# i8run/BigDL

Measured on AMD Instinct MI355X. Metric: images/sec (whole node) ResNet-50 224x224 bf16 at 1/2/4/8 MI355X, higher is better.
Workload: dtype bf16; 1 GPU; model=ResNet-50 v1.5 (BigDL ImageNet builder), global_batch=256, per_gpu_batch=256, image=224, parallelism=dp1, optimizer=SGD momentum 0.9 + L2 1e-4 (one rank: no gradient exchange), hip_graph=False, wgrad_side_stream=True, bucketed_overlap=False, grad_compress=none (no exchange)

## Files before the change

bigdl_amd/nn/conv.py:

```python
import math

import torch
import torch.nn.functional as F

from .. import ops
from ..ops import bn as bnops
from ..ops import conv as cv
from ..ops import conv_fn
from ..ops import side_stream
from .abstractnn import AutogradModule, TensorModule, _t_begin, _t_end
from .init_methods import RandomUniform, Zeros

CL = torch.channels_last
BF16 = torch.bfloat16


def _same_pad(inp, k, s, d=1):
    out = -(-inp // s)
    total = max((out - 1) * s + (k - 1) * d + 1 - inp, 0)
    return total // 2, total - total // 2


class SpatialConvolution(TensorModule):
    def __init__(self, nInputPlane, nOutputPlane, kernelW, kernelH, strideW=1, strideH=1, padW=0, padH=0,
# ... 66 lines not shown
            return 0, 0
        bh, ah = _same_pad(H, self.kernelH, self.strideH, self.dilationH)
        bw, aw = _same_pad(W, self.kernelW, self.strideW, self.dilationW)
        return ah - bh, aw - bw

    def _prep(self, x):
        H, W = x.shape[2], x.shape[3]
        ph, pw = self._pads(H, W)
        eh, ew = self._same_extra(H, W)
        if eh or ew:
            x = F.pad(x, (0, ew, 0, eh))
            if x.is_cuda:
                x = x.contiguous(memory_format=CL)
        return x, ph, pw, eh, ew

    def _nchw(self, x):
        if self.format == "NHWC":
            return x.permute(0, 3, 1, 2)
        return x

    def _fmt_out(self, y):
        if self.format == "NHWC":
            return y.permute(0, 2, 3, 1)
        return y

    def _pre_ok(self, x):
        if not (x.is_cuda and x.dim() == 4 and self.format == "NCHW" and self.nGroup == 1
                and x.shape[1] == self.nInputPlane and x.shape[1] % 8 == 0 and x.dtype == BF16
                and x.is_contiguous(memory_format=CL)):
            return False
        if self._same_extra(x.shape[2], x.shape[3]) != (0, 0) or self._pair_path(x):
            return False
        return getattr(self, "_fuse_out", None) is None and getattr(self, "_fuse_addend", None) is None

    def updateOutput(self, input):
        if getattr(input, "_bn_pre", None) is not None and not self._pre_ok(input):
            input = bnops.materialize(input)
        x = self._nchw(input)
        squeeze = x.dim() == 3
        if squeeze:
            x = x.unsqueeze(0)
        x, ph, pw, _, _ = self._prep(x)
        if x.is_cuda and self.nGroup == 1:
            y = self._fwd_gpu(x, ph, pw)
        elif x.is_cuda:
            y = self._fwd_gpu_grouped(x, ph, pw)
        else:
            y = F.conv2d(x.float(), self.weight, self.bias, (self.strideH, self.strideW), (ph, pw),
                         (self.dilationH, self.dilationW), self.nGroup)
            if self.fuse_relu:
                y = torch.relu(y)
        if squeeze:
            y = y.squeeze(0)
        return self._fmt_out(y)

    def _w16_padded(self):
        w16 = self.w16("weight")
        if w16.shape[1] % 8 != 0:
            w16 = cv.weight_krsc_bf16(w16.float())
        return w16

    def _pair_path(self, x):
        return (cv.pair_ok(x.shape[1], (self.strideH, self.strideW), (self.dilationH, self.dilationW), self.nGroup)
                and self.nInputPlane == x.shape[1] and getattr(self, "_fuse_out", None) is None
                and getattr(self, "_fuse_addend", None) is None)

    def _fwd_gpu_pairs(self, x, ph, pw):
        R, S, sh = self.kernelH, self.kernelW, self.strideH
        OH, OW, S2, _, _ = cv.pair_geometry(x.shape[2], x.shape[3], R, S, sh, ph, pw)
        xp = cv.to_pairs_bf16(x, R, S, sh, ph, pw)
        self._xpair = (xp, tuple(x.shape), ph, pw)
        self._x16 = None
        wp = cv.pair_weight(self.w16("weight"))
        stats = None
        if self.emit_stats and self.train and self.nOutputPlane % 8 == 0:
            stats = bnops.new_stats(self.nOutputPlane, x.device)
        y = cv.conv2d_pairs_fwd(xp, wp, self.bias, self.nOutputPlane, OH, OW, R, S2, sh, relu=self.fuse_relu,
                                stats=stats)
        if stats is not None:
            y._bn_stats = stats
        self._geom = (x.shape, ph, pw)
        return y

    def _wgrad_gpu_pairs(self, x, gy16):
        xp, shape, ph, pw = self._xpair
        R, S, K = self.kernelH, self.kernelW, self.nOutputPlane
        S2 = (S + 1) // 2
        dwp = ops.zeros(K, R * S2 * 8, device=x.device)
        db = None
        if self.bias is not None:
            db = self.gradBias if self.scaleB == 1.0 else ops.zeros(K, device=x.device)
        cv.conv2d_pairs_wgrad(gy16, xp, R, S2, self.strideH, dwp, db)
        ops.native.get().pair_wgrad_add(dwp, self.gradWeight, float(self.scaleW))
        if db is not None and db is not self.gradBias:
            self.gradBias.add_(db, alpha=self.scaleB)

    def _fwd_gpu(self, x, ph, pw):
        self._xpair = None
        self._x16_pre = None
        pre = getattr(x, "_bn_pre", None)
        if self._pair_path(x) and self.nOutputPlane % 8 == 0 and pre is None:
            return self._fwd_gpu_pairs(x, ph, pw)
        x16 = cv.to_nhwc_bf16(x)
        self._x16 = x16
        w16 = self._w16_padded()
        stats = None
        if self.emit_stats and self.train and self.nOutputPlane % 8 == 0:
            stats = bnops.new_stats(self.nOutputPlane, x.device)
        out, addend = getattr(self, "_fuse_out", None), getattr(self, "_fuse_addend", None)
        self._fuse_out = self._fuse_addend = None
        y = cv.conv2d_fwd(x16, w16, self.bias, (self.strideH, self.strideW), (ph, pw),
                          (self.dilationH, self.dilationW), relu=self.fuse_relu, stats=stats, out=out,
                          addend=addend, pre=pre)
        if pre is not None:
            y, mat = y
            if mat is None:
                self._x16_pre = pre
            else:
                self._x16 = mat
        if stats is not None:
            y._bn_stats = stats
        self._geom = (x.shape, ph, pw)
        return y

    def _direct_groups(self):
        return self.nGroup > 1 and self.nInputPlane // self.nGroup <= 16

    def _geo_g(self, ph, pw):
        return [self.strideH, self.strideW, ph, pw, self.dilationH, self.dilationW, self.nGroup]

    def _fwd_gpu_grouped(self, x, ph, pw):
        G = self.nGroup
        cin, cout = self.nInputPlane // G, self.nOutputPlane // G
        if self._direct_groups():
            xf = x.float().contiguous()
            OH = cv.out_size(x.shape[2], self.kernelH, self.strideH, ph, self.dilationH)
            OW = cv.out_size(x.shape[3], self.kernelW, self.strideW, pw, self.dilationW)
            y = xf.new_empty(x.shape[0], self.nOutputPlane, OH, OW)
            ops.native.get().gconv(0, xf, self.weight.float().contiguous(),
                                   self.bias.float().contiguous() if self.bias is not None else None, y,
                                   self._geo_g(ph, pw))
            if self.fuse_relu:
                y.relu_()
            self._xf = xf
            self._geom = (x.shape, ph, pw)
            return y.to(BF16).contiguous(memory_format=CL)
        outs = []
        w = self.weight
        self._x16 = cv.to_nhwc_bf16(x) if x.shape[1] % 8 == 0 else None
        for g in range(G):
            xg = cv.to_nhwc_bf16(x[:, g * cin:(g + 1) * cin].contiguous(memory_format=CL))
            wg = cv.weight_krsc_bf16(w[g * cout:(g + 1) * cout])
            bg = self.bias[g * cout:(g + 1) * cout] if self.bias is not None else None
            outs.append(cv.conv2d_fwd(xg, wg, bg, (self.strideH, self.strideW), (ph, pw),
                                      (self.dilationH, self.dilationW), relu=self.fuse_relu))
        self._geom = (x.shape, ph, pw)
        return torch.cat(outs, dim=1).contiguous(memory_format=CL)

    def updateGradInput(self, input, gradOutput):
        if not self.propagateBack:
            return None
        x = self._nchw(input)
        gy = self._nchw(gradOutput)
        squeeze = x.dim() == 3
        if squeeze:
            x, gy = x.unsqueeze(0), gy.unsqueeze(0)
        H, W = x.shape[2], x.shape[3]
        x, ph, pw, eh, ew = self._prep(x)
        compact = getattr(self, "_dgrad_compact_once", False) and not (squeeze or eh or ew or self.format != "NCHW")
        self._dgrad_compact_once = False
        if gy.is_cuda:
            gy = self._relu_mask(gy)
            once = getattr(self, "_dgrad_bn_once", False)
            self._dgrad_bn_once = False
            bn_src = getattr(input, "_bn_bwd", None) if (getattr(self, "_dgrad_bn_ok", False) or once) else None
# ... 27 lines not shown
            if gy16.shape[1] % 8:
                gy16 = cv.pad_dim(gy16, 1)
                w16 = cv.pad_dim(w16, 0)
            wt = getattr(self, "_wt_cache", None)
            if getattr(self, "_wt_stamp", None) != cv.WT_STAMP[0] or wt is None or \
                    tuple(wt.shape) != (w16.shape[1], w16.shape[2], w16.shape[3], w16.shape[0]):
                wt = cv.transpose_w(w16)
            Cp = w16.shape[1]
            xs = (x.shape[0], Cp, x.shape[2], x.shape[3])
            addend = getattr(self, "_dgrad_addend", None)
            self._dgrad_addend = None
            addend_zm = None
            if isinstance(addend, tuple):
                addend, addend_zm = addend
            if addend is not None and Cp != x.shape[1]:
                raise RuntimeError("dgrad addend requires unpadded channels")
            bn = None
            if bn_src is not None and Cp == x.shape[1]:
                bnmod, bx, bmean, baff, bz = bn_src
                bzm = None
                if bz is not None and bz.dtype == torch.uint8:
                    bz, bzm = None, bz
                bn = {"x": bx, "z": bz, "zm": bzm, "mean": bmean, "aff": baff,
                      "red": bnops.new_stats(Cp, gy16.device)}
            gi = cv.conv2d_dgrad(gy16, wt, xs, (self.strideH, self.strideW), (ph, pw),
                                 (self.dilationH, self.dilationW), addend=addend, bn=bn, addend_zm=addend_zm,
                                 compact=compact and Cp == x.shape[1])
            if Cp != x.shape[1]:
                gi = gi[:, : x.shape[1]].contiguous(memory_format=CL)
            elif bn is not None and bn.get("done"):
                gi._bn_red = (bnmod, bn["red"])
            return gi
        G = self.nGroup
        cin, cout = self.nInputPlane // G, self.nOutputPlane // G
        if self._direct_groups():
            gyf = gy.float().contiguous()
            dx = torch.empty(x.shape[0], self.nInputPlane, x.shape[2], x.shape[3], device=gy.device)
            ops.native.get().gconv(1, dx, self.weight.float().contiguous(), None, gyf, self._geo_g(ph, pw))
            return dx.to(BF16).contiguous(memory_format=CL)
        parts = []
        for g in range(G):
            wg = cv.pad_dim(cv.weight_krsc_bf16(self.weight[g * cout:(g + 1) * cout]), 0)
            gyg = cv.pad_dim(gy16[:, g * cout:(g + 1) * cout].contiguous(memory_format=CL), 1)
            xs = (x.shape[0], wg.shape[1], x.shape[2], x.shape[3])
            gi = cv.conv2d_dgrad(gyg, cv.transpose_w(wg), xs, (self.strideH, self.strideW), (ph, pw),
                                 (self.dilationH, self.dilationW))
            parts.append(gi[:, :cin])
        return torch.cat(parts, dim=1).contiguous(memory_format=CL)

    def backward(self, input, gradOutput):
        side = None if self._frozen else side_stream.stream_for(gradOutput)
        if side is None:
            return super().backward(input, gradOutput)
        t0 = _t_begin(gradOutput)
        self.gradInput = self.updateGradInput(input, gradOutput)
        side_stream.begin(side)
        with torch.cuda.stream(side):
            self.accGradParameters(input, gradOutput)
            self._apply_regularizers()
        side_stream.keep(side, input, gradOutput, self.output, getattr(self, "_x16", None),
                         *(getattr(self, "_xpair", None) or (None,))[:1])
        _t_end(self, t0, "backward_time")
        return self.gradInput

    def accGradParameters(self, input, gradOutput):
        x = self._nchw(input)
        gy = self._nchw(gradOutput)
        if x.dim() == 3:
            x, gy = x.unsqueeze(0), gy.unsqueeze(0)
        x, ph, pw, _, _ = self._prep(x)
        if gy.is_cuda:
            gy = self._relu_mask(gy) if self.fuse_relu and not getattr(self, "_masked_cached", False) else gy
            self._wgrad_gpu(x, gy, ph, pw)
            return
        gy = self._relu_mask(gy).float()
        gw = torch.nn.grad.conv2d_weight(x.float(), self.weight.shape, gy, (self.strideH, self.strideW), (ph, pw),
                                         (self.dilationH, self.dilationW), self.nGroup)
        self.gradWeight.add_(gw, alpha=self.scaleW)
        if self.bias is not None:
            self.gradBias.add_(gy.sum(dim=(0, 2, 3)), alpha=self.scaleB)

    def _wgrad_gpu(self, x, gy, ph, pw):
        gy16 = gy if (gy.dtype == BF16 and gy.is_contiguous(memory_format=CL)) else gy.to(BF16, memory_format=CL)
        xpair = getattr(self, "_xpair", None)
        if (xpair is not None and xpair[1] == tuple(x.shape) and xpair[2:] == (ph, pw) and self.nGroup == 1
                and self.gradWeight.dtype == torch.float32):
            self._wgrad_gpu_pairs(x, gy16)
            return
        x16 = getattr(self, "_x16", None)
        pre = None
        if x16 is None or x16.shape[0] != x.shape[0] or x16.shape[2:] != x.shape[2:]:
            x16 = cv.to_nhwc_bf16(bnops.materialize(x))
        elif getattr(self, "_x16_pre", None) is not None:
            pre = self._x16_pre
        st, pd, dl = (self.strideH, self.strideW), (ph, pw), (self.dilationH, self.dilationW)
        if self.nGroup != 1 and self._direct_groups():
            xf = getattr(self, "_xf", None)
            if xf is None or xf.shape != x.shape:
                xf = x.float().contiguous()
            dw = ops.zeros(self.weight.shape, device=x.device)
            db = ops.zeros(self.nOutputPlane, device=x.device) if self.bias is not None else None
            ops.native.get().gconv(2, xf, dw, db, gy.float().contiguous(), self._geo_g(pd[0], pd[1]))
            self.gradWeight.add_(dw, alpha=self.scaleW)
            if db is not None:
                self.gradBias.add_(db, alpha=self.scaleB)
            return
        if self.nGroup != 1:
            G = self.nGroup
            cin, cout = self.nInputPlane // G, self.nOutputPlane // G
            for g in range(G):
                xg = cv.to_nhwc_bf16(x[:, g * cin:(g + 1) * cin].contiguous(memory_format=CL))
                gyg = cv.pad_dim(gy16[:, g * cout:(g + 1) * cout].contiguous(memory_format=CL), 1)
                dw = ops.zeros(gyg.shape[1], xg.shape[1], self.kernelH, self.kernelW, device=x.device,
                               memory_format=CL)
                db = ops.zeros(gyg.shape[1], device=x.device) if self.bias is not None else None
                cv.conv2d_wgrad(gyg, xg, dw, db, st, pd, dl)
                self.gradWeight[g * cout:(g + 1) * cout].add_(dw[:cout, :cin], alpha=self.scaleW)
                if db is not None:
                    self.gradBias[g * cout:(g + 1) * cout].add_(db[:cout], alpha=self.scaleB)
            return
        K = self.nOutputPlane
        direct = (x16.shape[1] == self.nInputPlane and K % 8 == 0 and self.scaleW == 1.0 and self.scaleB == 1.0
                  and self.gradWeight.is_contiguous(memory_format=CL))
        if pre is not None and not direct:
            x16 = bnops.materialize(bnops.deferred(x16, pre))
        if direct:
            cv.conv2d_wgrad(gy16, x16, self.gradWeight, self.gradBias, st, pd, dl, pre=pre)
        else:
            gyp = cv.pad_dim(gy16, 1)
            dw = ops.zeros(gyp.shape[1], x16.shape[1], self.kernelH, self.kernelW, device=x.device,
                           memory_format=CL)
            db = ops.zeros(gyp.shape[1], device=x.device) if self.bias is not None else None
            cv.conv2d_wgrad(gyp, x16, dw, db, st, pd, dl)
            self.gradWeight.add_(dw[:K, : self.nInputPlane], alpha=self.scaleW)
            if db is not None:
                self.gradBias.add_(db[:K], alpha=self.scaleB)

    def clearState(self):
        super().clearState()
        self._x16 = None
        self._x16_pre = None
        self._xpair = None
        return self

    def __repr__(self):
        return (f"SpatialConvolution({self.nInputPlane} -> {self.nOutputPlane}, {self.kernelW} x {self.kernelH}, "
                f"{self.strideW}, {self.strideH}, {self.padW}, {self.padH})")


class SpatialShareConvolution(SpatialConvolution):
    """Reference shares im2col buffers across layers to save host memory (ResNet ``optnet``). On the GPU
    engine there is no im2col buffer at all (implicit GEMM), so this is SpatialConvolution."""


class SpatialDilatedConvolution(SpatialConvolution):
    def __init__(self, nInputPlane, nOutputPlane, kW, kH, dW=1, dH=1, padW=0, padH=0, dilationW=1, dilationH=1,
                 wRegularizer=None, bRegularizer=None):
        super().__init__(nInputPlane, nOutputPlane, kW, kH, dW, dH, padW, padH, wRegularizer=wRegularizer,
                         bRegularizer=bRegularizer, dilationW=dilationW, dilationH=dilationH)


class SpatialFullConvolution(AutogradModule):

    def __init__(self, nInputPlane, nOutputPlane, kW, kH, dW=1, dH=1, padW=0, padH=0, adjW=0, adjH=0, nGroup=1,
                 noBias=False, wRegularizer=None, bRegularizer=None):
        super().__init__()
        self.nInputPlane, self.nOutputPlane = nInputPlane, nOutputPlane
        self.kW, self.kH, self.dW, self.dH = kW, kH, dW, dH
        self.padW, self.padH, self.adjW, self.adjH, self.nGroup = padW, padH, adjW, adjH, nGroup
        self.wRegularizer, self.bRegularizer = wRegularizer, bRegularizer
        self.register_parameter("weight", "gradWeight", torch.empty(nInputPlane, nOutputPlane // nGroup, kH, kW))
# ... 249 lines not shown
```

bigdl_amd/nn/fusion.py:

```python
import os

import torch

from ..utils.table import Table
from .activation import ReLU
from .containers import ConcatTable, Sequential, add_activity
from .conv import SpatialConvolution
from .linear import Linear
from .normalization import BatchNormalization
from .table_ops import CAddTable


_TRAIN_NODE_ATTRS = ("res_src", "pass_index", "fold_fanout", "fold_bn")


def _reset(m):
    from .graph import Graph

    for x in [m] + list(m.flattened_layers()):
        if isinstance(x, Graph) and getattr(x, "_order0", None) is not None:
            x.order = x._order0
            x._order0 = None
        if isinstance(x, Graph):
            for n in x.order:
                for a in _TRAIN_NODE_ATTRS:
                    n.__dict__.pop(a, None)
        if isinstance(x, BatchNormalization):
            x._graph_dres = False
    for x in m.flattened_layers():
        for attr, val in (("emit_stats", False), ("fuse_relu", False), ("passthrough", False),
                          ("_dgrad_bn_ok", False), ("_defer_ok", False)):
            if hasattr(x, attr):
                setattr(x, attr, val)
        if isinstance(x, Sequential):
            x._residual_plan = None


def _dgrad_bn_enabled():
    return os.environ.get("BIGDL_DGRAD_BN", "1") == "1"


def fuse_for_training(model):
    from .graph import DynamicGraph, Graph

    _reset(model)
    for m in model.flattened_layers():
        if isinstance(m, Sequential):
            _fuse_sequential(m)
        elif isinstance(m, Graph) and not isinstance(m, DynamicGraph) and not getattr(m, "_inference_fused", False):
            _fuse_graph_training(m)
    return model


def _fuse_graph_training(g):
    users = _graph_users(g)
    outs = {n.id for n in g.output_nodes}
    _plan_graph_residuals(g, users, outs)

    def only_user(n):
        us = users.get(n.id, [])
        ok = (len(us) == 1 and n.id not in outs and len(us[0].prevs) == 1 and us[0].prev_index[0] is None
              and not (n.element.hasName() and n.element.getName() in g._stop_grad))
        return us[0] if ok else None

    for n in g.order:
        m, u = n.element, only_user(n)
        if u is None:
            continue
        c = u.element
        if isinstance(m, SpatialConvolution) and isinstance(c, BatchNormalization) and m.nGroup == 1:
            m.emit_stats = True
        elif isinstance(m, BatchNormalization) and isinstance(c, ReLU):
            m.fuse_relu = True
            c.passthrough = True
        elif isinstance(m, (SpatialConvolution, Linear)) and isinstance(c, ReLU):
            m.fuse_relu = True
            c.passthrough = True
    _plan_fanout_folds(g, users)
    for n in g.order:
        m, u = n.element, only_user(n)
        if isinstance(m, BatchNormalization) and u is not None and isinstance(u.element, ReLU):
            v = only_user(u)
            if v is not None:
                _plan_deferred_bn(m, u.element, v.element)
    if not _dgrad_bn_enabled():
        return
    for n in g.order:
        m, u = n.element, only_user(n)
        if not (isinstance(m, BatchNormalization) and m.fuse_relu and u is not None and isinstance(u.element, ReLU)
                and u.element.passthrough):
            continue
        v = only_user(u)
        if v is not None and isinstance(v.element, SpatialConvolution) and v.element.nGroup == 1:
            v.element._dgrad_bn_ok = True


def _stopped(g, n):
    return n.element.hasName() and n.element.getName() in g._stop_grad


def _plan_graph_residuals(g, users, outs):
    for a in list(g.order):
        if not isinstance(a.element, CAddTable) or len(a.prevs) != 2 or any(k is not None for k in a.prev_index):
            continue
        ua = users.get(a.id, [])
        if (len(ua) != 1 or a.id in outs or _stopped(g, a) or not isinstance(ua[0].element, ReLU)
                or len(ua[0].prevs) != 1 or ua[0].prev_index[0] is not None):
            continue
        for ib in (0, 1):
            b, sc = a.prevs[ib], a.prevs[1 - ib]
            bn = b.element
            if (b is sc or not isinstance(bn, BatchNormalization) or users.get(b.id) != [a] or b.id in outs
                    or _stopped(g, b) or bn.fuse_relu or bn.nOutput % 8 != 0 or getattr(b, "res_src", None)):
                continue
            order = g.order
            if order.index(sc) > order.index(b):
                if getattr(g, "_order0", None) is None:
                    g._order0 = list(order)
                order.remove(b)
                order.insert(order.index(sc) + 1, b)
            bn.fuse_relu = True
            bn._graph_dres = True
            b.res_src = sc
            a.pass_index = ib + 1
            ua[0].element.passthrough = True
            break


def _plan_fanout_folds(g, users):
    pos = {n.id: i for i, n in enumerate(g.order)}
    contrib = {}
    for n in g.order:
        rs = getattr(n, "res_src", None)
        if rs is not None:
            contrib.setdefault(rs.id, []).append(n)
    for p in g.order:
        us = [u for u in users.get(p.id, []) if getattr(u, "pass_index", None) is None]
        srcs = us + contrib.get(p.id, [])
        if len(srcs) < 2:
            continue
        c = min(srcs, key=lambda u: pos[u.id])
        cv = c.element
        if (c not in us or len(c.prevs) != 1 or c.prev_index[0] is not None or _stopped(g, c)
                or not isinstance(cv, SpatialConvolution) or cv.nGroup != 1 or not cv.propagateBack
                or cv.format != "NCHW" or cv.nInputPlane % 8 != 0):
            continue
        c.fold_fanout = True
        c.fold_bn = _dgrad_bn_enabled()


def unfuse(model):
    _reset(model)
    return model


def _last_leaf(m):
    while isinstance(m, Sequential) and m.modules and m._residual_plan is None:
        m = m.modules[-1]
    return m


def _fuse_sequential(seq):
    mods = seq.modules
    if (len(mods) == 3 and isinstance(mods[0], ConcatTable) and len(mods[0].modules) == 2
            and isinstance(mods[1], CAddTable) and isinstance(mods[2], ReLU)):
        branch, short = mods[0].modules
        if isinstance(branch, Sequential) and branch.modules and isinstance(branch.modules[-1], BatchNormalization):
            bn = branch.modules[-1]
            if bn.nOutput % 8 == 0:
                bn.fuse_relu = True
                seq._residual_plan = (branch, short, bn)
    for a, b in zip(mods[:-1], mods[1:]):
        if isinstance(a, SpatialConvolution) and isinstance(b, BatchNormalization) and a.nGroup == 1:
            a.emit_stats = True
        elif isinstance(a, BatchNormalization) and isinstance(b, ReLU):
            a.fuse_relu = True
            b.passthrough = True
    for a, b, c in zip(mods[:-2], mods[1:-1], mods[2:]):
        if (_dgrad_bn_enabled() and isinstance(a, BatchNormalization) and a.fuse_relu and isinstance(b, ReLU) and b.passthrough
                and isinstance(c, SpatialConvolution) and c.nGroup == 1):
            c._dgrad_bn_ok = True
        elif isinstance(a, (SpatialConvolution, Linear)) and isinstance(b, ReLU):
            a.fuse_relu = True
            b.passthrough = True
    for a, b, c in zip(mods[:-2], mods[1:-1], mods[2:]):
        _plan_deferred_bn(a, b, c)


DEFER_LEVEL = [int(os.environ.get("BIGDL_BN_DEFER", "1") or 0)]


def _defer_consumer(c):
    from .pooling import SpatialMaxPooling

    if isinstance(c, SpatialConvolution):
        if DEFER_LEVEL[0] < 2:
            return False
        return (c.nGroup == 1 and c.format == "NCHW" and type(c).updateOutput is SpatialConvolution.updateOutput
                and type(c)._wgrad_gpu is SpatialConvolution._wgrad_gpu and c.kernelW == 3 and c.kernelH == 3
                and c.strideW == 1 and c.strideH == 1 and c.dilationW == 1 and c.dilationH == 1)
    return DEFER_LEVEL[0] >= 1 and type(c) is SpatialMaxPooling and c.format == "NCHW"


def _plan_deferred_bn(a, b, c):
    if (isinstance(a, BatchNormalization) and a.fuse_relu and not getattr(a, "_graph_dres", False)
            and isinstance(b, ReLU) and b.passthrough and _defer_consumer(c)):
        a._defer_ok = True


def residual_forward(seq, x):
    branch, short, bn = seq._residual_plan
    concat, add, relu = seq.modules
    res = short.forward(x)
    h = x
    for m in branch.modules[:-1]:
        h = m.forward(h)
    if tuple(res.shape) != tuple(h.shape[:1]) + (bn.nOutput,) + tuple(h.shape[2:]):
        raise ValueError(f"residual block: shortcut output {tuple(res.shape)} does not match the branch output")
    out = bn.updateOutput(h, residual=res)
    bn.output = out
    branch.output = out
    concat.output = Table(out, res)
    add.output = out
    relu.output = out
    seq._res_h = h
    return out


MASKED_ADDEND = [os.environ.get("BIGDL_MASKED_ADDEND", "1") != "0"]


SHORTCUT_BN_RED = [os.environ.get("BIGDL_SHORTCUT_BN_RED", "1") != "0"]


def _native_det():
    from ..ops import native

    return native.deterministic()


def _compact_shortcut_conv(short, first, x):
    from ..ops import conv as cv

    if not (cv.COMPACT_SHORTCUT[0] and isinstance(short, Sequential) and len(short.modules) == 2):
        return None
    sconv, sbn = short.modules
    if not (isinstance(sconv, SpatialConvolution) and isinstance(sbn, BatchNormalization)
            and type(sconv).updateGradInput is SpatialConvolution.updateGradInput
            and type(sconv)._dgrad_gpu is SpatialConvolution._dgrad_gpu
            and torch.is_tensor(x) and x.is_cuda and x.dim() == 4 and x.dtype == torch.bfloat16
            and x.is_contiguous(memory_format=torch.channels_last)):
        return None

    def plain_1x1(c, strided):
        return (c.kernelH == 1 and c.kernelW == 1 and c.padH == 0 and c.padW == 0 and c.nGroup == 1
                and c.format == "NCHW" and c.propagateBack and not c._frozen
                and c.nInputPlane == x.shape[1] and c.nInputPlane % 8 == 0 and c.nOutputPlane % 8 == 0
                and ((c.strideH > 1 and c.strideW > 1) if strided else (c.strideH == 1 and c.strideW == 1)))

    if not (plain_1x1(sconv, True) and plain_1x1(first, False)
            and type(first)._dgrad_gpu is SpatialConvolution._dgrad_gpu):
        return None
    N, C, H, W = x.shape
    stride = (sconv.strideH, sconv.strideW)
    if not all(cv.addend_stride_applies(N, first.nOutputPlane, H, W, C, stride, bnm) for bnm in (0, 1, 2)):
        return None
    return sconv


def residual_backward(seq, x, gradOutput):
    branch, short, bn = seq._residual_plan
    mods = branch.modules
    first = mods[0]
    sconv = None
    can_fold = (isinstance(first, SpatialConvolution) and first.propagateBack and first.nGroup == 1
                and first.format == "NCHW" and first.nInputPlane % 8 == 0)
    masked = None
    zm = getattr(bn, "_zm", None)
    if (MASKED_ADDEND[0] and can_fold and zm is not None and type(short).__name__ == "Identity" and first.strideH == 1
            and first.strideW == 1 and torch.is_tensor(gradOutput) and gradOutput.is_cuda
            and tuple(gradOutput.shape) == tuple(x.shape) and x.dtype == torch.bfloat16):
        dh, _ = bn.backward_fused(seq._res_h, gradOutput, need_dres=False)
        gz = gradOutput
        if gz.dtype != torch.bfloat16 or not gz.is_contiguous(memory_format=torch.channels_last):
            gz = gz.to(torch.bfloat16).contiguous(memory_format=torch.channels_last)
        masked = (gz, zm)
        gs = None
    else:
        sec, sbn = None, None
        if SHORTCUT_BN_RED[0] and isinstance(short, Sequential) and short.modules:
            sbn = short.modules[-1]
            xs = getattr(sbn, "_xin", None)
            xb = getattr(bn, "_xin", None)
            if (isinstance(sbn, BatchNormalization) and sbn.train and not sbn.fuse_relu and xs is not None
                    and xb is not None and xs.is_cuda and xs.shape == xb.shape and xs.stride() == xb.stride()
                    and xs.dtype == torch.bfloat16 and xs.shape[1] % 8 == 0 and not _native_det()):
                from ..ops import bn as bnops

                sec = (xs, sbn.saveMean, bnops.new_stats(xs.shape[1], xs.device))
        dh, dres = bn.backward_fused(seq._res_h, gradOutput, need_dres=True, sec=sec)
        if sec is not None:
            dres._bn_red = (sbn, sec[2])
        sconv = _compact_shortcut_conv(short, first, x) if can_fold else None
        if sconv is not None:
            sconv._dgrad_compact_once = True
        gs = short.backward(x, dres)
        if sconv is not None:
            sconv._dgrad_compact_once = False
    bn.gradInput = dh
    from ..ops import conv as cv

    compact = gs is not None and cv.compact_stride(gs) is not None
    if compact and not (can_fold and sconv is not None and gs.dtype == x.dtype):
        gs, compact = cv.expand_compact(gs, x.shape[2], x.shape[3]), False
    fold = masked is not None or (can_fold and gs is not None and gs.dtype == x.dtype
                                  and (compact or gs.shape == x.shape))
    g = dh
    for i in range(len(mods) - 2, -1, -1):
        inp = mods[i - 1].output if i > 0 else x
        if i == 0 and fold:
            first._dgrad_addend = masked if masked is not None else gs
            first._dgrad_bn_once = _dgrad_bn_enabled()
        g = mods[i].backward(inp, g)
    return g if fold else add_activity(g, gs)


def _graph_users(g):
    users = {}
    for n in g.order:
        for p in n.prevs:
            users.setdefault(p.id, []).append(n)
    return users


def _conv_fusable(n):
    m = n.element
    return (type(m).__name__ in ("SpatialConvolution", "SpatialShareConvolution", "SpatialDilatedConvolution")
            and isinstance(m, SpatialConvolution) and m.nGroup == 1 and m.format == "NCHW")


def _conv_out_shape(conv, x):
    from ..ops.conv import out_size

    N, _, H, W = x.shape
    ph, pw = conv._pads(H, W)
    return (N, conv.nOutputPlane, out_size(H, conv.kernelH, conv.strideH, ph, conv.dilationH),
            out_size(W, conv.kernelW, conv.strideW, pw, conv.dilationW))


def _topo_with_deps(g, extra):
    order, state = [], {}
    for root in list(g.output_nodes) + list(g.inputs_nodes):
        stack = [(root, False)]
        while stack:
            n, done = stack.pop()
            if done:
                if state.get(n.id) != 2:
                    state[n.id] = 2
                    order.append(n)
                continue
            st = state.get(n.id)
            if st == 2:
                continue
            if st == 1:
                raise ValueError("inference fusion created a cycle")
            state[n.id] = 1
            stack.append((n, True))
            for p in reversed(list(n.prevs) + extra.get(n.id, [])):
                if state.get(p.id) != 2:
                    if state.get(p.id) == 1:
                        raise ValueError("inference fusion created a cycle")
                    stack.append((p, False))
    return order


class _ResidualLink:

    def __init__(self, conv, other_id, add, idx, relu):
        self.conv, self.other_id, self.add, self.idx, self.relu = conv, other_id, add, idx, relu
        self.used = False

    def pre_conv(self, outs, x):
        import torch
# ... 140 lines not shown
```

bigdl_amd/nn/normalization.py:

```python
import math
import os

import torch
import torch.nn.functional as F

from .. import ops
from ..ops import bn as bnops
from .abstractnn import AutogradModule, TensorModule, _t_begin, _t_end
from .init_methods import Ones, RandomUniform, Zeros

_ZMASK = os.environ.get("BIGDL_BN_ZMASK", "1") != "0"
_DEFER = [os.environ.get("BIGDL_BN_DEFER", "1") != "0"]
CL = torch.channels_last
BF16 = torch.bfloat16


class BatchNormalization(TensorModule):

    def __init__(self, nOutput, eps=1e-5, momentum=0.1, affine=True, initWeight=None, initBias=None,
                 initGradWeight=None, initGradBias=None, dataFormat="NCHW"):
        super().__init__()
        self.nOutput = nOutput
        self.eps = eps
        self.momentum = momentum
        self.affine = affine
        self.dataFormat = dataFormat
        self.fuse_relu = False
        self.sync_fn = None
        if affine:
            self.register_parameter("weight", "gradWeight", torch.empty(nOutput))
            self.register_parameter("bias", "gradBias", torch.empty(nOutput))
        else:
            self.weight = self.bias = self.gradWeight = self.gradBias = None
        self.runningMean = torch.zeros(nOutput)
        self.runningVar = torch.ones(nOutput)
        self._buffers = ["runningMean", "runningVar"]
        self.saveMean = None
        self.saveStd = None
        self.weightInitMethod = RandomUniform(0.0, 1.0) if affine else None
        self.biasInitMethod = Zeros()
        self.reset()
        if initWeight is not None and affine:
            self.weight.copy_(torch.as_tensor(initWeight))
        if initBias is not None and affine:
            self.bias.copy_(torch.as_tensor(initBias))
        if initGradWeight is not None and affine:
            self.gradWeight.copy_(torch.as_tensor(initGradWeight))
        if initGradBias is not None and affine:
            self.gradBias.copy_(torch.as_tensor(initGradBias))

    def reset(self):
        if self.affine:
            with torch.no_grad():
                self.weightInitMethod.init(self.weight)
                self.biasInitMethod.init(self.bias)
        self.runningMean.zero_()
        self.runningVar.fill_(1.0)

    def setParallism(self, n):
        from ..parallel.sync_bn import make_sync_fn

        self.sync_fn = make_sync_fn() if n and n > 1 else None
        return self

    def _to_nchw(self, x):
        if self.dataFormat == "NHWC" and x.dim() == 4:
            return x.permute(0, 3, 1, 2)
        return x

    def _from_nchw(self, y):
        if self.dataFormat == "NHWC" and y.dim() == 4:
            return y.permute(0, 2, 3, 1)
        return y

    def _gpu_ok(self, x):
        if not x.is_cuda or self.nOutput % 8 != 0:
            return False
        if x.dim() == 4:
            return True
        return x.dim() == 2

    def _prep_gpu(self, x):
        if x.dim() == 4:
            if x.dtype != BF16 or not x.is_contiguous(memory_format=CL):
                x = x.to(BF16, memory_format=CL)
        else:
            if x.dtype != BF16 or not x.is_contiguous():
                x = x.to(BF16).contiguous()
        return x

    def updateOutput(self, input, residual=None):
        if residual is None:
            residual = self.__dict__.pop("_graph_residual", None)
        x = self._to_nchw(input)
        if self._gpu_ok(x):
            stats = getattr(input, "_bn_stats", None) if self.train else None
            x = self._prep_gpu(x)
            res = residual
            if res is not None and (res.dtype != BF16 or res.stride() != x.stride()):
                res = res.to(BF16).contiguous(memory_format=CL if x.dim() == 4 else torch.contiguous_format)
            zm = None
            if self.train and self.fuse_relu and res is not None and x.shape[1] % 8 == 0 and _ZMASK:
                zm = torch.empty(x.numel() // 8, dtype=torch.uint8, device=x.device)
            if (self.train and self.fuse_relu and res is None and getattr(self, "_defer_ok", False) and _DEFER[0]
                    and x.dim() == 4 and self.dataFormat == "NCHW"):
                sm, si, aff = bnops.bn_prepare_gpu(x, self.weight, self.bias, self.runningMean, self.runningVar,
                                                   self.eps, self.momentum, stats=stats, sync_fn=self.sync_fn)
                self.saveMean, self.saveStd = sm, si
                self._aff, self._zm, self._xin = aff, None, x
                y = bnops.deferred(x, aff)
                y._bn_bwd = (self, x, sm, aff, False)
                return y
            y, sm, si, aff = bnops.bn_forward_gpu(x, self.weight, self.bias, self.runningMean, self.runningVar,
                                                   self.eps, self.momentum, self.train, stats=stats, res=res,
                                                   relu=self.fuse_relu, sync_fn=self.sync_fn if self.train else None,
                                                   zm=zm)
            self.saveMean, self.saveStd = sm, si
            self._aff = aff if (self.fuse_relu and res is None) else None
            self._zm = zm
            self._xin = x
            if self.train and self.fuse_relu:
                y._bn_bwd = (self, x, sm, self._aff, zm if zm is not None else res is not None)
            return self._from_nchw(y)
        xf = x.float()
        y, mean, invstd = bnops.bn_forward_cpu(xf, self.weight, self.bias, self.runningMean, self.runningVar, self.eps,
                                               self.momentum, self.train,
                                               sync_fn=self.sync_fn if self.train else None)
        if residual is not None:
            y = y + residual.float()
        if self.fuse_relu:
            y = torch.relu(y)
        self.saveMean, self.saveStd = mean, invstd
        self._xin = xf
        return self._from_nchw(y.to(input.dtype) if input.is_floating_point() else y)

    def _direct_grads(self):
        return (not self._frozen) and self.affine and self.scaleW == 1.0 and self.scaleB == 1.0

    def backward_fused(self, input, gradOutput, need_dres=False, sec=None):
        gz = self._to_nchw(gradOutput)
        x = self._xin
        if gz.dtype != BF16 or gz.stride() != x.stride():
            gz = gz.to(BF16).contiguous(memory_format=CL if x.dim() == 4 else torch.contiguous_format)
        aff = getattr(self, "_aff", None)
        zm = getattr(self, "_zm", None)
        z = self._to_nchw(self.output) if (self.fuse_relu and aff is None and zm is None) else None
        direct = self._direct_grads()
        dg = self.gradWeight if direct else (torch.zeros_like(self.runningMean) if self.affine else None)
        db = self.gradBias if direct else (torch.zeros_like(self.runningMean) if self.affine else None)
        pre = getattr(gradOutput, "_bn_red", None)
        red = pre[1] if (pre is not None and pre[0] is self and self.train) else None
        graph_res = getattr(self, "_graph_dres", False)
        dx, dres = bnops.bn_backward_gpu(gz, z, x, self.saveMean, self.saveStd, self.weight, dg, db,
                                         training=self.train, need_dres=need_dres or graph_res,
                                         sync_fn=self.sync_fn if self.train else None, aff=aff, red=red, zm=zm,
                                         sec=sec)
        if graph_res:
            self._dres = dres
        if not direct and self.affine and not self._frozen:
            self.gradWeight.add_(dg, alpha=self.scaleW)
            self.gradBias.add_(db, alpha=self.scaleB)
        return self._from_nchw(dx), dres

    def backward(self, input, gradOutput):
        t0 = _t_begin(gradOutput)
        x = self._to_nchw(input)
        if self._gpu_ok(x):
            self.gradInput, _ = self.backward_fused(input, gradOutput)
        else:
            self.gradInput = self.updateGradInput(input, gradOutput)
            if not self._frozen:
                self.accGradParameters(input, gradOutput)
        _t_end(self, t0, "backward_time")
        return self.gradInput

    def _cpu_grads(self, gradOutput):
        gy = self._to_nchw(gradOutput).float()
        if self.fuse_relu:
            gy = gy * (self._to_nchw(self.output) > 0)
        return bnops.bn_backward_cpu(self._xin, gy, self.saveMean, self.saveStd, self.weight, self.train,
                                     sync_fn=self.sync_fn if self.train else None)

    def updateGradInput(self, input, gradOutput):
        x = self._to_nchw(input)
        if self._gpu_ok(x):
            dx, _ = self.backward_fused(input, gradOutput)
            return dx
        gx, dg, db = self._cpu_grads(gradOutput)
        self._pending = (dg, db)
        return self._from_nchw(gx.to(input.dtype))

    def accGradParameters(self, input, gradOutput):
        if not self.affine:
            return
        if input.is_cuda and self._gpu_ok(self._to_nchw(input)):
            return
        pend = getattr(self, "_pending", None)
        if pend is None:
            _, dg, db = self._cpu_grads(gradOutput)
        else:
            dg, db = pend
        self.gradWeight.add_(dg.to(self.gradWeight.device), alpha=self.scaleW)
        self.gradBias.add_(db.to(self.gradBias.device), alpha=self.scaleB)
        self._pending = None

    def __repr__(self):
        return f"{type(self).__name__}[{self.nOutput}, eps={self.eps}, momentum={self.momentum}, affine={self.affine}]"


class SpatialBatchNormalization(BatchNormalization):
    pass


class LayerNormalization(AutogradModule):
    def __init__(self, hiddenSize, eps=1e-6):
        super().__init__()
        self.hiddenSize, self.eps = hiddenSize, eps
        self.register_parameter("weight", "gradWeight", torch.ones(hiddenSize))
        self.register_parameter("bias", "gradBias", torch.zeros(hiddenSize))

    def fn(self, x):
        from ..ops.norm import layer_norm

        xf = x.float()
        y = layer_norm(xf, self.weight, self.bias, self.eps)
        return y.to(x.dtype)


class SpatialCrossMapLRN(AutogradModule):

    def __init__(self, size=5, alpha=1.0, beta=0.75, k=1.0, format="NCHW"):
        super().__init__()
        self.size, self.alpha, self.beta, self.k, self.format = size, alpha, beta, k, format

    def fn(self, x):
        from ..ops import nnk

        xf = x.float()
        if self.format == "NHWC":
# ... 120 lines not shown
```

bigdl_amd/ops/bn.py:

```python
import os
import torch

from . import native


def _P(x):
    return x.numel() // x.shape[1]


def stat_slots():
    return native.get().STAT_SLOTS


class _StatsArena:

    def __init__(self):
        self.buf, self.off, self.active, self.need = None, 0, False, 0

    def begin(self, device):
        if self.need and (self.buf is None or self.buf.numel() < self.need or self.buf.device != device):
            self.buf = torch.empty(self.need, dtype=torch.float32, device=device)
        if self.buf is not None:
            if self.buf.is_cuda and int(os.environ.get("BIGDL_NATIVE_FILL", "7")) & 2:
                native.get().fill_bytes(self.buf, 0)
            else:
                self.buf.zero_()
        self.off, self.need, self.active = 0, 0, True

    def end(self):
        self.active = False

    def take(self, n, device):
        n_al = (n + 63) // 64 * 64
        self.need += n_al
        if self.active and self.buf is not None and self.buf.device == device and self.off + n_al <= self.buf.numel():
            t = self.buf[self.off:self.off + n]
            self.off += n_al
            return t
        t = torch.empty(n, dtype=torch.float32, device=device)
        if t.is_cuda:
            native.get().fill_bytes(t, 0)
            return t
        return t.zero_()


ARENA = _StatsArena()


def new_stats(C, device):
    return ARENA.take(stat_slots() * 2 * C, torch.device(device))


def _reduce_slots_for_sync(buf, C, P, sync_fn):
    red = torch.empty(2 * C, dtype=torch.float32, device=buf.device)
    native.get().bn_slot_reduce(buf, stat_slots(), C, red)
    P = sync_fn(red, P)
    return red, 1, P


def bn_forward_gpu(x, gamma, beta, rmean, rvar, eps, momentum, training, stats=None, res=None, relu=False,
                   out=None, sync_fn=None, zm=None):
    C = x.shape[1]
    P = _P(x)
    C_ = native.get()
    dev = x.device
    if out is None:
        out = torch.empty_like(x)
    aff = torch.empty(2 * C, dtype=torch.float32, device=dev)
    scale, shift = aff[:C], aff[C:]
    smean = torch.empty(C, dtype=torch.float32, device=dev)
    sinv = torch.empty(C, dtype=torch.float32, device=dev)
    nslots = stat_slots()
    Ptot = P
    if training:
        if stats is None:
            stats = new_stats(C, dev)
            C_.bn_stats(x, stats, P, C)
        if sync_fn is not None:
            stats, nslots, Ptot = _reduce_slots_for_sync(stats, C, P, sync_fn)
    else:
        stats, nslots = scale, 0
    C_.bn_finalize(stats, nslots, gamma, beta, rmean, rvar, smean, sinv, scale, shift, Ptot, C, float(eps),
                   float(momentum), bool(training))
    C_.bn_apply(x, scale, shift, res, out, P, C, bool(relu), zm)
    return out, smean, sinv, aff


def bn_prepare_gpu(x, gamma, beta, rmean, rvar, eps, momentum, stats=None, sync_fn=None):
    C = x.shape[1]
    P = _P(x)
    C_ = native.get()
    dev = x.device
    aff = torch.empty(2 * C, dtype=torch.float32, device=dev)
    smean = torch.empty(C, dtype=torch.float32, device=dev)
    sinv = torch.empty(C, dtype=torch.float32, device=dev)
    nslots, Ptot = stat_slots(), P
    if stats is None:
        stats = new_stats(C, dev)
        C_.bn_stats(x, stats, P, C)
    if sync_fn is not None:
        stats, nslots, Ptot = _reduce_slots_for_sync(stats, C, P, sync_fn)
    C_.bn_finalize(stats, nslots, gamma, beta, rmean, rvar, smean, sinv, aff[:C], aff[C:], Ptot, C, float(eps),
                   float(momentum), True)
    return smean, sinv, aff


def deferred(x, aff):
    y = x.detach()
    y._bn_pre = aff
    return y


def materialize(t):
    aff = getattr(t, "_bn_pre", None)
    if aff is None:
        return t
    C = t.shape[1]
    y = torch.empty_like(t)
    native.get().bn_apply(t, aff[:C], aff[C:], None, y, _P(t), C, True)
    return y


def bn_backward_gpu(dz, z, x, smean, sinv, gamma, dgamma, dbeta, training=True, need_dres=False, need_dx=True,
                    sync_fn=None, aff=None, red=None, zm=None, sec=None):
    C = x.shape[1]
    P = _P(x)
    C_ = native.get()
    nslots, Ptot = 0, P
    if not training:
        red = None
    elif red is None:
        red = new_stats(C, x.device)
        C_.bn_bwd_reduce(dz, z, x, smean, red, P, C, aff, zm)
    if training:
        nslots = stat_slots()
        if sync_fn is not None:
            red, nslots, Ptot = _reduce_slots_for_sync(red, C, P, sync_fn)
    coef = torch.empty(3 * C, dtype=torch.float32, device=x.device)
    dx = torch.empty_like(x) if need_dx else None
    dres = torch.empty_like(x) if need_dres else None
    if sec is not None and dres is not None and training:
        x2, mean2, red2 = sec
        C_.bn_bwd_apply(dz, z, x, smean, sinv, gamma, red, nslots, coef, dx, dres, dgamma, dbeta, Ptot, C, aff, zm,
                        x2=x2, mean2=mean2, red2=red2)
    else:
        C_.bn_bwd_apply(dz, z, x, smean, sinv, gamma, red, nslots, coef, dx, dres, dgamma, dbeta, Ptot, C, aff, zm)
    return dx, dres


def bn_forward_cpu(x, gamma, beta, rmean, rvar, eps, momentum, training, sync_fn=None):
    dims = [0] + list(range(2, x.dim()))
    shape = [1, -1] + [1] * (x.dim() - 2)
    if training:
        n = x.numel() // x.shape[1]
        if sync_fn is not None:
            buf = torch.cat([x.sum(dim=dims), (x * x).sum(dim=dims)]).double()
            n = sync_fn(buf, n)
            C = x.shape[1]
            mean = (buf[:C] / n).float()
            var = (buf[C:] / n - (buf[:C] / n) ** 2).clamp_min(0).float()
        else:
            mean = x.mean(dim=dims)
            var = x.var(dim=dims, unbiased=False)
        if rmean is not None:
            unb = var * n / max(n - 1, 1)
            rmean.mul_(1 - momentum).add_(momentum * mean)
            rvar.mul_(1 - momentum).add_(momentum * unb)
    else:
        mean, var = rmean, rvar
    invstd = torch.rsqrt(var + eps)
    xhat = (x - mean.view(shape)) * invstd.view(shape)
    y = xhat
    if gamma is not None:
        y = y * gamma.view(shape) + beta.view(shape)
    return y, mean, invstd


def bn_backward_cpu(x, gy, mean, invstd, gamma, training=True, sync_fn=None):
    dims = [0] + list(range(2, x.dim()))
    shape = [1, -1] + [1] * (x.dim() - 2)
    xhat = (x - mean.view(shape)) * invstd.view(shape)
    g = gamma.view(shape) if gamma is not None else 1.0
    dgamma = (gy * xhat).sum(dim=dims)
    dbeta = gy.sum(dim=dims)
    if training:
        n = x.numel() // x.shape[1]
        sdg, sdb = dgamma, dbeta
        if sync_fn is not None:
            buf = torch.cat([dbeta, dgamma]).double()
            n = sync_fn(buf, n)
            C = x.shape[1]
            sdb, sdg = buf[:C].float(), buf[C:].float()
        gx = g * invstd.view(shape) * (gy - sdb.view(shape) / n - xhat * sdg.view(shape) / n)
    else:
        gx = g * invstd.view(shape) * gy
    return gx, dgamma, dbeta
```

bigdl_amd/ops/conv.py:

```python
import os
import torch
import torch.nn.functional as F

from . import native

CL = torch.channels_last
BF16 = torch.bfloat16


def out_size(inp, k, s, p, d=1, ceil=False):
    eff = d * (k - 1) + 1
    num = inp + 2 * p - eff
    if ceil:
        o = -(-num // s) + 1
        if (o - 1) * s >= inp + p:
            o -= 1
        return o
    return num // s + 1


def to_nhwc_bf16(x, cpad=8):
    N, C, H, W = x.shape
    Cp = -(-C // cpad) * cpad
    if x.dtype == BF16 and Cp == C and x.is_contiguous(memory_format=CL):
# ... 268 lines not shown

def gemm_wgrad_nt(dy2d, x2d, dw32, dbias32=None):
    P, K = dy2d.shape
    C = x2d.shape[1]
    dyT, xT = _rows_T64(dy2d), _rows_T64(x2d)
    P64 = dyT.shape[1]
    geo = [K, 1, 1, P64, 1, 1, 1, 1, P64, C, C, 1, 1, 1, 1, 0, 0]
    native.get().conv_nt(dyT, xT, dw32.view(K, C), None, None, geo, [0, 0, 0], False, accumulate=True)
    if dbias32 is not None:
        native.get().colsum_bf16(dy2d, dbias32)


def pair_ok(C, stride, dil, groups):
    import os

    return (groups == 1 and C <= 4 and stride[1] == 2 and tuple(dil) == (1, 1)
            and os.environ.get("BIGDL_CONV_PAIR", "1") != "0")


def pair_geometry(H, W, R, S, sh, ph, pw):
    OH, OW = out_size(H, R, sh, ph), out_size(W, S, 2, pw)
    S2 = (S + 1) // 2
    Hp = max(H + 2 * ph, (OH - 1) * sh + R)
    Wp = max(2 * (OW - 1 + S2), W + 2 * pw)
    return OH, OW, S2, Hp, Wp + (Wp & 1)


def to_pairs_bf16(x, R, S, sh, ph, pw):
    N, C, H, W = x.shape
    _, _, _, Hp, Wp = pair_geometry(H, W, R, S, sh, ph, pw)
    y = torch.empty((N, Hp, Wp // 2, 8), dtype=BF16, device=x.device)
    xf = x if (x.dtype == torch.float32 and x.is_contiguous()) else x.float().contiguous()
    native.get().nchw_to_pairs(xf, y, ph, pw)
    return y


def pair_weight(w16):
    K, C, R, S = w16.shape
    wp = torch.empty((K, R * ((S + 1) // 2) * 8), dtype=BF16, device=w16.device)
    native.get().pair_weight(w16, wp)
    return wp


def _pair_taps(R, S2):
    key = ("p", R, S2)
    t = _TAP_CACHE.get(key)
    if t is None:
        t = []
        for r in range(R):
            for j in range(S2):
                t += [r, j, r * S2 + j]
        _TAP_CACHE[key] = t
    return t


def _window_taps(R):
    key = ("w", R)
    t = _TAP_CACHE.get(key)
    if t is None:
        t = [v for r in range(R) for v in (r, 0, r)]
        _TAP_CACHE[key] = t
    return t


def conv2d_pairs_fwd(xp, wp, bias, K, OH, OW, R, S2, sh, relu=False, stats=None):
    N, Hp, Wq, _ = xp.shape
    out = torch.empty((N, K, OH, OW), dtype=BF16, device=xp.device, memory_format=CL)
    if S2 == 4 and os.environ.get("BIGDL_STEM_WINDOW", "0") != "0":
        geo = [N, Hp, Wq, 32, OH, OW, sh, 1, R * 32, K, K, OH, OW, 1, 1, 0, 0, 8]
        det = stats is not None and native.deterministic()
        native.get().conv_nt(xp, wp, out, bias, None if det else stats, geo, _window_taps(R), relu, None)
        if det:
            native.get().bn_stats(out, stats, N * OH * OW, K)
        return out
    geo = [N, Hp, Wq, 8, OH, OW, sh, 1, R * S2 * 8, K, K, OH, OW, 1, 1, 0, 0]
    if stats is not None and native.deterministic():
        native.get().conv_nt(xp, wp, out, bias, None, geo, _pair_taps(R, S2), relu, None)
        native.get().bn_stats(out, stats, N * OH * OW, K)
        return out
    native.get().conv_nt(xp, wp, out, bias, stats, geo, _pair_taps(R, S2), relu, None)
    return out


def conv2d_pairs_wgrad(dy, xp, R, S2, sh, dwp32, dbias32):
    N, Hp, Wq, _ = xp.shape
    _, K, OH, OW = dy.shape
    geo = [N, Hp, Wq, 8, OH, OW, R, S2, sh, 1, 0, 0, 1, 1, N * OH * OW, K, R * S2 * 8, K]
    native.get().conv_wgrad(dy, xp, dwp32, dbias32, geo)


def conv2d_wgrad(dy, x, dw32, dbias32, stride, pad, dil=(1, 1), pre=None):
    N, C, H, W = x.shape
    _, K, OH, OW = dy.shape
    Kw, Cw, R, S = dw32.shape
    assert Kw == K and Cw == C
    P = N * OH * OW
    sh, sw = stride
    ph, pw = pad
    dh, dw = dil
    geo = [N, H, W, C, OH, OW, R, S, sh, sw, ph, pw, dh, dw, N * OH * OW, K, R * S * C, K]
    if pre is not None and _gemm_shaped(dy, x, dw32, stride, pad, dil):
        from . import bn as bnops

        x, pre = bnops.materialize(bnops.deferred(x, pre)), None
    if (P >= 512 and ((K + 127) // 128) * ((C + 127) // 128) >= 192 and _gemm_shaped(dy, x, dw32, stride, pad, dil)
            and not native.get().conv_wgrad_uses_p8(geo, dbias32 is not None)):
        gemm_wgrad_nt(dy.reshape(P, K) if dy.is_contiguous() else dy.permute(0, 2, 3, 1).reshape(P, K),
                      x.reshape(P, C) if x.is_contiguous() else x.permute(0, 2, 3, 1).reshape(P, C), dw32, dbias32)
        return
    native.get().conv_wgrad(dy, x, dw32, dbias32, geo, pre)


def conv2d_cpu(x, w, b, stride, pad, dil=(1, 1), groups=1):
    return F.conv2d(x, w, b, stride=stride, padding=pad, dilation=dil, groups=groups)


def conv2d_grads_cpu(x, w, gy, stride, pad, dil=(1, 1), groups=1, need_input=True):
    gi = None
    if need_input:
        gi = torch.nn.grad.conv2d_input(x.shape, w, gy, stride=stride, padding=pad, dilation=dil, groups=groups)
    gw = torch.nn.grad.conv2d_weight(x, w.shape, gy, stride=stride, padding=pad, dilation=dil, groups=groups)
    gb = gy.sum(dim=(0, 2, 3))
    return gi, gw, gb
```

csrc/batchnorm.hip:

```cpp
#include "common.h"
#include "kernels.h"
#include <stdlib.h>

#define STAT_SLOTS BIGDL_STAT_SLOTS

namespace {

template <int MODE, int U>
__global__ __launch_bounds__(256) void chan_reduce_kernel(const bf16_t* __restrict__ x, const bf16_t* __restrict__ dz,
                                                          const bf16_t* __restrict__ z, const float* __restrict__ mean,
                                                          float* __restrict__ out, long P, int C, long rows_per_block,
                                                          const float* __restrict__ aff, const uint8_t* __restrict__ zm) {
  __shared__ float sm[256 * 16];
  const int G = C >> 3;
  const int tid = threadIdx.x;
  const long rbeg = blockIdx.x * rows_per_block;
  const long rend = min(P, rbeg + rows_per_block);
  for (int gbase = 0; gbase < G; gbase += 256) {
    const int gcount = min(256, G - gbase);
    const int rpi = 256 / gcount;
    const int g = gbase + tid % gcount, rsub = tid / gcount;
    float a1[8], a2[8], mu[8], sc[8], sh[8];
#pragma unroll
    for (int e = 0; e < 8; ++e) { a1[e] = 0.f; a2[e] = 0.f; mu[e] = 0.f; sc[e] = 0.f; sh[e] = 0.f; }
// ... 46 lines not shown
              if (xmask) {
                if (!(xl * sc[2 * e] + sh[2 * e] > 0.f)) dl = 0.f;
                if (!(xh * sc[2 * e + 1] + sh[2 * e + 1] > 0.f)) dh = 0.f;
              }
              a1[2 * e] += dl; a1[2 * e + 1] += dh;
              a2[2 * e] += dl * (xl - mu[2 * e]);
              a2[2 * e + 1] += dh * (xh - mu[2 * e + 1]);
            }
          }
        }
      }
    }
#pragma unroll
    for (int e = 0; e < 8; ++e) { sm[tid * 16 + e] = a1[e]; sm[tid * 16 + 8 + e] = a2[e]; }
    __syncthreads();
    for (int w = tid; w < gcount * 16; w += 256) {
      const int gg = w >> 4, slot = w & 15;
      float t = 0.f;
      for (int rs = 0; rs < rpi; ++rs) t += sm[(rs * gcount + gg) * 16 + slot];
      const int ch = (gbase + gg) * 8 + (slot & 7);
      atomicAdd(out + (size_t)(blockIdx.x & (STAT_SLOTS - 1)) * 2 * C + (slot < 8 ? 0 : C) + ch, t);
    }
    __syncthreads();
  }
}

int bn_unroll() {
  static int u = [] {
    const char* e = getenv("BIGDL_BN_UNROLL");
    const int v = e ? atoi(e) : 4;
    return (v == 1 || v == 2 || v == 8) ? v : 4;
  }();
  return u;
}

__device__ __forceinline__ void slot_sums(const float* __restrict__ red, int nslots, int C, int c, int sl, double& s1,
                                          double& s2) {
  s1 = 0.0;
  s2 = 0.0;
  for (int k = sl; k < nslots; k += 32) {
    s1 += red[(size_t)k * 2 * C + c];
    s2 += red[(size_t)k * 2 * C + C + c];
  }
#pragma unroll
  for (int o = 16; o > 0; o >>= 1) {
    s1 += __shfl_xor(s1, o, 64);
    s2 += __shfl_xor(s2, o, 64);
  }
}

__global__ void bn_finalize_kernel(const float* __restrict__ stats, int nslots, const float* __restrict__ gamma,
                                   const float* __restrict__ beta, float* run_mean, float* run_var, float* save_mean,
                                   float* save_invstd, float* scale, float* shift, long P, int C, float eps,
                                   float momentum, int training) {
  const int lane = threadIdx.x & 63, sl = lane & 31;
  const int c = (blockIdx.x * (blockDim.x >> 6) + (threadIdx.x >> 6)) * 2 + (lane >> 5);
  if (c >= C) return;
  float mean, invstd;
  if (training) {
    double s1, s2;
    slot_sums(stats, nslots, C, c, sl, s1, s2);
    if (sl != 0) return;
    mean = (float)(s1 / (double)P);
    const float var = fmaxf((float)(s2 / (double)P - (double)mean * mean), 0.f);
    invstd = rsqrtf(var + eps);
    save_mean[c] = mean;
    save_invstd[c] = invstd;
    if (run_mean) {
      const float unbiased = P > 1 ? var * (float)P / (float)(P - 1) : var;
      run_mean[c] = momentum * mean + (1.f - momentum) * run_mean[c];
      run_var[c] = momentum * unbiased + (1.f - momentum) * run_var[c];
    }
  } else {
    if (sl != 0) return;
    mean = run_mean[c];
    invstd = rsqrtf(run_var[c] + eps);
    if (save_mean) { save_mean[c] = mean; save_invstd[c] = invstd; }
  }
  const float g = gamma ? gamma[c] : 1.f, b = beta ? beta[c] : 0.f;
  scale[c] = g * invstd;
  shift[c] = b - mean * g * invstd;
}

template <int U>
__global__ __launch_bounds__(256) void bn_apply_kernel(const bf16_t* __restrict__ x, const float* __restrict__ scale,
                                                       const float* __restrict__ shift, const bf16_t* __restrict__ res,
                                                       bf16_t* __restrict__ y, long P, int C, long rpb, int relu,
                                                       uint8_t* __restrict__ zm) {
  const int G = C >> 3;
  const int gbase = blockIdx.y * 256;
  const int gcount = min(256, G - gbase);
  const int rpi = 256 / gcount;
  const int g = gbase + threadIdx.x % gcount, rsub = threadIdx.x / gcount;
  if (rsub >= rpi) return;
  const long rbeg = blockIdx.x * rpb, rend = min(P, rbeg + rpb);
  const int c0 = g * 8;
  const v4f s0 = *reinterpret_cast<const v4f*>(scale + c0), s1 = *reinterpret_cast<const v4f*>(scale + c0 + 4);
  const v4f b0 = *reinterpret_cast<const v4f*>(shift + c0), b1 = *reinterpret_cast<const v4f*>(shift + c0 + 4);
  const float sc[8] = {s0[0], s0[1], s0[2], s0[3], s1[0], s1[1], s1[2], s1[3]};
  const float sh[8] = {b0[0], b0[1], b0[2], b0[3], b1[0], b1[1], b1[2], b1[3]};
  for (long r0 = rbeg + rsub; r0 < rend; r0 += (long)U * rpi) {
    v4u vx[U], vr[U];
#pragma unroll
    for (int u = 0; u < U; ++u) {
      const long r = r0 + (long)u * rpi;
      const long i = (r < rend ? r : rbeg) * G + g;
      vx[u] = reinterpret_cast<const v4u*>(x)[i];
      vr[u] = v4u{0u, 0u, 0u, 0u};
      if (res) vr[u] = reinterpret_cast<const v4u*>(res)[i];
    }
#pragma unroll
    for (int u = 0; u < U; ++u) {
      const long r = r0 + (long)u * rpi;
      v4u o;
#pragma unroll
      for (int e = 0; e < 4; ++e) {
        float l = lo_bf(vx[u][e]) * sc[2 * e] + sh[2 * e];
        float h = hi_bf(vx[u][e]) * sc[2 * e + 1] + sh[2 * e + 1];
        if (res) { l += lo_bf(vr[u][e]); h += hi_bf(vr[u][e]); }
        if (relu) { l = fmaxf(l, 0.f); h = fmaxf(h, 0.f); }
        o[e] = pack2bf(l, h);
      }
      if (r < rend) {
        reinterpret_cast<v4u*>(y)[r * G + g] = o;
        if (zm) zm[r * G + g] = (uint8_t)bf_to_mask8(o);
      }
    }
  }
}

__global__ void bn_bwd_coeff_kernel(const float* __restrict__ red, int nslots, const float* __restrict__ mean,
                                    const float* __restrict__ invstd, const float* __restrict__ gamma,
                                    float* __restrict__ coef, float* dgamma, float* dbeta, long P, int C, int training) {
  const int lane = threadIdx.x & 63, sl = lane & 31;
  const int c = (blockIdx.x * (blockDim.x >> 6) + (threadIdx.x >> 6)) * 2 + (lane >> 5);
  if (c >= C) return;
  double sdy = 0.0, sdyx = 0.0;
  if (training) slot_sums(red, nslots, C, c, sl, sdy, sdyx);
  if (sl != 0) return;
  const float is = invstd[c];
  const float g = gamma ? gamma[c] : 1.f;
  float A = g * is, B = 0.f, D = 0.f;
  if (training) {
    const float mdy = (float)(sdy / (double)P);
    const float mdyx = (float)(sdyx / (double)P) * is;
    B = -g * is * is * mdyx;
    D = g * is * (mean[c] * is * mdyx - mdy);
    if (dgamma) dgamma[c] += (float)sdyx * is;
    if (dbeta) dbeta[c] += (float)sdy;
  }
  coef[c] = A; coef[C + c] = B; coef[2 * C + c] = D;
}

__global__ void bn_slot_reduce_kernel(const float* __restrict__ in, int nslots, int C, float* __restrict__ out) {
  const int c = blockIdx.x * blockDim.x + threadIdx.x;
  if (c >= 2 * C) return;
  float t = 0.f;
  for (int k = 0; k < nslots; ++k) t += in[(size_t)k * 2 * C + c];
  out[c] = t;
}

__device__ __forceinline__ void load8(const float* p, float* v) {
  const v4f a = *reinterpret_cast<const v4f*>(p), b = *reinterpret_cast<const v4f*>(p + 4);
  v[0] = a[0]; v[1] = a[1]; v[2] = a[2]; v[3] = a[3]; v[4] = b[0]; v[5] = b[1]; v[6] = b[2]; v[7] = b[3];
}

template <int U, bool R2>
__global__ __launch_bounds__(256) void bn_bwd_apply_kernel(const bf16_t* __restrict__ dz, const bf16_t* __restrict__ z,
                                                           const bf16_t* __restrict__ x, const float* __restrict__ coef,
                                                           bf16_t* __restrict__ dx, bf16_t* __restrict__ dres, long P,
                                                           int C, long rpb, const float* __restrict__ aff,
                                                           const uint8_t* __restrict__ zm, const bf16_t* __restrict__ x2,
                                                           const float* __restrict__ mean2, float* __restrict__ red2) {
  const int G = C >> 3;
  const bool xmask = z == nullptr && zm == nullptr && aff != nullptr;
  const __amdgpu_buffer_rsrc_t rzm = __builtin_amdgcn_make_buffer_rsrc(
      const_cast<uint8_t*>(zm), (short)0, zm ? (int)min(P * C / 8, 0x7fffffffl) : 0, 0x00020000);
  const bf16_t* zp = (z && !zm) ? z : x;
  const int gbase = blockIdx.y * 256;
  const int gcount = min(256, G - gbase);
  const int rpi = 256 / gcount;
  const int g = gbase + threadIdx.x % gcount, rsub = threadIdx.x / gcount;
  if (!R2 && rsub >= rpi) return;
  const long rbeg = blockIdx.x * rpb, rend = rsub < rpi ? min(P, rbeg + rpb) : rbeg;
  const int c0 = g * 8;
  float A[8], B[8], D[8], S[8], T[8], M2[8], a1[8], a2[8];
  load8(coef + c0, A);
  load8(coef + C + c0, B);
  load8(coef + 2 * C + c0, D);
  if (xmask) {
    load8(aff + c0, S);
    load8(aff + C + c0, T);
  }
  if (R2) {
    load8(mean2 + c0, M2);
#pragma unroll
    for (int e = 0; e < 8; ++e) { a1[e] = 0.f; a2[e] = 0.f; }
  }
  for (long r0 = rbeg + rsub; r0 < rend; r0 += (long)U * rpi) {
    v4u vd[U], vz[U], vx[U], vx2[U];
    unsigned zb[U];
#pragma unroll
    for (int u = 0; u < U; ++u) {
      const long r = r0 + (long)u * rpi;
      const long i = (r < rend ? r : rbeg) * G + g;
      vd[u] = reinterpret_cast<const v4u*>(dz)[i];
      zb[u] = __builtin_amdgcn_raw_buffer_load_b8(rzm, (unsigned)i, 0, 0);
      vz[u] = reinterpret_cast<const v4u*>(zp)[i];
      vx[u] = reinterpret_cast<const v4u*>(x)[i];
      if (R2) vx2[u] = reinterpret_cast<const v4u*>(x2)[i];
    }
#pragma unroll
    for (int u = 0; u < U; ++u)
      vz[u] = zm ? mask8_to_bf(zb[u]) : z ? vz[u] : v4u{0xffffffffu, 0xffffffffu, 0xffffffffu, 0xffffffffu};
#pragma unroll
    for (int u = 0; u < U; ++u) {
      const long r = r0 + (long)u * rpi;
      v4u o, od;
#pragma unroll
      for (int e = 0; e < 4; ++e) {
        float d0 = lo_bf(vd[u][e]), d1 = hi_bf(vd[u][e]);
        const float x0 = lo_bf(vx[u][e]), x1 = hi_bf(vx[u][e]);
        if (z || zm) { if (!(lo_bf(vz[u][e]) > 0.f)) d0 = 0.f; if (!(hi_bf(vz[u][e]) > 0.f)) d1 = 0.f; }
        if (xmask) {
          if (!(x0 * S[2 * e] + T[2 * e] > 0.f)) d0 = 0.f;
          if (!(x1 * S[2 * e + 1] + T[2 * e + 1] > 0.f)) d1 = 0.f;
        }
        const float r0v = A[2 * e] * d0 + B[2 * e] * x0 + D[2 * e];
        const float r1v = A[2 * e + 1] * d1 + B[2 * e + 1] * x1 + D[2 * e + 1];
        o[e] = pack2bf(r0v, r1v);
        od[e] = pack2bf(d0, d1);
        if (R2 && r < rend) {
          const float q0 = lo_bf(od[e]), q1 = hi_bf(od[e]);
          a1[2 * e] += q0; a1[2 * e + 1] += q1;
          a2[2 * e] += q0 * (lo_bf(vx2[u][e]) - M2[2 * e]);
          a2[2 * e + 1] += q1 * (hi_bf(vx2[u][e]) - M2[2 * e + 1]);
        }
      }
      if (r < rend) {
        if (dx) reinterpret_cast<v4u*>(dx)[r * G + g] = o;
        if (dres) reinterpret_cast<v4u*>(dres)[r * G + g] = od;
      }
    }
  }
  if (R2) {
    __shared__ float sm[256 * 16];
#pragma unroll
    for (int e = 0; e < 8; ++e) { sm[threadIdx.x * 16 + e] = a1[e]; sm[threadIdx.x * 16 + 8 + e] = a2[e]; }
    __syncthreads();
    for (int w = threadIdx.x; w < gcount * 16; w += 256) {
      const int gg = w >> 4, slot = w & 15;
      float t = 0.f;
      for (int rs = 0; rs < rpi; ++rs) t += sm[(rs * gcount + gg) * 16 + slot];
      const int ch = (gbase + gg) * 8 + (slot & 7);
      atomicAdd(red2 + (size_t)(blockIdx.x & (STAT_SLOTS - 1)) * 2 * C + (slot < 8 ? 0 : C) + ch, t);
    }
  }
}

dim3 stationary_grid(long P, int C, long* rpb_out) {
  const int G = C >> 3;
  const int rpi = 256 / (G < 256 ? G : 256);
  const int gy = (G + 255) / 256;
  long rpb = (long)rpi * 8;
  long bx = (P + rpb - 1) / rpb;
  const long cap = 8192 / gy;
  if (bx > cap) {
    bx = cap;
    rpb = (P + bx - 1) / bx;
  }
  if (bx < 1) bx = 1;
  *rpb_out = rpb;
  return dim3((unsigned)bx, (unsigned)gy);
}

int grid_for(long work, int per_block, int cap) {
  long g = (work + per_block - 1) / per_block;
  if (g > cap) g = cap;
  if (g < 1) g = 1;
  return (int)g;
}

void launch_reduce(int mode, const bf16_t* x, const bf16_t* dz, const bf16_t* z, const float* mean, float* out, long P,
                   int C, hipStream_t st, const float* aff = nullptr, const uint8_t* zm = nullptr) {
  const int G = C >> 3;
  const int rpi = 256 / (G < 256 ? G : 256);
  long blocks = (P + rpi * 16 - 1) / (rpi * 16);
  if (blocks > 2048) blocks = 2048;
  if (bigdl_deterministic() && blocks > 2 * STAT_SLOTS) blocks = 2 * STAT_SLOTS;
  if (blocks < 1) blocks = 1;
  const long rpb = (P + blocks - 1) / blocks;
  blocks = (P + rpb - 1) / rpb;
#define BN_RED(M, U) chan_reduce_kernel<M, U><<<(int)blocks, 256, 0, st>>>(x, dz, z, mean, out, P, C, rpb, aff, zm)
  if (mode == 0) { aff = nullptr; zm = nullptr; }
  switch (bn_unroll()) {
    case 1: if (mode == 0) BN_RED(0, 1); else BN_RED(1, 1); break;
    case 2: if (mode == 0) BN_RED(0, 2); else BN_RED(1, 2); break;
    case 8: if (mode == 0) BN_RED(0, 8); else BN_RED(1, 8); break;
    default: if (mode == 0) BN_RED(0, 4); else BN_RED(1, 4); break;
  }
#undef BN_RED
}

}

extern "C" {

void bigdl_bn_stats(const uint16_t* x, float* stats, long P, int C, hipStream_t st) {
  launch_reduce(0, x, nullptr, nullptr, nullptr, stats, P, C, st);
  HIP_LAUNCH_CHECK();
}

void bigdl_bn_finalize(const float* stats, int nslots, const float* gamma, const float* beta, float* run_mean,
                       float* run_var, float* save_mean, float* save_invstd, float* scale, float* shift, long P, int C,
                       float eps, float momentum, int training, hipStream_t st) {
  bn_finalize_kernel<<<(C + 7) / 8, 256, 0, st>>>(stats, nslots, gamma, beta, run_mean, run_var, save_mean,
                                                   save_invstd, scale, shift, P, C, eps, momentum, training);
  HIP_LAUNCH_CHECK();
}

void bigdl_bn_slot_reduce(const float* in, int nslots, int C, float* out, hipStream_t st) {
  bn_slot_reduce_kernel<<<(2 * C + 255) / 256, 256, 0, st>>>(in, nslots, C, out);
  HIP_LAUNCH_CHECK();
}

void bigdl_bn_apply(const uint16_t* x, const float* scale, const float* shift, const uint16_t* res, uint16_t* y,
                    long P, int C, int relu, hipStream_t st, uint8_t* zm) {
  long rpb = 0;
  const dim3 grid = stationary_grid(P, C, &rpb);
  switch (bn_unroll()) {
    case 1: bn_apply_kernel<1><<<grid, 256, 0, st>>>(x, scale, shift, res, y, P, C, rpb, relu, zm); break;
    case 2: bn_apply_kernel<2><<<grid, 256, 0, st>>>(x, scale, shift, res, y, P, C, rpb, relu, zm); break;
    case 8: bn_apply_kernel<8><<<grid, 256, 0, st>>>(x, scale, shift, res, y, P, C, rpb, relu, zm); break;
    default: bn_apply_kernel<4><<<grid, 256, 0, st>>>(x, scale, shift, res, y, P, C, rpb, relu, zm); break;
  }
  HIP_LAUNCH_CHECK();
}

void bigdl_bn_bwd_reduce(const uint16_t* dz, const uint16_t* z, const uint16_t* x, const float* mean, float* red,
                         long P, int C, const float* aff, hipStream_t st, const uint8_t* zm) {
  launch_reduce(1, x, dz, z, mean, red, P, C, st, aff, zm);
  HIP_LAUNCH_CHECK();
}

void bigdl_bn_bwd_apply(const uint16_t* dz, const uint16_t* z, const uint16_t* x, const float* mean,
                        const float* invstd, const float* gamma, const float* red, int nslots, float* coef,
                        uint16_t* dx, uint16_t* dres, float* dgamma, float* dbeta, long P, int C, int training,
                        const float* aff, hipStream_t st, const uint8_t* zm, const uint16_t* x2u,
                        const float* mean2, float* red2) {
  const bf16_t* x2 = reinterpret_cast<const bf16_t*>(x2u);
  bn_bwd_coeff_kernel<<<(C + 7) / 8, 256, 0, st>>>(red, nslots, mean, invstd, gamma, coef, dgamma, dbeta, P, C,
                                                    training);
  if (dx || dres) {
    long rpb = 0;
    const dim3 grid = stationary_grid(P, C, &rpb);
    if (red2) {
#define BWD2(UU) bn_bwd_apply_kernel<UU, true><<<grid, 256, 0, st>>>(dz, z, x, coef, dx, dres, P, C, rpb, aff, zm, x2, mean2, red2)
      switch (bn_unroll()) {
        case 1: BWD2(1); break;
        case 2: BWD2(2); break;
        case 8: BWD2(8); break;
        default: BWD2(4); break;
      }
#undef BWD2
    } else {
#define BWD1(UU) bn_bwd_apply_kernel<UU, false><<<grid, 256, 0, st>>>(dz, z, x, coef, dx, dres, P, C, rpb, aff, zm, nullptr, nullptr, nullptr)
      switch (bn_unroll()) {
        case 1: BWD1(1); break;
        case 2: BWD1(2); break;
        case 8: BWD1(8); break;
        default: BWD1(4); break;
      }
#undef BWD1
    }
  }
  HIP_LAUNCH_CHECK();
}

}
```

csrc/bindings.cpp:

```cpp
#include <torch/extension.h>
#include <ATen/hip/HIPContext.h>
#include <vector>
#include <algorithm>
#include "kernels.h"

namespace {

using at::Tensor;
using OptT = c10::optional<Tensor>;

hipStream_t stream() { return at::hip::getCurrentHIPStream().stream(); }

void check(const Tensor& t, at::ScalarType dt, const char* name) {
  TORCH_CHECK(t.is_cuda(), name, " must be a GPU tensor");
  TORCH_CHECK(t.scalar_type() == dt, name, " has dtype ", t.scalar_type(), ", expected ", dt);
}
const uint16_t* cbf(const Tensor& t, const char* n) { check(t, at::kBFloat16, n); return (const uint16_t*)t.data_ptr(); }
uint16_t* mbf(const Tensor& t, const char* n) { check(t, at::kBFloat16, n); return (uint16_t*)t.data_ptr(); }
const float* cf(const Tensor& t, const char* n) { check(t, at::kFloat, n); return (const float*)t.data_ptr(); }
float* mf(const Tensor& t, const char* n) { check(t, at::kFloat, n); return (float*)t.data_ptr(); }
const uint16_t* ocbf(const OptT& t, const char* n) { return (t && t->defined()) ? cbf(*t, n) : nullptr; }
uint16_t* ombf(const OptT& t, const char* n) { return (t && t->defined()) ? mbf(*t, n) : nullptr; }
const float* ocf(const OptT& t, const char* n) { return (t && t->defined()) ? cf(*t, n) : nullptr; }
float* omf(const OptT& t, const char* n) { return (t && t->defined()) ? mf(*t, n) : nullptr; }
// ... 85 lines not shown
    TORCH_CHECK(bigdl_conv_addend_stride_applies(&a), "conv_nt: no kernel takes this subsampled addend");
  }
  TORCH_CHECK((a.OH - 1) * a.omul_h + a.ooff_h < a.OHo && (a.OW - 1) * a.omul_w + a.ooff_w < a.OWo,
              "conv_nt: output placement out of range");
  OptT materialised;
  if (a.pre && !bigdl_conv_pre_applies(&a)) {
    Tensor y = at::empty_like(src);
    const int64_t P = src.numel() / a.Cs;
    bigdl_bn_apply(a.src, a.pre, a.pre + a.Cs, nullptr, (uint16_t*)y.data_ptr(), P, a.Cs, 1, stream(), nullptr);
    a.src = (const uint16_t*)y.data_ptr();
    a.pre = nullptr;
    materialised = y;
  }
  a.ws = nullptr;
  Tensor ws;
  const long wsn = bigdl_conv_nt_plan(&a);
  if (wsn > 0) {
    ws = at::empty({wsn}, out.options().dtype(at::kFloat));
    a.ws = ws.data_ptr<float>();
  }
  const int rc = bigdl_conv_nt(&a, stream());
  TORCH_CHECK(rc == 0, "conv_nt: unsupported shape (channels must be a multiple of 8; fp32 output needs Ncol % 8 "
              "== 0 and no fused stats / BN / ReLU / addend)");
  return materialised;
}

bool dgrad_s2(const Tensor& dy, const Tensor& wt, const Tensor& out, const OptT& bn_x, const OptT& bn_z,
              const OptT& bn_mean, const OptT& bn_aff, const OptT& bn_red, const OptT& bn_zm) {
  if (dy.dim() != 4 || out.dim() != 4 || wt.dim() != 4 || !dy.is_contiguous(at::MemoryFormat::ChannelsLast) ||
      !wt.is_contiguous() || wt.size(1) != 3 || wt.size(2) != 3 || wt.size(3) != dy.size(1) ||
      wt.size(0) != out.size(1) || out.size(0) != dy.size(0) || out.stride(1) != 1 ||
      out.scalar_type() != at::kBFloat16 || !out.is_contiguous(at::MemoryFormat::ChannelsLast))
    return false;
  ConvArgs a{};
  a.src = cbf(dy, "dy"); a.wt = cbf(wt, "wt"); a.out = mbf(out, "out");
  a.Nb = (int)dy.size(0); a.Hs = (int)dy.size(2); a.Ws = (int)dy.size(3); a.Cs = (int)dy.size(1);
  a.OH = (int)out.size(2); a.OW = (int)out.size(3);
  a.mul_h = a.mul_w = 1; a.ldw = 9 * a.Cs; a.Ncol = (int)out.size(1); a.ldo = a.Ncol;
  a.OHo = a.OH; a.OWo = a.OW; a.omul_h = a.omul_w = 1; a.ident_out = 1;
  a.ntaps = 9; a.Kdim = 9 * a.Cs; a.M = a.Nb * a.OH * a.OW;
  for (int t = 0; t < 9; ++t) { a.tap_h[t] = (t / 3) == 0; a.tap_w[t] = (t % 3) == 0; a.tap_k[t] = (short)t; }
  bigdl_conv_addend_stride(&a, 1, 1, 0, 0);
  a.bnx = ocbf(bn_x, "bn_x"); a.bnz = ocbf(bn_z, "bn_z"); a.bnmean = ocf(bn_mean, "bn_mean");
  a.bnaff = ocf(bn_aff, "bn_aff"); a.bnred = omf(bn_red, "bn_red");
  if (bn_zm && bn_zm->defined()) a.bnzm = omzm(bn_zm, out.numel() / a.Ncol, a.Ncol, "bn_zm");
  if (a.bnred) {
    TORCH_CHECK(!bigdl_deterministic(), "dgrad_s2: epilogue BN reductions are not deterministic");
    TORCH_CHECK(a.bnx && a.bnmean && bn_x->numel() == out.numel() && bn_mean->numel() >= a.Ncol &&
                    (!a.bnaff || bn_aff->numel() >= 2 * a.Ncol) && bn_red->numel() >= BIGDL_STAT_SLOTS * 2 * a.Ncol,
                "dgrad_s2: bn operands");
  }
  if (!bigdl_dgrad_s2_applies(&a)) return false;
  TORCH_CHECK(bigdl_dgrad_s2(&a, stream()) == 0, "dgrad_s2: launch failed");
  return true;
}

bool conv_addend_stride_applies(std::vector<int64_t> geo, std::vector<int64_t> taps, int64_t sh, int64_t sw,
                                int64_t bn) {
  if (geo.size() != 17 || taps.size() % 3 != 0 || taps.empty() || taps.size() / 3 > CONV_MAX_TAPS) return false;
  ConvArgs a{};
  const uint16_t* present = reinterpret_cast<const uint16_t*>(uintptr_t(256));
  a.src = present; a.wt = present; a.out = const_cast<uint16_t*>(present); a.addend = present;
  if (bn) {
    a.bnx = present; a.bnmean = reinterpret_cast<const float*>(present);
    a.bnred = reinterpret_cast<float*>(const_cast<uint16_t*>(present));
    if (bn == 2) a.bnz = present;
  }
  a.Nb = geo[0]; a.Hs = geo[1]; a.Ws = geo[2]; a.Cs = geo[3]; a.OH = geo[4]; a.OW = geo[5];
  a.mul_h = geo[6]; a.mul_w = geo[7]; a.ldw = geo[8]; a.Ncol = geo[9]; a.ldo = geo[10];
  a.OHo = geo[11]; a.OWo = geo[12]; a.omul_h = geo[13]; a.omul_w = geo[14]; a.ooff_h = geo[15]; a.ooff_w = geo[16];
  a.ntaps = (int)(taps.size() / 3);
  a.Kdim = a.ntaps * a.Cs;
  a.M = a.Nb * a.OH * a.OW;
  a.ident_out = (a.OHo == a.OH && a.OWo == a.OW && a.omul_h == 1 && a.omul_w == 1 && a.ooff_h == 0 && a.ooff_w == 0);
  for (int t = 0; t < a.ntaps; ++t) {
    a.tap_h[t] = (short)taps[3 * t]; a.tap_w[t] = (short)taps[3 * t + 1]; a.tap_k[t] = (short)taps[3 * t + 2];
  }
  if (sh < 2 || sw < 2 || a.OH < 1 || a.OW < 1) return false;
  bigdl_conv_addend_stride(&a, (int)sh, (int)sw, (int)((a.OH + sh - 1) / sh), (int)((a.OW + sw - 1) / sw));
  return bigdl_conv_addend_stride_applies(&a) != 0;
}

void conv_wgrad(const Tensor& dy, const Tensor& src, const Tensor& dw, const OptT& dbias, std::vector<int64_t> geo,
                const OptT& pre) {
  TORCH_CHECK(geo.size() == 18, "conv_wgrad: bad geometry");
  WgradArgs a;
  a.dy = cbf(dy, "dy"); a.src = cbf(src, "src"); a.dw = mf(dw, "dw"); a.dbias = omf(dbias, "dbias");
  int* f = &a.Nb;
  for (int i = 0; i < 18; ++i) f[i] = (int)geo[i];
  a.m_per_split = 0;
  a.ws = nullptr;
  a.splits = 0;
  a.pre = ocf(pre, "pre");
  Tensor det_ws;
  a.det_ws = nullptr;
  if (bigdl_deterministic() && a.dbias) {
    det_ws = at::empty({(int64_t)BIGDL_DET_SLOTS * a.Ncol}, dw.options().dtype(at::kFloat));
    a.det_ws = det_ws.data_ptr<float>();
  }
  Tensor mat;
  if (a.pre) {
    TORCH_CHECK(pre->numel() >= 2 * a.Cs && src.numel() % a.Cs == 0, "conv_wgrad: pre must hold 2 x Cs floats");
    if (!bigdl_wgrad_pre_applies(&a)) {
      mat = at::empty_like(src);
      bigdl_bn_apply(a.src, a.pre, a.pre + a.Cs, nullptr, (uint16_t*)mat.data_ptr(), src.numel() / a.Cs, a.Cs, 1,
                     stream(), nullptr);
      a.src = (const uint16_t*)mat.data_ptr();
      a.pre = nullptr;
    }
  }
  TORCH_CHECK(dw.numel() >= (int64_t)a.Ncol * a.Kdim, "conv_wgrad: dw too small");
  TORCH_CHECK(a.M == a.Nb * a.OH * a.OW, "conv_wgrad: M mismatch");
  TORCH_CHECK(dy.numel() >= (int64_t)(a.M - 1) * a.ldy + a.Ncol, "conv_wgrad: dy too small");
  TORCH_CHECK(src.numel() >= (int64_t)a.Nb * a.Hs * a.Ws * a.Cs, "conv_wgrad: src too small");
  Tensor ws;
  const long wsn = bigdl_conv_wgrad_plan(&a);
  if (wsn > 0) {
    ws = at::empty({wsn}, dw.options().dtype(at::kFloat));
    a.ws = ws.data_ptr<float>();
  }
  const int rc = bigdl_conv_wgrad(&a, stream());
  TORCH_CHECK(rc == 0, "conv_wgrad: unsupported shape (channels must be a multiple of 8)");
}

bool conv_wgrad_uses_p8(std::vector<int64_t> geo, bool bias) {
  TORCH_CHECK(geo.size() == 18, "conv_wgrad_uses_p8: bad geometry");
  WgradArgs a{};
  int* f = &a.Nb;
  for (int i = 0; i < 18; ++i) f[i] = (int)geo[i];
  static float dummy;
  a.dbias = bias ? &dummy : nullptr;
  return bigdl_conv_wgrad_uses_p8(&a) != 0;
}

std::vector<int64_t> conv_wgrad_plan_info(std::vector<int64_t> geo, bool bias) {
  TORCH_CHECK(geo.size() == 18, "conv_wgrad_plan_info: bad geometry");
  WgradArgs a{};
  int* f = &a.Nb;
  for (int i = 0; i < 18; ++i) f[i] = (int)geo[i];
  static float dummy;
  a.dbias = bias ? &dummy : nullptr;
  WgradArgs h = a, p = a;
  const int halo = bigdl_wgrad_halo_plan(&h);
  const int p8 = halo > 0 ? 0 : bigdl_conv_wgrad_uses_p8(&p);
  const long wsn = bigdl_conv_wgrad_plan(&a);
  return {a.splits, wsn, halo, p8, bigdl_conv_wgrad_uses_register_kernel(&a)};
}

void transpose_krsc(const Tensor& w, const Tensor& wt, int64_t K, int64_t RS, int64_t C) {
  TORCH_CHECK(w.numel() == K * RS * C && wt.numel() == K * RS * C, "transpose_krsc: size mismatch");
  bigdl_transpose_krsc(cbf(w, "w"), mbf(wt, "wt"), (int)K, (int)RS, (int)C, stream());
}

void bn_stats(const Tensor& x, const Tensor& stats, int64_t P, int64_t C) {
  TORCH_CHECK(C % 8 == 0 && x.numel() == P * C, "bn_stats: shape");
  TORCH_CHECK(stats.numel() >= BIGDL_STAT_SLOTS * 2 * C, "bn_stats: stats must hold STAT_SLOTS x 2C");
  bigdl_bn_stats(cbf(x, "x"), mf(stats, "stats"), P, (int)C, stream());
}
void bn_finalize(const Tensor& stats, int64_t nslots, const OptT& gamma, const OptT& beta, const OptT& rmean,
                 const OptT& rvar, const OptT& smean, const OptT& sinv, const Tensor& scale, const Tensor& shift,
                 int64_t P, int64_t C, double eps, double momentum, bool training) {
  TORCH_CHECK(stats.numel() >= nslots * 2 * C, "bn_finalize: stats size");
  bigdl_bn_finalize(cf(stats, "stats"), (int)nslots, ocf(gamma, "gamma"), ocf(beta, "beta"), omf(rmean, "rmean"),
                    omf(rvar, "rvar"), omf(smean, "smean"), omf(sinv, "sinv"), mf(scale, "scale"),
                    mf(shift, "shift"), P, (int)C, (float)eps, (float)momentum, training ? 1 : 0, stream());
}
void bn_slot_reduce(const Tensor& in, int64_t nslots, int64_t C, const Tensor& out) {
  TORCH_CHECK(in.numel() >= nslots * 2 * C && out.numel() >= 2 * C, "bn_slot_reduce: size");
  bigdl_bn_slot_reduce(cf(in, "in"), (int)nslots, (int)C, mf(out, "out"), stream());
}
void bn_apply(const Tensor& x, const Tensor& scale, const Tensor& shift, const OptT& res, const Tensor& y, int64_t P,
              int64_t C, bool relu, const OptT& zm) {
  TORCH_CHECK(C % 8 == 0 && x.numel() == P * C && y.numel() == P * C, "bn_apply: shape");
  bigdl_bn_apply(cbf(x, "x"), cf(scale, "scale"), cf(shift, "shift"), ocbf(res, "res"), mbf(y, "y"), P, (int)C,
                 relu ? 1 : 0, stream(), omzm(zm, P, C, "zm"));
}
void bn_bwd_reduce(const Tensor& dz, const OptT& z, const Tensor& x, const Tensor& mean, const Tensor& red, int64_t P,
                   int64_t C, const OptT& aff, const OptT& zm) {
  TORCH_CHECK(C % 8 == 0 && x.numel() == P * C && dz.numel() == P * C, "bn_bwd_reduce: shape");
  TORCH_CHECK(red.numel() >= BIGDL_STAT_SLOTS * 2 * C, "bn_bwd_reduce: red must hold STAT_SLOTS x 2C");
  if (aff && aff->defined()) TORCH_CHECK(aff->numel() >= 2 * C && aff->is_contiguous(), "bn_bwd_reduce: aff is [2C]");
  bigdl_bn_bwd_reduce(cbf(dz, "dz"), ocbf(z, "z"), cbf(x, "x"), cf(mean, "mean"), mf(red, "red"), P, (int)C,
                      ocf(aff, "aff"), stream(), omzm(zm, P, C, "zm"));
}
void bn_bwd_apply(const Tensor& dz, const OptT& z, const Tensor& x, const Tensor& mean, const Tensor& invstd,
                  const OptT& gamma, const OptT& red, int64_t nslots, const Tensor& coef, const OptT& dx,
                  const OptT& dres, const OptT& dgamma, const OptT& dbeta, int64_t P, int64_t C, const OptT& aff,
                  const OptT& zm, const OptT& x2, const OptT& mean2, const OptT& red2) {
  TORCH_CHECK(coef.numel() >= 3 * C, "bn_bwd_apply: coef size");
  const bool r2 = red2 && red2->defined();
  if (r2) {
    TORCH_CHECK(dres && dres->defined() && x2 && x2->defined() && mean2 && mean2->defined(),
                "bn_bwd_apply: red2 needs dres, x2 and mean2");
    TORCH_CHECK(x2->numel() == x.numel() && x2->strides() == x.strides(), "bn_bwd_apply: x2 must match x's layout");
    TORCH_CHECK(mean2->numel() >= C && red2->numel() >= (int64_t)BIGDL_STAT_SLOTS * 2 * C, "bn_bwd_apply: mean2 / red2 size");
  }
  if (aff && aff->defined()) TORCH_CHECK(aff->numel() >= 2 * C && aff->is_contiguous(), "bn_bwd_apply: aff is [2C]");
  const bool training = red && red->defined();
  bigdl_bn_bwd_apply(cbf(dz, "dz"), ocbf(z, "z"), cbf(x, "x"), cf(mean, "mean"), cf(invstd, "invstd"),
                     ocf(gamma, "gamma"), ocf(red, "red"), (int)nslots, mf(coef, "coef"), ombf(dx, "dx"),
                     ombf(dres, "dres"), omf(dgamma, "dgamma"), omf(dbeta, "dbeta"), P, (int)C, training ? 1 : 0,
                     ocf(aff, "aff"), stream(), omzm(zm, P, C, "zm"), r2 ? cbf(*x2, "x2") : nullptr,
                     r2 ? cf(*mean2, "mean2") : nullptr, r2 ? omf(red2, "red2") : nullptr);
}

void dgrad_fill(const Tensor& out, const OptT& addend, int64_t sh, int64_t sw, int64_t mask) {
  TORCH_CHECK(out.dim() == 4 && out.is_contiguous(at::MemoryFormat::ChannelsLast) && out.size(1) % 8 == 0,
              "dgrad_fill: out must be NHWC bf16 with C % 8 == 0");
  TORCH_CHECK(sh * sw <= 32, "dgrad_fill: at most 32 stride phases");
  if (addend && addend->defined())
    TORCH_CHECK(addend->sizes() == out.sizes() && addend->is_contiguous(at::MemoryFormat::ChannelsLast),
                "dgrad_fill: addend must match out (NHWC)");
  bigdl_dgrad_fill(mbf(out, "out"), ocbf(addend, "addend"), out.size(0) * out.size(2) * out.size(3), out.size(2),
                   out.size(3), out.size(1), (int)sh, (int)sw, (unsigned)mask, stream());
}
void hog_cus(int64_t n, double us, const Tensor& done) {
  TORCH_CHECK(done.is_cuda() && done.scalar_type() == at::kInt && done.numel() >= n, "hog_cus: done must be int32 cuda [n]");
  bigdl_hog_cus((int)n, us, done.data_ptr<int>(), stream());
}
void spin_us(double us, const Tensor& done) {
  TORCH_CHECK(done.is_cuda() && done.scalar_type() == at::kInt && done.numel() >= 1, "spin_us: done must be int32 cuda");
  bigdl_spin_us(us, done.data_ptr<int>(), stream());
}
void relu_fwd(const Tensor& x, const Tensor& y) {
  TORCH_CHECK(x.numel() == y.numel(), "relu: size");
  bigdl_relu_fwd(cbf(x, "x"), mbf(y, "y"), x.numel(), stream());
}
void relu_bwd(const Tensor& dy, const Tensor& y, const Tensor& dx) {
  TORCH_CHECK(dy.numel() == y.numel() && dx.numel() == y.numel(), "relu_bwd: size");
  bigdl_relu_bwd(cbf(dy, "dy"), cbf(y, "y"), mbf(dx, "dx"), y.numel(), stream());
}
void add_bf16(const Tensor& a, const Tensor& b, const Tensor& y) {
  TORCH_CHECK(a.numel() == b.numel() && a.numel() == y.numel(), "add: size");
  bigdl_add_bf16(cbf(a, "a"), cbf(b, "b"), mbf(y, "y"), a.numel(), stream());
}
void nchw_to_nhwc(const Tensor& x, const Tensor& y, int64_t Cp) {
  TORCH_CHECK(x.dim() == 4 && x.is_contiguous(), "nchw_to_nhwc: x must be contiguous NCHW");
  const int N = x.size(0), C = x.size(1), H = x.size(2), W = x.size(3);
  TORCH_CHECK(y.numel() == (int64_t)N * H * W * Cp && Cp >= C && Cp % 8 == 0, "nchw_to_nhwc: y size / Cp % 8");
  bigdl_nchw_f32_to_nhwc_bf16(cf(x, "x"), mbf(y, "y"), N, C, H, W, (int)Cp, stream());
}
void nchw_to_pairs(const Tensor& x, const Tensor& y, int64_t ph, int64_t pw) {
  TORCH_CHECK(x.dim() == 4 && x.is_contiguous() && x.size(1) <= 4, "nchw_to_pairs: x must be contiguous NCHW, C <= 4");
  TORCH_CHECK(y.dim() == 4 && y.is_contiguous() && y.size(3) == 8 && y.size(0) == x.size(0), "nchw_to_pairs: y shape");
  const int Hp = y.size(1), Wp = 2 * y.size(2);
  TORCH_CHECK(Hp >= x.size(2) + ph && Wp >= x.size(3) + pw, "nchw_to_pairs: padded image too small");
  bigdl_nchw_to_pairs(cf(x, "x"), mbf(y, "y"), x.size(0), x.size(1), x.size(2), x.size(3), Hp, Wp, (int)ph, (int)pw,
                      stream());
}
void pair_weight(const Tensor& w, const Tensor& wp) {
  TORCH_CHECK(w.dim() == 4 && w.size(1) <= 4, "pair_weight: w must be (K, C<=4, R, S)");
  const int K = w.size(0), C = w.size(1), R = w.size(2), S = w.size(3), S2 = (S + 1) / 2;
  TORCH_CHECK(wp.numel() == (int64_t)K * R * S2 * 8 && wp.is_contiguous(), "pair_weight: wp size");
  const long st[4] = {(long)w.stride(0), (long)w.stride(1), (long)w.stride(2), (long)w.stride(3)};
  bigdl_pair_weight(cbf(w, "w"), mbf(wp, "wp"), K, C, R, S, st, stream());
}
void pair_wgrad_add(const Tensor& dwp, const Tensor& gw, double scale) {
  TORCH_CHECK(gw.dim() == 4 && gw.size(1) <= 4, "pair_wgrad_add: gw must be (K, C<=4, R, S)");
  const int K = gw.size(0), C = gw.size(1), R = gw.size(2), S = gw.size(3), S2 = (S + 1) / 2;
  TORCH_CHECK(dwp.numel() == (int64_t)K * R * S2 * 8 && dwp.is_contiguous(), "pair_wgrad_add: dwp size");
  const long st[4] = {(long)gw.stride(0), (long)gw.stride(1), (long)gw.stride(2), (long)gw.stride(3)};
  bigdl_pair_wgrad_add(cf(dwp, "dwp"), mf(gw, "gw"), K, C, R, S, st, (float)scale, stream());
}
static void bmm_operand(const Tensor& t, const char* n, at::ScalarType ty) {
  TORCH_CHECK(t.is_cuda() && t.scalar_type() == ty, "bmm_nt: ", n, " has the wrong dtype / device");
  TORCH_CHECK(t.stride(2) == 1 && t.stride(1) >= t.size(2) && t.stride(0) >= 0, "bmm_nt: ", n, " rows must be dense");
  const int64_t last = (t.size(0) - 1) * t.stride(0) + (t.size(1) - 1) * t.stride(1) + t.size(2);
  TORCH_CHECK((int64_t)(t.storage().nbytes() / t.element_size()) - t.storage_offset() >= last, "bmm_nt: ", n,
              " view exceeds its storage");
}
void bmm_nt(const Tensor& a, const Tensor& b, const Tensor& c, double alpha, bool accum) {
  TORCH_CHECK(a.dim() == 3 && b.dim() == 3 && c.dim() == 3, "bmm_nt: [batch, rows, K] operands, [batch, M, N] out");
  bmm_operand(a, "a", at::kBFloat16); bmm_operand(b, "b", at::kBFloat16); bmm_operand(c, "c", at::kFloat);
  TORCH_CHECK(a.size(0) == b.size(0) && a.size(0) == c.size(0) && a.size(2) == b.size(2) && c.size(1) == a.size(1) &&
              c.size(2) == b.size(1), "bmm_nt: shapes");
  TORCH_CHECK(a.size(2) % 32 == 0, "bmm_nt: K must be padded to a multiple of 32");
// ... 1130 lines not shown
}
void ones_col_pack(const Tensor& x, const Tensor& xe) {
  TORCH_CHECK(x.dim() == 2 && x.is_contiguous() && x.size(1) % 8 == 0, "ones_col_pack: x must be [M, K] contiguous, K % 8 == 0");
  TORCH_CHECK(xe.dim() == 2 && xe.is_contiguous() && xe.size(0) == x.size(0) && xe.size(1) == x.size(1) + 8,
              "ones_col_pack: xe must be [M, K + 8] contiguous");
  bigdl_ones_col_pack(cbf(x, "x"), mbf(xe, "xe"), x.size(0), (int)x.size(1), stream());
}
void ones_col_acc(const Tensor& gw, const Tensor& gW, const OptT& gB, double sW, double sB) {
  TORCH_CHECK(gW.dim() == 2 && gW.is_contiguous() && gW.size(1) % 4 == 0, "ones_col_acc: gW must be [N, K] contiguous");
  TORCH_CHECK(gw.is_contiguous() && gw.dim() == 2 && gw.size(0) == gW.size(0) && gw.size(1) == gW.size(1) + 8,
              "ones_col_acc: gw must be [N, K + 8] contiguous");
  if (gB && gB->defined()) TORCH_CHECK(gB->numel() == gW.size(0) && gB->is_contiguous(), "ones_col_acc: gB is [N]");
  bigdl_ones_col_acc(cf(gw, "gw"), mf(gW, "gW"), omf(gB, "gB"), gW.size(0), (int)gW.size(1), (float)sW, (float)sB,
                     stream());
}
void colsum_bf16(const Tensor& x, const Tensor& out) {
  TORCH_CHECK(x.dim() == 2 && x.is_contiguous() && x.size(1) % 8 == 0, "colsum_bf16: x must be [P, K] contiguous, K % 8 == 0");
  TORCH_CHECK(out.is_contiguous() && out.numel() == x.size(1), "colsum_bf16: out must hold K floats");
  Tensor ws;
  if (bigdl_deterministic()) ws = at::empty({(int64_t)BIGDL_DET_SLOTS * x.size(1)}, out.options().dtype(at::kFloat));
  bigdl_colsum_bf16(cbf(x, "x"), mf(out, "out"), x.size(0), (int)x.size(1), stream(),
                    ws.defined() ? ws.data_ptr<float>() : nullptr);
}
int64_t rows_of(const OptT& t, int64_t B, int64_t cols, const char* name) {
  if (!(t && t->defined())) return 0;
  TORCH_CHECK(t->dim() == 2 && t->size(0) == B && t->size(1) >= cols && t->stride(1) == 1, name,
              ": expected [B, >=", cols, "] rows with unit inner stride");
  return t->stride(0);
}
void need_flat(const OptT& t, int64_t n, const char* name) {
  if (t && t->defined()) TORCH_CHECK(t->is_contiguous() && t->numel() == n, name, ": expected ", n, " contiguous elements");
}
void gru_step(int64_t mode, const OptT& A, const Tensor& W, int64_t B, int64_t H, const OptT& xg, const OptT& hprev,
              const OptT& r, const OptT& z, const OptT& n, const OptT& rh16, const OptT& hout, const OptT& h16out,
              const OptT& dout, const OptT& dhp, const OptT& dx, const OptT& dn16, const OptT& drz16, const OptT& dh0) {
  TORCH_CHECK(W.dim() == 2 && W.is_contiguous(), "gru_step: W must be [N, K] contiguous");
  const int64_t N = W.size(0), K = W.size(1);
  TORCH_CHECK(H % 32 == 0 && K % 32 == 0 && N % 16 == 0 && B > 0, "gru_step: H, K multiples of 32, N of 16");
  TORCH_CHECK(mode >= 0 && mode <= 4, "gru_step: bad mode");
  TORCH_CHECK(N == (mode == 0 ? 2 * H : H) && K == (mode == 2 || mode == 4 ? 2 * H : H), "gru_step: W shape vs mode");
  GruStepArgs a{};
  a.mode = (int)mode; a.B = (int)B; a.H = (int)H; a.K = (int)K; a.N = (int)N;
  a.W = cbf(W, "W");
  if (A && A->defined()) { a.lda = rows_of(A, B, K, "A"); a.A = cbf(*A, "A"); }
  need_flat(r, B * H, "r"); need_flat(z, B * H, "z"); need_flat(n, B * H, "n"); need_flat(rh16, B * H, "rh16");
  need_flat(h16out, B * H, "h16out"); need_flat(dhp, B * H, "dhp"); need_flat(dn16, B * H, "dn16");
  need_flat(drz16, B * 2 * H, "drz16"); need_flat(dh0, B * H, "dh0");
  a.ldx = rows_of(xg, B, 3 * H, "xg"); a.ldhp = rows_of(hprev, B, H, "hprev"); a.ldho = rows_of(hout, B, H, "hout");
  a.ldd = rows_of(dout, B, H, "dout"); a.lddx = rows_of(dx, B, 3 * H, "dx");
  a.xg = ocf(xg, "xg"); a.hprev = ocf(hprev, "hprev"); a.r = omf(r, "r"); a.z = omf(z, "z"); a.n = omf(n, "n");
  a.rh16 = ombf(rh16, "rh16"); a.hout = omf(hout, "hout"); a.h16out = ombf(h16out, "h16out"); a.dout = ocf(dout, "dout");
  a.dhp = omf(dhp, "dhp"); a.dx = omf(dx, "dx"); a.dn16 = ombf(dn16, "dn16"); a.drz16 = ombf(drz16, "drz16");
  a.dh0 = omf(dh0, "dh0");
  switch (mode) {
    case 0: TORCH_CHECK(a.xg && a.r && a.z && a.rh16, "gru_step fwd r/z: xg, r, z, rh16 required"); break;
    case 1: TORCH_CHECK(a.A && a.xg && a.z && a.n && a.hout && a.h16out, "gru_step fwd n: A, xg, z, n, hout, h16out required"); break;
    case 2: TORCH_CHECK(a.z && a.n && a.dhp && a.dx && a.dn16 && a.drz16, "gru_step bwd h: z, n, dhp, dx, dn16, drz16 required"); break;
    case 3: TORCH_CHECK(a.A && a.r && a.dhp && a.dx && a.drz16, "gru_step bwd r: A, r, dhp, dx, drz16 required"); break;
    default: TORCH_CHECK(a.dhp && a.dh0, "gru_step bwd h0: dhp, dh0 required"); break;
  }
  TORCH_CHECK(bigdl_gru_step(&a, stream()) == 0, "gru_step: unsupported shape");
}

}

void register_host_runtime(pybind11::module& m);

PYBIND11_MODULE(TORCH_EXTENSION_NAME, m) {
  register_host_runtime(m);
  m.doc() = "bigdl_amd native HIP kernels for gfx950 (MI355X)";
  m.def("conv_nt", &conv_nt, py::arg("src"), py::arg("wt"), py::arg("out"), py::arg("bias"), py::arg("stats"),
        py::arg("geo"), py::arg("taps"), py::arg("relu"), py::arg("addend") = py::none(), py::arg("bn_x") = py::none(),
        py::arg("bn_z") = py::none(), py::arg("bn_mean") = py::none(), py::arg("bn_aff") = py::none(),
        py::arg("bn_red") = py::none(), py::arg("accumulate") = false, py::arg("bn_zm") = py::none(),
        py::arg("addend_zm") = py::none(), py::arg("pre") = py::none(),
        py::arg("addend_stride") = std::vector<int64_t>());
  m.def("dgrad_s2", &dgrad_s2, py::arg("dy"), py::arg("wt"), py::arg("out"), py::arg("bn_x") = py::none(),
        py::arg("bn_z") = py::none(), py::arg("bn_mean") = py::none(), py::arg("bn_aff") = py::none(),
        py::arg("bn_red") = py::none(), py::arg("bn_zm") = py::none());
  m.def("set_dgrad_s2", &bigdl_set_dgrad_s2);
  m.def("conv_addend_stride_applies", &conv_addend_stride_applies, py::arg("geo"), py::arg("taps"), py::arg("sh"),
        py::arg("sw"), py::arg("bn") = 0);
  m.def("conv_wgrad", &conv_wgrad, py::arg("dy"), py::arg("src"), py::arg("dw"), py::arg("dbias"), py::arg("geo"),
        py::arg("pre") = py::none());
  m.def("transpose_krsc", &transpose_krsc);
  m.def("bn_stats", &bn_stats);
  m.def("bn_finalize", &bn_finalize);
  m.def("bn_apply", &bn_apply, py::arg("x"), py::arg("scale"), py::arg("shift"), py::arg("res"), py::arg("y"),
        py::arg("P"), py::arg("C"), py::arg("relu"), py::arg("zm") = py::none());
  m.def("bn_slot_reduce", &bn_slot_reduce);
  m.attr("STAT_SLOTS") = BIGDL_STAT_SLOTS;
  m.def("bn_bwd_reduce", &bn_bwd_reduce, py::arg("dz"), py::arg("z"), py::arg("x"), py::arg("mean"), py::arg("red"),
        py::arg("P"), py::arg("C"), py::arg("aff") = py::none(), py::arg("zm") = py::none());
  m.def("bn_bwd_apply", &bn_bwd_apply, py::arg("dz"), py::arg("z"), py::arg("x"), py::arg("mean"), py::arg("invstd"),
        py::arg("gamma"), py::arg("red"), py::arg("nslots"), py::arg("coef"), py::arg("dx"), py::arg("dres"),
        py::arg("dgamma"), py::arg("dbeta"), py::arg("P"), py::arg("C"), py::arg("aff") = py::none(),
        py::arg("zm") = py::none(), py::arg("x2") = py::none(), py::arg("mean2") = py::none(),
        py::arg("red2") = py::none());
  m.def("relu_fwd", &relu_fwd);
  m.def("dgrad_fill", &dgrad_fill);
  m.def("maxpool_bwd_bnred", &maxpool_bwd_bnred, "k3 s2 maxpool backward + the producing BN's backward reduction",
        py::arg("dy"), py::arg("idx"), py::arg("dx"), py::arg("g"), py::arg("bx"), py::arg("mean"), py::arg("aff"),
        py::arg("zm"), py::arg("red"));
  m.def("hog_cus", &hog_cus, "n one-wave workgroups holding a whole CU's LDS each, spinning `us` microseconds");
  m.def("spin_us", &spin_us, "device-side delay of `us` microseconds on the current stream (straggler injection)");
  m.def("relu_bwd", &relu_bwd);
  m.def("add_bf16", &add_bf16);
  m.def("nchw_to_nhwc", &nchw_to_nhwc);
  m.def("nchw_to_pairs", &nchw_to_pairs);
  m.def("bmm_nt", &bmm_nt, py::arg("a"), py::arg("b"), py::arg("c"), py::arg("alpha") = 1.0, py::arg("accum") = false);
  m.def("pair_weight", &pair_weight);
  m.def("pair_wgrad_add", &pair_wgrad_add);
  m.def("tensor_apply", &tensor_apply, py::arg("out"), py::arg("a"), py::arg("b"), py::arg("c"), py::arg("size"),
        py::arg("so"), py::arg("sa"), py::arg("sb"), py::arg("sc"), py::arg("op"), py::arg("s0") = 0.0,
        py::arg("s1") = 0.0, py::arg("contiguous") = false);
  m.def("tensor_reduce", &tensor_reduce, py::arg("x"), py::arg("outer"), py::arg("R"), py::arg("inner"), py::arg("op"),
        py::arg("p"), py::arg("out"), py::arg("outi"), py::arg("mean"), py::arg("ws"), py::arg("chunks"));
  m.def("gemm_f32", &gemm_f32);
  m.def("index_op", &index_op);
  m.def("masked_fill", &masked_fill);
  m.def("mask_blocks", &mask_blocks);
  m.def("mask_scan", &mask_scan);
  m.def("mask_write", &mask_write);
  m.def("topk_f32", &topk_f32);
  m.def("gemv_f32", &gemv_f32);
  m.def("fill_bytes", &fill_bytes);
  m.def("gemm_bf16", &gemm_bf16, py::arg("a"), py::arg("b"), py::arg("out"), py::arg("form"), py::arg("alpha") = 1.0,
        py::arg("beta") = 0.0, py::arg("bias") = py::none(), py::arg("colsum") = py::none(), py::arg("colscale") = 1.0,
        py::arg("ws") = py::none());
  m.def("gemm_bf16_ws_bytes", &gemm_bf16_ws_bytes);
  m.def("copy_rows_i8", &copy_rows_i8);
  m.def("cast_f32_bf16", &cast_f32_bf16);
  m.def("cast_bf16_f32", &cast_bf16_f32);
  m.def("maxpool_fwd", &maxpool_fwd, py::arg("x"), py::arg("y"), py::arg("idx"), py::arg("g"), py::arg("pre") = py::none());
  m.def("maxpool_bwd", &maxpool_bwd);
  m.def("avgpool_fwd", &avgpool_fwd);
  m.def("avgpool_bwd", &avgpool_bwd);
  m.def("softmax_xent", &softmax_xent);
  m.def("sgd_step", &sgd_step, py::arg("w"), py::arg("g"), py::arg("mom"), py::arg("w16"), py::arg("lr"), py::arg("wd"), py::arg("momentum"), py::arg("dampening"), py::arg("nesterov"), py::arg("first"), py::arg("lr_dev") = py::none(), py::arg("seg_off") = py::none(), py::arg("seg_wd") = py::none(), py::arg("base") = 0);
  m.def("adam_step", &adam_step);
  m.def("optim_step", &optim_step);
  m.def("sumsq", &sumsq);
  m.def("scale_f32", &scale_f32);
  m.def("lstm_cell_fwd", &lstm_cell_fwd);
  m.def("lstm_cell_bwd", &lstm_cell_bwd);
  m.def("image_augment", &image_augment);
  m.def("quantize_act", &quantize_act, py::arg("x"), py::arg("q"), py::arg("amax"), py::arg("scale"), py::arg("N"),
        py::arg("P"), py::arg("C"), py::arg("Cp"), py::arg("static_amax") = false);
  m.def("conv_i8", &conv_i8, py::arg("src"), py::arg("wt"), py::arg("out"), py::arg("bias"), py::arg("xscale"),
        py::arg("wscale"), py::arg("geo"), py::arg("taps"), py::arg("relu"), py::arg("xs_const") = 0.0,
        py::arg("out_scale") = 0.0, py::arg("addend") = py::none(), py::arg("add_scale") = 0.0);
  m.def("pool_i8", &pool_i8);
  m.def("act_fwd", &act_fwd);
  m.def("transpose_krsc_batched", &transpose_krsc_batched);
  m.def("image_pipeline", &image_pipeline);
  m.def("act_bwd", &act_bwd);
  m.def("poolnd_fwd", &poolnd_fwd);
  m.def("poolnd_bwd", &poolnd_bwd);
  m.def("upsample_nearest", &upsample_nearest);
  m.def("quantize_nchw_f32", &quantize_nchw_f32);
  m.def("quantize_wim2col_f32", &quantize_wim2col_f32);
  m.def("quantize_rows_bf16", &quantize_rows_bf16);
  m.def("dequantize_rows", &dequantize_rows);
  m.def("nms", &nms);
  m.def("roi_align_fwd", &roi_align_fwd);
  m.def("roi_pool_fwd", &roi_pool_fwd);
  m.def("roi_pool_bwd", &roi_pool_bwd);
  m.def("lrn_fwd", &lrn_fwd);
  m.def("lrn_bwd", &lrn_bwd);
  m.def("dropout", &dropout);
  m.def("lstm_drop_rep", &lstm_drop_rep);
  m.def("lstm_drop_rep_bwd", &lstm_drop_rep_bwd);
// ... 89 lines not shown
```

csrc/common.h:

```cpp
#pragma once
#include <hip/hip_runtime.h>
#include <stdint.h>

typedef uint16_t bf16_t;

typedef short v8s __attribute__((ext_vector_type(8)));
typedef short v4s __attribute__((ext_vector_type(4)));
typedef float v4f __attribute__((ext_vector_type(4)));
typedef int v4i __attribute__((ext_vector_type(4)));
typedef float v16f __attribute__((ext_vector_type(16)));
typedef unsigned int v4u __attribute__((ext_vector_type(4)));
typedef unsigned int v2u __attribute__((ext_vector_type(2)));

#define WAVE 64
#define LDS_PTR(T) __attribute__((address_space(3))) T*

__device__ __forceinline__ float bf2f(bf16_t v) { return __uint_as_float(((unsigned)v) << 16); }
__device__ __forceinline__ bf16_t f2bf(float f) {
  __bf16 b = (__bf16)f;
  return __builtin_bit_cast(bf16_t, b);
}
__device__ __forceinline__ unsigned pack2bf(float lo, float hi) {
  return (unsigned)f2bf(lo) | ((unsigned)f2bf(hi) << 16);
}
__device__ __forceinline__ float lo_bf(unsigned u) { return __uint_as_float(u << 16); }
__device__ __forceinline__ float hi_bf(unsigned u) { return __uint_as_float(u & 0xffff0000u); }

__device__ __forceinline__ float wave_sum(float v) {
#pragma unroll
  for (int o = 32; o > 0; o >>= 1) v += __shfl_xor(v, o, 64);
  return v;
}
__device__ __forceinline__ float wave_max(float v) {
#pragma unroll
  for (int o = 32; o > 0; o >>= 1) v = fmaxf(v, __shfl_xor(v, o, 64));
  return v;
}

__device__ __forceinline__ int xcd_remap(int bid, int nwg) {
  if (nwg < 16) return bid;
  const int xcd = bid & 7, q = nwg >> 3, r = nwg & 7;
  const int base = (xcd < r) ? xcd * (q + 1) : r * (q + 1) + (xcd - r) * q;
  return base + (bid >> 3);
}

__device__ __forceinline__ v4u mask8_to_bf(unsigned b) {
  v4u r;
#pragma unroll
  for (int e = 0; e < 4; ++e) r[e] = (((b >> (2 * e)) & 1u) ? 0x3f80u : 0u) | (((b >> (2 * e + 1)) & 1u) ? 0x3f800000u : 0u);
  return r;
}
__device__ __forceinline__ v4u mask8_to_and(unsigned b) {
  v4u r;
#pragma unroll
  for (int e = 0; e < 4; ++e) r[e] = (((b >> (2 * e)) & 1u) ? 0xffffu : 0u) | (((b >> (2 * e + 1)) & 1u) ? 0xffff0000u : 0u);
  return r;
}
__device__ __forceinline__ unsigned bf_to_mask8(const v4u& o) {
  unsigned b = 0;
#pragma unroll
  for (int e = 0; e < 4; ++e) b |= ((lo_bf(o[e]) > 0.f) ? 1u : 0u) << (2 * e) | ((hi_bf(o[e]) > 0.f) ? 1u : 0u) << (2 * e + 1);
  return b;
}

#define HIP_LAUNCH_CHECK() (void)hipGetLastError()
```

csrc/conv_igemm.hip:

```cpp
#include "common.h"
#include "kernels.h"
#include <stdlib.h>

#include "conv_epilogue.h"
#include "lds_tr.h"


namespace {

constexpr int BK = 64;

__device__ __attribute__((aligned(64))) bf16_t g_zero_granule[32];
__device__ __forceinline__ v4u load16(const bf16_t* p, bool ok) {
  return *reinterpret_cast<const v4u*>(ok ? p : g_zero_granule);
}

template <int MI, int NI, int TM, int TN>
__device__ __forceinline__ void nt_epilogue(const ConvArgs& a, v4f (&acc)[MI][NI], int mbase, int nbase, int lane,
                                            int bid) {
  const int ohw = a.OH * a.OW;
  const bool vec_ok = (a.Ncol & 3) == 0 && (a.ldo & 3) == 0;
#pragma unroll
  for (int j = 0; j < NI; ++j) {
    const int nb = nbase + j * 16 + (lane >> 4) * 4;
// ... 2883 lines not shown
int bigdl_get_wgrad_tr_asm() { return wgrad_tr_asm() ? 1 : 0; }

static void launch_wgrad_g3(const WgradArgs& a, int blocks, hipStream_t st) {
  if (wgrad_tr_asm()) conv_wgrad_g3_kernel<true><<<dim3(blocks), dim3(256), 0, st>>>(a);
  else conv_wgrad_g3_kernel<false><<<dim3(blocks), dim3(256), 0, st>>>(a);
}
static void launch_wgrad_glds(const WgradArgs& a, int blocks, hipStream_t st) {
  if (wgrad_tr_asm()) conv_wgrad_glds_kernel<true><<<dim3(blocks), dim3(256), 0, st>>>(a);
  else conv_wgrad_glds_kernel<false><<<dim3(blocks), dim3(256), 0, st>>>(a);
}

static int p8w_pick(WgradArgs* a) {
  if (g_wgrad_p8 < 0) {
    const char* e = getenv("BIGDL_WGRAD_P8");
    g_wgrad_p8 = e ? atoi(e) : 1;
  }
  if (!g_wgrad_p8 || conv_impl() < 1 || a->Ncol < 256 || a->Kdim < 256 || (a->Cs % 8) ||
      (a->Ncol % 8) || (a->Kdim % 8) || a->M <= 0)
    return 0;
  const long tiles = (long)((a->Ncol + 255) / 256) * ((a->Kdim + 255) / 256);
  if (g_wgrad_p8 == 1 && !(a->R * a->S == 1 && tiles >= 32)) return 0;
  const long steps = (a->M + 63) / 64;
  const long cap = std::max(1L, (256L << 20) / ((long)a->Ncol * a->Kdim * 4));
  const long smax = std::max(1L, std::min({8L, steps / 8, cap}));
  long splits = 1;
  double best = 0.0;
  for (long sp = 1; sp <= smax; ++sp) {
    const long wgs = tiles * sp;
    const double eff = (double)wgs / (double)(((wgs + 255) / 256) * 256);
    if (eff > best + 0.02) { best = eff; splits = sp; }
  }
  long mps = (a->M + splits - 1) / splits;
  mps = (mps + 63) / 64 * 64;
  splits = (a->M + mps - 1) / mps;
  a->m_per_split = (int)mps;
  return (int)splits;
}

int bigdl_conv_wgrad_uses_p8(const WgradArgs* a_in) {
  WgradArgs a = *a_in;
  return p8w_pick(&a) > 0 ? 1 : 0;
}

int bigdl_conv_wgrad_uses_register_kernel(const WgradArgs* a) {
  return (conv_impl() < 1 || wgrad_prefers_atomic(a)) ? 1 : 0;
}

long bigdl_conv_wgrad_plan(WgradArgs* a) {
  if (conv_impl() >= 1) {
    const long sw = bigdl_stem_wgrad_plan(a);
    if (sw > 0) {
      a->splits = -1;
      return sw;
    }
  }
  const int hs = bigdl_wgrad_halo_plan(a);
  if (hs > 0) {
    a->splits = hs;
    return hs > 1 ? (long)hs * a->Ncol * a->Kdim + (a->dbias ? (long)hs * a->Ncol : 0) : 0;
  }
  const int p8w = p8w_pick(a);
  if (p8w > 0) {
    a->splits = p8w;
    return p8w > 1 ? (long)p8w * a->Ncol * a->Kdim : 0;
  }
  const int tiles = ((a->Ncol + WT - 1) / WT) * ((a->Kdim + WT - 1) / WT);
  if (conv_impl() < 1 || wgrad_prefers_atomic(a)) { a->splits = 0; return 0; }
  static const int target = [] { const char* e = getenv("BIGDL_WGRAD_WGS"); return e ? atoi(e) : 512; }();
  int splits = (target + tiles - 1) / tiles;
  const int maxsplit = (a->M + 8 * WBM - 1) / (8 * WBM);
  if (splits > maxsplit) splits = maxsplit;
  if (splits < 1) splits = 1;
  int mps = (a->M + splits - 1) / splits;
  mps = (mps + WBM - 1) / WBM * WBM;
  splits = (a->M + mps - 1) / mps;
  a->m_per_split = mps;
  a->splits = splits;
  return splits > 1 ? (long)splits * a->Ncol * a->Kdim : 0;
}

static int conv_wgrad_impl(const WgradArgs* a_in, hipStream_t st);

int bigdl_conv_wgrad(const WgradArgs* a_in, hipStream_t st) {
  if (bigdl_deterministic() && a_in->dbias != nullptr && (a_in->ldy % 8) == 0) {
    WgradArgs b = *a_in;
    b.dbias = nullptr;
    const int rc = conv_wgrad_impl(&b, st);
    if (rc == 0) bigdl_colsum_bf16_ld(a_in->dy, a_in->dbias, a_in->M, a_in->Ncol, a_in->ldy, st, a_in->det_ws);
    return rc;
  }
  return conv_wgrad_impl(a_in, st);
}

static int conv_wgrad_impl(const WgradArgs* a_in, hipStream_t st) {
  WgradArgs a = *a_in;
  if (a.pre) {
    WgradArgs b = a;
    const int hs = bigdl_wgrad_halo_plan(&b);
    if (hs <= 0 || hs != a.splits || (hs > 1 && a.ws == nullptr)) return -6;
    b.splits = hs;
    b.ws = hs > 1 ? a.ws : nullptr;
    const int rc = bigdl_wgrad_halo(&b, st);
    HIP_LAUNCH_CHECK();
    return rc;
  }
  if (a.splits == -1 && a.ws != nullptr && bigdl_stem_wgrad_plan(&a) > 0) {
    const int rc = bigdl_stem_wgrad(&a, st);
    HIP_LAUNCH_CHECK();
    return rc;
  }
  if (a.Cs % 8 != 0 || a.Ncol % 8 != 0 || a.Kdim % 8 != 0) return -1;
  {
    WgradArgs b = a;
    const int hs = bigdl_wgrad_halo_plan(&b);
    if (hs > 0 && hs == a.splits && (hs == 1 || a.ws != nullptr)) {
      b.splits = hs;
      b.ws = hs > 1 ? a.ws : nullptr;
      if (bigdl_wgrad_halo(&b, st) == 0) {
        HIP_LAUNCH_CHECK();
        return 0;
      }
    }
  }
  {
    WgradArgs b = a;
    const int p8w = p8w_pick(&b);
    if (p8w > 0 && p8w == a.splits && (p8w == 1 || a.ws != nullptr)) {
      b.splits = p8w;
      b.ws = a.ws;
      const int tiles = ((a.Ncol + 255) / 256) * ((a.Kdim + 255) / 256);
      const bool direct = a.R == 1 && a.S == 1 && a.sh == 1 && a.sw == 1 && a.ph == 0 && a.pw == 0 && a.Hs == a.OH &&
                          a.Ws == a.OW;
      const dim3 grid(tiles, p8w);
      if (wgrad_tr_asm()) {
        if (direct) conv_wgrad_p8_kernel<true, true><<<grid, dim3(512), 0, st>>>(b);
        else conv_wgrad_p8_kernel<false, true><<<grid, dim3(512), 0, st>>>(b);
      } else {
        if (direct) conv_wgrad_p8_kernel<true, false><<<grid, dim3(512), 0, st>>>(b);
        else conv_wgrad_p8_kernel<false, false><<<grid, dim3(512), 0, st>>>(b);
      }
      if (p8w > 1) {
        const long n4 = (long)a.Ncol * a.Kdim / 4;
        const int blocks = (int)std::min<long>((n4 + 255) / 256, 8192);
        if ((reinterpret_cast<uintptr_t>(a.dw) & 15) == 0) wgrad_reduce_kernel<true><<<dim3(blocks, 1), 256, 0, st>>>(a.ws, a.dw, n4, p8w);
        else wgrad_reduce_kernel<false><<<dim3(blocks, 1), 256, 0, st>>>(a.ws, a.dw, n4, p8w);
      }
      HIP_LAUNCH_CHECK();
      return 0;
    }
  }
  if (a.ws != nullptr && a.splits > 1 && conv_impl() >= 1) {
    const int tiles = ((a.Ncol + WT - 1) / WT) * ((a.Kdim + WT - 1) / WT);
    const int spad = (a.splits + 7) / 8 * 8;
    if (wgrad_g3()) launch_wgrad_g3(a, tiles * spad, st);
    else launch_wgrad_glds(a, tiles * spad, st);
    const long n4 = (long)a.Ncol * a.Kdim / 4;
    const int blocks = (int)std::min<long>((n4 + 255) / 256, 8192);
    const int groups = (blocks >= 256 || bigdl_deterministic()) ? 1
                                                               : std::max(1, std::min({2048 / blocks, a.splits / 4, 64}));
    const dim3 rgrid(blocks, groups);
    if ((reinterpret_cast<uintptr_t>(a.dw) & 15) == 0) wgrad_reduce_kernel<true><<<rgrid, 256, 0, st>>>(a.ws, a.dw, n4, a.splits);
    else wgrad_reduce_kernel<false><<<rgrid, 256, 0, st>>>(a.ws, a.dw, n4, a.splits);
    HIP_LAUNCH_CHECK();
    return 0;
  }
  a.ws = nullptr;
  const int tiles = ((a.Ncol + WT - 1) / WT) * ((a.Kdim + WT - 1) / WT);
  int splits = (512 + tiles - 1) / tiles;
  const long tile_bytes = (long)tiles * WT * WT * 4;
  static const long atomic_mb = [] { const char* e = getenv("BIGDL_WGRAD_ATOMIC_MB"); return e ? atol(e) : 32l; }();
  const int cap_atomic = (int)((atomic_mb << 20) / tile_bytes);
  if (splits > cap_atomic) splits = cap_atomic;
  const int maxsplit = (a.M + 4 * WBM - 1) / (4 * WBM);
  if (splits > maxsplit) splits = maxsplit;
  if (splits < 1 || bigdl_deterministic()) splits = 1;
  int mps = (a.M + splits - 1) / splits;
  mps = (mps + WBM - 1) / WBM * WBM;
  splits = (a.M + mps - 1) / mps;
// ... 28 lines not shown
```

csrc/kernels.h:

```cpp
#pragma once
#include <hip/hip_runtime.h>
#include <stdint.h>

#define CONV_MAX_TAPS 64
struct ConvArgs {
  const uint16_t* src;
  const uint16_t* wt;
  uint16_t* out;
  const float* bias;
  float* stats;
  const uint16_t* addend;
  const uint8_t* addzm;
  const uint16_t* bnx;
  const uint16_t* bnz;
  const uint8_t* bnzm;
  const float* bnmean;
  const float* bnaff;
  float* bnred;
  int Nb, Hs, Ws, Cs;
  int OH, OW;
  int mul_h, mul_w;
  int ntaps, ldw;
  int M, Ncol, Kdim, ldo;
  int OHo, OWo, omul_h, omul_w, ooff_h, ooff_w, ident_out;
  int relu;
  short tap_h[CONV_MAX_TAPS], tap_w[CONV_MAX_TAPS], tap_k[CONV_MAX_TAPS];
  float* out32;
  int accum32;
  float* ws;
  int ksplit;
  int pstride;
  const float* pre;
  int add_sh, add_sw, add_H, add_W;
  unsigned add_mow, add_moh, add_msh, add_msw;
};

struct I8Epi {
  const float* xscale;
  float xs_const;
  const float* wscale;
  int out_mode;
  float out_inv;
  const int8_t* add8;
  float add_scale;
  long add_ld;
};

struct WgradArgs {
  const uint16_t* dy;
  const uint16_t* src;
  float* dw;
  float* dbias;
  int Nb, Hs, Ws, Cs, OH, OW, R, S;
  int sh, sw, ph, pw, dh, dwl;
  int M, Ncol, Kdim, ldy;
  int m_per_split;
  float* ws;
  int splits;
  float* det_ws;
  const float* pre;
};

extern "C" {
void bigdl_fill_bytes(void* ptr, int value, long bytes, hipStream_t st);
int bigdl_deterministic();
void bigdl_set_deterministic(int v);
#define BIGDL_DET_SLOTS 128
void bigdl_colsum_bf16_ld(const uint16_t* x, float* out, long P, int K, long ld, hipStream_t st,
                          float* det_ws = nullptr);
int bigdl_conv_pre_applies(const ConvArgs* a);
void bigdl_conv_addend_stride(ConvArgs* a, int sh, int sw, int add_h, int add_w);
int bigdl_conv_addend_stride_applies(const ConvArgs* a);
int bigdl_conv_nt(const ConvArgs* a, hipStream_t st);
int bigdl_conv_halo_applies(const ConvArgs* a);
int bigdl_conv_halo(const ConvArgs* a, hipStream_t st);
void bigdl_set_conv_halo(int v);
int bigdl_dgrad_s2_applies(const ConvArgs* a);
int bigdl_dgrad_s2(const ConvArgs* a, hipStream_t st);
void bigdl_set_dgrad_s2(int v);
int bigdl_conv_halo_i8_applies(const ConvArgs* a, const I8Epi* ep);
int bigdl_conv_halo_i8(const ConvArgs* a, const I8Epi* ep, hipStream_t st);
int bigdl_stem_fwd_applies(const ConvArgs* a);
int bigdl_stem_fwd(const ConvArgs* a, hipStream_t st);
void bigdl_set_stem_fwd(int v);
long bigdl_stem_wgrad_plan(const WgradArgs* a);
int bigdl_stem_wgrad(const WgradArgs* a, hipStream_t st);
void bigdl_set_stem_wgrad(int v);
long bigdl_conv_nt_plan(ConvArgs* a);
int bigdl_bmm_nt(const uint16_t* A, const uint16_t* B, float* C, int batch, int M, int N, int K, long sa, long sb,
                 long sc, int lda, int ldb, int ldc, float alpha, int accum, hipStream_t st);
void bigdl_nchw_to_pairs(const float* x, uint16_t* y, int N, int C, int H, int W, int Hp, int Wp, int ph, int pw,
                         hipStream_t st);
void bigdl_pair_weight(const uint16_t* w, uint16_t* wp, int K, int C, int R, int S, const long* strides,
                       hipStream_t st);
void bigdl_pair_wgrad_add(const float* dwp, float* gw, int K, int C, int R, int S, const long* strides, float scale,
                          hipStream_t st);
int bigdl_conv_wgrad(const WgradArgs* a, hipStream_t st);
long bigdl_conv_wgrad_plan(WgradArgs* a);
void bigdl_transpose_krsc(const uint16_t* w, uint16_t* wt, int K, int RS, int C, hipStream_t st);
void bigdl_transpose_krsc_batched(const long* desc, int n, int total_tiles, hipStream_t st);

#define BIGDL_STAT_SLOTS 128
void bigdl_bn_stats(const uint16_t* x, float* stats, long P, int C, hipStream_t st);
void bigdl_bn_finalize(const float* stats, int nslots, const float* gamma, const float* beta, float* run_mean,
                       float* run_var, float* save_mean, float* save_invstd, float* scale, float* shift,
                       long P, int C, float eps, float momentum, int training, hipStream_t st);
void bigdl_bn_slot_reduce(const float* in, int nslots, int C, float* out, hipStream_t st);
void bigdl_bn_apply(const uint16_t* x, const float* scale, const float* shift, const uint16_t* res,
                    uint16_t* y, long P, int C, int relu, hipStream_t st, uint8_t* zm = nullptr);
void bigdl_bn_bwd_reduce(const uint16_t* dz, const uint16_t* z, const uint16_t* x, const float* mean,
                         float* red, long P, int C, const float* aff, hipStream_t st, const uint8_t* zm = nullptr);
void bigdl_bn_bwd_apply(const uint16_t* dz, const uint16_t* z, const uint16_t* x, const float* mean,
                        const float* invstd, const float* gamma, const float* red, int nslots, float* coef,
                        uint16_t* dx, uint16_t* dres, float* dgamma, float* dbeta, long P, int C, int training,
                        const float* aff, hipStream_t st, const uint8_t* zm = nullptr,
                        const uint16_t* x2 = nullptr, const float* mean2 = nullptr, float* red2 = nullptr);

void bigdl_relu_fwd(const uint16_t* x, uint16_t* y, long n, hipStream_t st);
void bigdl_spin_us(double us, int* done, hipStream_t st);
void bigdl_dgrad_fill(uint16_t* out, const uint16_t* add, long npix, int H, int W, int C, int sh, int sw, unsigned mask,
                      hipStream_t st);
void bigdl_relu_bwd(const uint16_t* dy, const uint16_t* y, uint16_t* dx, long n, hipStream_t st);
void bigdl_add_bf16(const uint16_t* a, const uint16_t* b, uint16_t* y, long n, hipStream_t st);
void bigdl_nchw_f32_to_nhwc_bf16(const float* x, uint16_t* y, int N, int C, int H, int W, int Cp,
                                 hipStream_t st);
void bigdl_cast_f32_bf16(const float* x, uint16_t* y, long n, hipStream_t st);
void bigdl_colsum_bf16(const uint16_t* x, float* out, long P, int K, hipStream_t st, float* det_ws = nullptr);
void bigdl_ones_col_pack(const uint16_t* x, uint16_t* xe, long M, int K, hipStream_t st);
void bigdl_ones_col_acc(const float* gw, float* gW, float* gB, long N, int K, float sW, float sB, hipStream_t st);
void bigdl_cast_bf16_f32(const uint16_t* x, float* y, long n, hipStream_t st);

void bigdl_maxpool_fwd(const uint16_t* x, uint16_t* y, uint8_t* idx, int N, int H, int W, int C, int OH,
                       int OW, int kh, int kw, int sh, int sw, int ph, int pw, hipStream_t st, const float* pre = nullptr);
int bigdl_maxpool_pre_applies(int N, int H, int W, int C, int OH, int OW, int kh, int kw, int sh, int sw);
int bigdl_stem_i8_applies(const ConvArgs* a, const I8Epi* ep);
void bigdl_set_stem_i8(int v);
int bigdl_stem_i8_f32(const ConvArgs* a, const I8Epi* ep, const float* img, int C, int W, float inv, hipStream_t st);
int bigdl_stem_i8(const ConvArgs* a, const I8Epi* ep, hipStream_t st);
void bigdl_split_reduce_f32(const float* ws, float* dw, long n, int splits, hipStream_t st);
int bigdl_maxpool_bwd_bnred_applies(int N, int H, int W, int C, int OH, int OW, int kh, int kw, int sh, int sw, int ph,
                                    int pw);
void bigdl_maxpool_bwd_bnred(const uint16_t* dy, const uint8_t* idx, uint16_t* dx, int N, int C, int OH, int OW,
                             const uint16_t* bx, const float* mean, const float* aff, const uint8_t* zm, float* red,
                             hipStream_t st);
void bigdl_maxpool_bwd(const uint16_t* dy, const uint8_t* idx, uint16_t* dx, int N, int H, int W, int C,
                       int OH, int OW, int kh, int kw, int sh, int sw, int ph, int pw, hipStream_t st);
void bigdl_avgpool_fwd(const uint16_t* x, uint16_t* y, int N, int H, int W, int C, int OH, int OW, int kh,
                       int kw, int sh, int sw, int ph, int pw, int count_pad, hipStream_t st);
void bigdl_avgpool_bwd(const uint16_t* dy, uint16_t* dx, int N, int H, int W, int C, int OH, int OW, int kh,
                       int kw, int sh, int sw, int ph, int pw, int count_pad, hipStream_t st);

void bigdl_softmax_xent(const uint16_t* logits_bf16, const float* logits_f32, const float* labels,
                        float* loss, uint16_t* dlogits_bf16, float* dlogits_f32, int B, int K,
                        float label_base, float grad_scale, hipStream_t st);

void bigdl_sgd_step(float* w, const float* g, float* mom, uint16_t* w16, long n, const float* lr_dev, float lr,
                    float wd, float momentum, float dampening, int nesterov, int first, const long* seg_off,
                    const float* seg_wd, int nseg, long base, hipStream_t st);
void bigdl_adam_step(float* w, const float* g, float* m, float* v, uint16_t* w16, long n, float lr,
                     float beta1, float beta2, float eps, float wd, float bc1, float bc2, hipStream_t st);
void bigdl_sumsq(const float* x, float* out, long n, hipStream_t st, float* det_ws = nullptr);
void bigdl_scale_f32(float* x, long n, const float* scale_dev, float scale, hipStream_t st);

void bigdl_lstm_cell_fwd(const float* gates, const float* c_prev, float* c, float* h, float* act, int B,
                         int H, hipStream_t st);
void bigdl_lstm_cell_bwd(const float* act, const float* c_prev, const float* c, const float* dh,
                         const float* dc_next, float* dgates, float* dc_prev, int B, int H, hipStream_t st);

int bigdl_quantize_act(const void* x, int is_bf16, int8_t* q, float* amax, float* scale, int N, long P, int C,
                       int Cp, int static_amax, hipStream_t st);
int bigdl_conv_i8(const ConvArgs* a, const float* xscale, float xs_const, const float* wscale, int out_mode,
                  float out_inv, const int8_t* add8, float add_scale, long add_ld, hipStream_t st);
void bigdl_pool_i8(const int8_t* x, int8_t* y, int N, int H, int W, int Cp, int OH, int OW, int kh, int kw, int sh,
                   int sw, int ph, int pw, int avg, int count_pad, long ldo, hipStream_t st);
void bigdl_quantize_nchw_f32(const float* x, int8_t* q, int N, int C, int HW, int Cp, float inv, hipStream_t st);
void bigdl_quantize_wim2col_f32(const float* x, int8_t* y, int N, int C, int H, int W, int OW, int S, int sw, int pw,
                                float inv, hipStream_t st);
void bigdl_quantize_rows_bf16(const uint16_t* x, int8_t* q, long P, int C, long ldq, float inv, hipStream_t st);
void bigdl_dequantize_rows(const int8_t* q, uint16_t* y, long P, int C, long ld, float scale, hipStream_t st);

int bigdl_tensor_apply(float* out, const float* a, const float* b, const float* c, int nd, const long* size,
                       const long* so, const long* sa, const long* sb, const long* sc, int op, float s0, float s1,
                       int contiguous, hipStream_t st);
int bigdl_index_op(int op, float* a, const void* idx, int idx_i64, const float* b, float* out, long outer, long R,
                   long n, long inner, long Rsrc, int* err, hipStream_t st);
void bigdl_masked_fill(float* x, const float* mask, float v, long n, hipStream_t st);
long bigdl_mask_blocks(long n);
void bigdl_mask_scan(const float* mask, long n, int* counts, hipStream_t st);
void bigdl_mask_write(int copy, float* x, const float* mask, const float* src, float* out, long n, const int* counts,
                      long nsrc, hipStream_t st);
int bigdl_topk(const float* x, long outer, long R, long inner, int k, int largest, float* vals, float* inds,
               hipStream_t st);
// ... 179 lines not shown
```

csrc/stem_fwd.hip:

```cpp
#include <algorithm>
#include <cstdlib>
#include <type_traits>
#include <utility>

#include "common.h"
#include "kernels.h"
#include "conv_epilogue.h"

namespace {

constexpr int SR = 7, SRB = 4, SOW = 112, SFM = SOW / 16, SXROWS = 2 * SRB + SR - 2;
constexpr int SWST = 30 * 16;

template <int WQ>
struct StemL {
  static constexpr int XB = SXROWS * WQ * 16;
  static constexpr int XG = (XB / 16 + 255) / 256;
  static constexpr int WOFF = (XG * 256 * 16 + 1023) / 1024 * 1024;
  static constexpr int LDS0 = WOFF + 64 * SWST;
  static constexpr int EPI = 4 * SFM * 16 * 128 + 4 * 128 * 4;
  static constexpr int LDS = LDS0 > EPI ? LDS0 : EPI;
};

struct StemRowMap {
// ... 8 lines not shown
  const int tid = threadIdx.x, lane = tid & 63;
  const int wave = __builtin_amdgcn_readfirstlane(tid >> 6);
  const int tiles_img = a.OH / SRB;
  const int bid = xcd_remap(blockIdx.x, a.Nb * tiles_img);
  const int n = bid / tiles_img, oh0 = (bid - n * tiles_img) * SRB;

  const bf16_t* src = reinterpret_cast<const bf16_t*>(a.src);
  const size_t xoff = ((size_t)n * a.Hs + 2 * oh0) * WQ * 8;
  const size_t xend = (size_t)a.Nb * a.Hs * WQ * 8;
  const __amdgpu_buffer_rsrc_t rx = __builtin_amdgcn_make_buffer_rsrc(const_cast<bf16_t*>(src + xoff), (short)0,
                                                                      (int)((xend - xoff) * 2), 0x00020000);
#pragma unroll
  for (int d = 0; d < L::XG; ++d)
    __builtin_amdgcn_raw_ptr_buffer_load_lds(rx, (LDS_PTR(void))(lds + (d * 4 + wave) * 1024), 16,
                                             ((d * 4 + wave) * 64 + lane) * 16, 0, 0, 0);
  const bf16_t* wt = reinterpret_cast<const bf16_t*>(a.wt);
  for (int q = tid; q < 64 * 28; q += 256) {
    const int k = q / 28, g = q - k * 28;
    *reinterpret_cast<v4u*>(lds + L::WOFF + k * SWST + g * 16) =
        *reinterpret_cast<const v4u*>(wt + (size_t)k * a.ldw + g * 8);
  }
  asm volatile("s_waitcnt vmcnt(0)" ::: "memory");
  __syncthreads();

  v4f acc[SFM][4];
#pragma unroll
  for (int i = 0; i < SFM; ++i)
#pragma unroll
    for (int j = 0; j < 4; ++j) acc[i][j] = v4f{0.f, 0.f, 0.f, 0.f};
  const unsigned char* W = lds + L::WOFF + (lane & 15) * SWST + (lane >> 4) * 16;
#pragma unroll
  for (int r = 0; r < SR; ++r) {
    v8s fw[4], fx[SFM];
#pragma unroll
    for (int j = 0; j < 4; ++j) fw[j] = *reinterpret_cast<const v8s*>(W + j * 16 * SWST + r * 64);
    const unsigned char* X = lds + ((2 * wave + r) * WQ + (lane & 15) + (lane >> 4)) * 16;
#pragma unroll
    for (int i = 0; i < SFM; ++i) fx[i] = *reinterpret_cast<const v8s*>(X + i * 16 * 16);
#pragma unroll
    for (int i = 0; i < SFM; ++i)
#pragma unroll
      for (int j = 0; j < 4; ++j) acc[i][j] = __builtin_amdgcn_mfma_f32_16x16x32_bf16(fw[j], fx[i], acc[i][j], 0, 0, 0);
  }
  __syncthreads();
  const StemRowMap rm{((long)n * a.OH + oh0) * SOW};
  halo_epi_lean<SFM, 4, 1, 64>(a, acc, wave * SOW, 0, lane, bid, lds + wave * SFM * 16 * 128, rm,
                               reinterpret_cast<float*>(lds + 4 * SFM * 16 * 128), 0);
}

}

extern "C" {

static int g_stem_fwd = -1;
void bigdl_set_stem_fwd(int v) { g_stem_fwd = v; }

int bigdl_stem_fwd_applies(const ConvArgs* a) {
  if (g_stem_fwd < 0) {
    const char* e = getenv("BIGDL_STEM_FWD");
    g_stem_fwd = e ? atoi(e) : 1;
  }
  if (!g_stem_fwd || a->Cs != 8 || a->ntaps != SR * 4 || a->mul_h != 2 || a->mul_w != 1 || a->OW != SOW || a->Ws != 115 ||
      a->OH % SRB || a->Ncol != 64 || a->ldw != SR * 32 || a->Kdim != SR * 32 || !a->ident_out || a->ldo != 64 ||
      a->out32 || a->addend || a->bnred || a->pstride || a->ws)
    return 0;
  if (a->Hs < 2 * a->OH + SR - 2) return 0;
  for (int t = 0; t < SR * 4; ++t)
    if (a->tap_h[t] != t / 4 || a->tap_w[t] != t % 4 || a->tap_k[t] != t) return 0;
  if ((size_t)a->Nb * a->Hs * a->Ws * 16 >= (1ull << 31) || (size_t)a->Nb * a->OH * a->OW * 128 >= (1ull << 31)) return 0;
  return 1;
}

int bigdl_stem_fwd(const ConvArgs* a, hipStream_t st) {
  stem_fwd_kernel<115><<<dim3(a->Nb * (a->OH / SRB)), dim3(256), 0, st>>>(*a);
  return 0;
}

}

namespace {

constexpr int SWRB = 2, SWPX = SWRB * SOW, SWXROWS = 2 * SWRB + SR - 2;

template <int WQ>
struct StemW {
  static constexpr int XB = SWXROWS * WQ * 16;
  static constexpr int XI = (XB + 7 * 1024 - 1) / (7 * 1024);
  static constexpr int XR = XI * 7 * 1024;
  static constexpr int DB = SWPX * 128;
  static constexpr int DI = DB / (7 * 1024);
  static constexpr int LDS1 = XR + DB;
  static constexpr int LDS = 2 * LDS1;
  static_assert(DB % (7 * 1024) == 0, "dy tile must split into DMA rounds");
  static_assert(LDS <= 160 * 1024, "two tile buffers per workgroup");
};

__device__ __forceinline__ int dyswz(int row) { return (((row >> 1) & 1) << 1) | (((row >> 3) & 1) << 2); }

template <int OFF>
__device__ __forceinline__ v8s trd2s(unsigned a0, unsigned a1) {
  v4s lo, hi;
  asm volatile("ds_read_b64_tr_b16 %0, %1 offset:%2" : "=v"(lo) : "v"(a0), "n"(OFF));
  asm volatile("ds_read_b64_tr_b16 %0, %1 offset:%2" : "=v"(hi) : "v"(a1), "n"(OFF));
  return v8s{lo[0], lo[1], lo[2], lo[3], hi[0], hi[1], hi[2], hi[3]};
}

template <int WQ>
__global__ __launch_bounds__(448, 1) void stem_wgrad_kernel(WgradArgs a) {
  using L = StemW<WQ>;
  __shared__ __attribute__((aligned(1024))) unsigned char lds[L::LDS];
  const int tid = threadIdx.x, lane = tid & 63;
  const int r = __builtin_amdgcn_readfirstlane(tid >> 6);
  const int tiles_img = a.OH / SWRB, ntiles = a.Nb * tiles_img;
  const bf16_t* xs = reinterpret_cast<const bf16_t*>(a.src);
  const bf16_t* dys = reinterpret_cast<const bf16_t*>(a.dy);
  const size_t xend = (size_t)a.Nb * a.Hs * WQ * 8, dend = (size_t)a.M * 64;
  const unsigned lb = (unsigned)(uintptr_t)(LDS_PTR(unsigned char))lds;
  unsigned dsrc[L::DI];
#pragma unroll
  for (int d = 0; d < L::DI; ++d) {
    const int Q = (d * 7 + r) * 64 + lane, row = Q >> 3, sl = Q & 7;
    dsrc[d] = (unsigned)((row * 8 + (sl ^ dyswz(row))) * 16);
  }
  const int g = lane >> 4, q = (lane & 15) >> 2, p = lane & 3;
  v4f acc[4][2], accb[4];
#pragma unroll
  for (int i = 0; i < 4; ++i) acc[i][0] = acc[i][1] = accb[i] = v4f{0.f, 0.f, 0.f, 0.f};
  const bool bias = a.dbias != nullptr && r == 0;
  const v8s ones = {(short)0x3f80, (short)0x3f80, (short)0x3f80, (short)0x3f80,
                    (short)0x3f80, (short)0x3f80, (short)0x3f80, (short)0x3f80};

  auto issue = [&](int t, int buf) {
    const int n = t / tiles_img, oh0 = (t - n * tiles_img) * SWRB;
    const size_t xo = ((size_t)n * a.Hs + 2 * oh0) * WQ * 8, dofs = ((size_t)n * a.OH + oh0) * SOW * 64;
    const __amdgpu_buffer_rsrc_t rx = __builtin_amdgcn_make_buffer_rsrc(const_cast<bf16_t*>(xs + xo), (short)0,
                                                                        (int)((xend - xo) * 2), 0x00020000);
    const __amdgpu_buffer_rsrc_t rd = __builtin_amdgcn_make_buffer_rsrc(const_cast<bf16_t*>(dys + dofs), (short)0,
                                                                        (int)((dend - dofs) * 2), 0x00020000);
    unsigned char* B = lds + buf * L::LDS1;
#pragma unroll
    for (int d = 0; d < L::XI; ++d)
      __builtin_amdgcn_raw_ptr_buffer_load_lds(rx, (LDS_PTR(void))(B + (d * 7 + r) * 1024), 16,
                                               ((d * 7 + r) * 64 + lane) * 16, 0, 0, 0);
#pragma unroll
    for (int d = 0; d < L::DI; ++d)
      __builtin_amdgcn_raw_ptr_buffer_load_lds(rd, (LDS_PTR(void))(B + L::XR + (d * 7 + r) * 1024), 16,
                                               (int)dsrc[d], 0, 0, 0);
  };
  int buf = 0;
  if ((int)blockIdx.x < ntiles) issue(blockIdx.x, 0);
  for (int t = blockIdx.x; t < ntiles; t += gridDim.x, buf ^= 1) {
    asm volatile("s_waitcnt vmcnt(0)" ::: "memory");
    __syncthreads();
    if (t + (int)gridDim.x < ntiles) issue(t + gridDim.x, buf ^ 1);
    const unsigned bb = lb + (unsigned)(buf * L::LDS1);
#pragma unroll
    for (int c = 0; c < SWPX / 32; ++c) {
      const int ra = c * 32 + 8 * g + q;
      unsigned da[2][4];
#pragma unroll
      for (int h = 0; h < 2; ++h)
#pragma unroll
        for (int kf = 0; kf < 4; ++kf)
          da[h][kf] = bb + L::XR + (unsigned)((ra + 4 * h) * 128 + (((2 * kf + (p >> 1)) ^ dyswz(ra + 4 * h)) << 4) +
                                              (p & 1) * 8);
      unsigned xa[2];
#pragma unroll
      for (int h = 0; h < 2; ++h) {
        const int px = ra + 4 * h;
        const int ohl = px >= SOW ? 1 : 0, ow = px - ohl * SOW;
        xa[h] = bb + (unsigned)((((2 * ohl + r) * WQ + ow + (p >> 1)) * 16) + (p & 1) * 8);
      }
      v8s fa[4], fb[2];
#pragma unroll
      for (int kf = 0; kf < 4; ++kf) fa[kf] = trd2s<0>(da[0][kf], da[1][kf]);
      fb[0] = trd2s<0>(xa[0], xa[1]);
      fb[1] = trd2s<32>(xa[0], xa[1]);
      asm volatile("s_waitcnt lgkmcnt(0)" ::: "memory");
      __builtin_amdgcn_sched_barrier(0);
#pragma unroll
      for (int kf = 0; kf < 4; ++kf)
#pragma unroll
        for (int nf = 0; nf < 2; ++nf)
          acc[kf][nf] = __builtin_amdgcn_mfma_f32_16x16x32_bf16(fa[kf], fb[nf], acc[kf][nf], 0, 0, 0);
      if (bias) {
#pragma unroll
        for (int kf = 0; kf < 4; ++kf) accb[kf] = __builtin_amdgcn_mfma_f32_16x16x32_bf16(fa[kf], ones, accb[kf], 0, 0, 0);
      }
      __builtin_amdgcn_sched_barrier(0);
    }
  }
  float* o = a.ws + (size_t)blockIdx.x * 64 * 224;
#pragma unroll
  for (int kf = 0; kf < 4; ++kf)
#pragma unroll
    for (int nf = 0; nf < 2; ++nf)
#pragma unroll
      for (int e = 0; e < 4; ++e)
        o[(size_t)(kf * 16 + 4 * (lane >> 4) + e) * 224 + r * 32 + nf * 16 + (lane & 15)] = acc[kf][nf][e];
  if (bias && (lane & 15) == 0) {
    float* ob = a.ws + (size_t)gridDim.x * 64 * 224 + (size_t)blockIdx.x * 64;
#pragma unroll
    for (int kf = 0; kf < 4; ++kf)
#pragma unroll
      for (int e = 0; e < 4; ++e) ob[kf * 16 + 4 * (lane >> 4) + e] = accb[kf][e];
  }
}

}

extern "C" {

static int g_stem_wgrad = -1;
void bigdl_set_stem_wgrad(int v) { g_stem_wgrad = v; }

static int stem_wgrad_grid() {
  static int cus = 0;
  if (cus == 0) {
    int dev = 0;
    (void)hipGetDevice(&dev);
    (void)hipDeviceGetAttribute(&cus, hipDeviceAttributeMultiprocessorCount, dev);
    if (cus <= 0) cus = 256;
  }
  return cus;
}

long bigdl_stem_wgrad_plan(const WgradArgs* a) {
  if (g_stem_wgrad < 0) {
    const char* e = getenv("BIGDL_STEM_WGRAD");
    g_stem_wgrad = e ? atoi(e) : 1;
  }
  if (!g_stem_wgrad || a->Cs != 8 || a->R != SR || a->S != 4 || a->sh != 2 || a->sw != 1 || a->ph || a->pw ||
      a->dh != 1 || a->dwl != 1 || a->OW != SOW || a->Ws != 115 || (a->OH % SWRB) || a->Ncol != 64 ||
      a->Kdim != SR * 32 || a->ldy != 64 || a->M != a->Nb * a->OH * a->OW || a->Hs < 2 * a->OH + SR - 2)
    return 0;
  if ((size_t)a->Nb * a->Hs * a->Ws * 16 >= (1ull << 31) || (size_t)a->M * 128 >= (1ull << 31)) return 0;
  const long tiles = (long)a->Nb * (a->OH / SWRB);
  return (long)std::min<long>(tiles, stem_wgrad_grid()) * (64 * 224 + 64);
}

int bigdl_stem_wgrad(const WgradArgs* a, hipStream_t st) {
  const long tiles = (long)a->Nb * (a->OH / SWRB);
  const int grid = (int)std::min<long>(tiles, stem_wgrad_grid());
  stem_wgrad_kernel<115><<<dim3(grid), dim3(448), 0, st>>>(*a);
  bigdl_split_reduce_f32(a->ws, a->dw, 64 * 224, grid, st);
  if (a->dbias) bigdl_split_reduce_f32(a->ws + (size_t)grid * 64 * 224, a->dbias, 64, grid, st);
  return 0;
}

}
```

Measured before the change: 12250 images/sec.

## Fuse stem BN backward into stem wgrad load and fold shortcut BN into residual apply

The stem BN backward no longer writes dx. It computes only its coefficients and passes the raw gradient plus those coefficients to the stem weight-gradient kernel, which applies the BN backward and ReLU mask as tiles arrive in LDS. Separately, the shortcut BN output is deferred: its affine transform is applied inside the main branch's BN apply kernel. Its backward also skips materializing dres by reusing the output gradient with a mask. The aim is to remove full-activation writes and reads, in exchange for more LDS per block and complex eligibility checks with error paths.

```diff
diff --git a/bigdl_amd/nn/conv.py b/bigdl_amd/nn/conv.py
--- a/bigdl_amd/nn/conv.py
+++ b/bigdl_amd/nn/conv.py
@@ -172,7 +172,23 @@
         self._geom = (x.shape, ph, pw)
         return y
 
-    def _wgrad_gpu_pairs(self, x, gy16):
+    def _takes_bn_grad_pre(self, gz, y):
+        xpair = getattr(self, "_xpair", None)
+        if (xpair is None or self.propagateBack or self._frozen or self.fuse_relu or self.nGroup != 1
+                or self.format != "NCHW" or self.gradWeight.dtype != torch.float32
+                or type(self)._wgrad_gpu is not SpatialConvolution._wgrad_gpu
+                or type(self).accGradParameters is not SpatialConvolution.accGradParameters
+                or y is not self.output or not (gz.is_cuda and gz.dtype == BF16 and gz.shape == y.shape
+                                                and gz.stride() == y.stride())):
+            return False
+        xp = xpair[0]
+        K = self.nOutputPlane
+        if y.shape[0] != xp.shape[0] or y.shape[1] != K or y.dtype != BF16:
+            return False
+        return cv.pairs_wgrad_takes_bn_pre(xp, K, y.shape[2], y.shape[3], self.kernelH, (self.kernelW + 1) // 2,
+                                           self.strideH, self.bias is not None)
+
+    def _wgrad_gpu_pairs(self, x, gy16, bn_pre=None):
         xp, shape, ph, pw = self._xpair
         R, S, K = self.kernelH, self.kernelW, self.nOutputPlane
         S2 = (S + 1) // 2
@@ -180,7 +196,7 @@
         db = None
         if self.bias is not None:
             db = self.gradBias if self.scaleB == 1.0 else ops.zeros(K, device=x.device)
-        cv.conv2d_pairs_wgrad(gy16, xp, R, S2, self.strideH, dwp, db)
+        cv.conv2d_pairs_wgrad(gy16, xp, R, S2, self.strideH, dwp, db, bn_pre=bn_pre)
         ops.native.get().pair_wgrad_add(dwp, self.gradWeight, float(self.scaleW))
         if db is not None and db is not self.gradBias:
             self.gradBias.add_(db, alpha=self.scaleB)
@@ -374,11 +390,15 @@
 
     def _wgrad_gpu(self, x, gy, ph, pw):
         gy16 = gy if (gy.dtype == BF16 and gy.is_contiguous(memory_format=CL)) else gy.to(BF16, memory_format=CL)
+        bn_pre = getattr(gy, "_bn_grad_pre", None)
         xpair = getattr(self, "_xpair", None)
         if (xpair is not None and xpair[1] == tuple(x.shape) and xpair[2:] == (ph, pw) and self.nGroup == 1
-                and self.gradWeight.dtype == torch.float32):
-            self._wgrad_gpu_pairs(x, gy16)
+                and self.gradWeight.dtype == torch.float32 and (bn_pre is None or gy16 is gy)):
+            self._wgrad_gpu_pairs(x, gy16, bn_pre)
             return
+        if bn_pre is not None:
+            raise RuntimeError("SpatialConvolution: a BN backward to apply on load reached a weight gradient other "
+                               "than the pair-view stem kernel's")
         x16 = getattr(self, "_x16", None)
         pre = None
         if x16 is None or x16.shape[0] != x.shape[0] or x16.shape[2:] != x.shape[2:]:
diff --git a/bigdl_amd/nn/fusion.py b/bigdl_amd/nn/fusion.py
--- a/bigdl_amd/nn/fusion.py
+++ b/bigdl_amd/nn/fusion.py
@@ -29,7 +29,7 @@
             x._graph_dres = False
     for x in m.flattened_layers():
         for attr, val in (("emit_stats", False), ("fuse_relu", False), ("passthrough", False),
-                          ("_dgrad_bn_ok", False), ("_defer_ok", False)):
+                          ("_dgrad_bn_ok", False), ("_defer_ok", False), ("_grad_to", None)):
             if hasattr(x, attr):
                 setattr(x, attr, val)
         if isinstance(x, Sequential):
@@ -173,6 +173,8 @@
     for a, b in zip(mods[:-1], mods[1:]):
         if isinstance(a, SpatialConvolution) and isinstance(b, BatchNormalization) and a.nGroup == 1:
             a.emit_stats = True
+            if not a.propagateBack:
+                b._grad_to = a
         elif isinstance(a, BatchNormalization) and isinstance(b, ReLU):
             a.fuse_relu = True
             b.passthrough = True
@@ -208,10 +210,33 @@
         a._defer_ok = True
 
 
+SHORTCUT_FOLD = [os.environ.get("BIGDL_SHORTCUT_FOLD", "1") != "0"]
+
+SHORTCUT_NODRES = [os.environ.get("BIGDL_SHORTCUT_NODRES", "1") != "0"]
+
+
+def _shortcut_fold_bn(short, x):
+    if not (SHORTCUT_FOLD[0] and isinstance(short, Sequential) and len(short.modules) >= 2
+            and short._residual_plan is None and torch.is_tensor(x) and x.is_cuda):
+        return None
+    sbn = short.modules[-1]
+    if not (isinstance(sbn, BatchNormalization) and sbn.train and not sbn.fuse_relu and sbn.nOutput % 8 == 0
+            and sbn.sync_fn is None and sbn.dataFormat == "NCHW"):
+        return None
+    return sbn
+
+
 def residual_forward(seq, x):
     branch, short, bn = seq._residual_plan
     concat, add, relu = seq.modules
-    res = short.forward(x)
+    sbn = _shortcut_fold_bn(short, x)
+    if sbn is not None:
+        sbn._fold_once = True
+    try:
+        res = short.forward(x)
+    finally:
+        if sbn is not None:
+            sbn.__dict__.pop("_fold_once", None)
     h = x
     for m in branch.modules[:-1]:
         h = m.forward(h)
@@ -298,7 +323,15 @@
                 from ..ops import bn as bnops
 
                 sec = (xs, sbn.saveMean, bnops.new_stats(xs.shape[1], xs.device))
-        dh, dres = bn.backward_fused(seq._res_h, gradOutput, need_dres=True, sec=sec)
+        nodres = (SHORTCUT_NODRES[0] and sec is not None and zm is not None and bn.train and xs.dim() == 4
+                  and torch.is_tensor(gradOutput) and gradOutput.is_cuda and tuple(gradOutput.shape) == tuple(xs.shape))
+        dh, dres = bn.backward_fused(seq._res_h, gradOutput, need_dres=not nodres, sec=sec)
+        if nodres:
+            dres = gradOutput
+            if dres.dtype != torch.bfloat16 or dres.stride() != xs.stride():
+                dres = dres.to(torch.bfloat16).contiguous(memory_format=torch.channels_last)
+            dres = dres.detach()
+            dres._bn_gmask = zm
         if sec is not None:
             dres._bn_red = (sbn, sec[2])
         sconv = _compact_shortcut_conv(short, first, x) if can_fold else None
diff --git a/bigdl_amd/nn/normalization.py b/bigdl_amd/nn/normalization.py
--- a/bigdl_amd/nn/normalization.py
+++ b/bigdl_amd/nn/normalization.py
@@ -11,11 +11,14 @@
 
 _ZMASK = os.environ.get("BIGDL_BN_ZMASK", "1") != "0"
 _DEFER = [os.environ.get("BIGDL_BN_DEFER", "1") != "0"]
+_STEM_BNPRE = os.environ.get("BIGDL_STEM_BNPRE", "1") != "0"
 CL = torch.channels_last
 BF16 = torch.bfloat16
 
 
 class BatchNormalization(TensorModule):
+
+    _grad_to = None
 
     def __init__(self, nOutput, eps=1e-5, momentum=0.1, affine=True, initWeight=None, initBias=None,
                  initGradWeight=None, initGradBias=None, dataFormat="NCHW"):
@@ -92,9 +95,22 @@
     def updateOutput(self, input, residual=None):
         if residual is None:
             residual = self.__dict__.pop("_graph_residual", None)
+        fold = self.__dict__.pop("_fold_once", False)
         x = self._to_nchw(input)
+        res_aff = getattr(residual, "_bn_lin", None)
+        if res_aff is not None and not (self._gpu_ok(x) and residual.dtype == BF16 and x.dtype == BF16
+                                        and residual.stride() == x.stride()):
+            residual, res_aff = bnops.materialize(residual), None
         if self._gpu_ok(x):
             stats = getattr(input, "_bn_stats", None) if self.train else None
+            if (fold and self.train and not self.fuse_relu and residual is None and self.sync_fn is None
+                    and x.dim() == 4 and self.dataFormat == "NCHW" and x.dtype == BF16
+                    and x.is_contiguous(memory_format=CL)):
+                sm, si, aff = bnops.bn_prepare_gpu(x, self.weight, self.bias, self.runningMean, self.runningVar,
+                                                   self.eps, self.momentum, stats=stats)
+                self.saveMean, self.saveStd = sm, si
+                self._aff, self._zm, self._xin = None, None, x
+                return bnops.deferred(x, aff, relu=False)
             x = self._prep_gpu(x)
             res = residual
             if res is not None and (res.dtype != BF16 or res.stride() != x.stride()):
@@ -114,7 +130,7 @@
             y, sm, si, aff = bnops.bn_forward_gpu(x, self.weight, self.bias, self.runningMean, self.runningVar,
                                                    self.eps, self.momentum, self.train, stats=stats, res=res,
                                                    relu=self.fuse_relu, sync_fn=self.sync_fn if self.train else None,
-                                                   zm=zm)
+                                                   zm=zm, res_aff=res_aff)
             self.saveMean, self.saveStd = sm, si
             self._aff = aff if (self.fuse_relu and res is None) else None
             self._zm = zm
@@ -145,16 +161,32 @@
         aff = getattr(self, "_aff", None)
         zm = getattr(self, "_zm", None)
         z = self._to_nchw(self.output) if (self.fuse_relu and aff is None and zm is None) else None
+        gmask = getattr(gradOutput, "_bn_gmask", None)
+        if gmask is not None:
+            if self.fuse_relu:
+                raise ValueError("BatchNormalization: a masked output gradient needs a BN without fused ReLU")
+            z, aff, zm = None, None, gmask
         direct = self._direct_grads()
         dg = self.gradWeight if direct else (torch.zeros_like(self.runningMean) if self.affine else None)
         db = self.gradBias if direct else (torch.zeros_like(self.runningMean) if self.affine else None)
         pre = getattr(gradOutput, "_bn_red", None)
         red = pre[1] if (pre is not None and pre[0] is self and self.train) else None
         graph_res = getattr(self, "_graph_dres", False)
-        dx, dres = bnops.bn_backward_gpu(gz, z, x, self.saveMean, self.saveStd, self.weight, dg, db,
-                                         training=self.train, need_dres=need_dres or graph_res,
-                                         sync_fn=self.sync_fn if self.train else None, aff=aff, red=red, zm=zm,
-                                         sec=sec)
+        conv = self._grad_to
+        if (_STEM_BNPRE and conv is not None and red is not None and self.sync_fn is None and aff is not None
+                and z is None and zm is None and not need_dres and sec is None and not graph_res and x.dim() == 4
+                and self.dataFormat == "NCHW" and gz.is_contiguous(memory_format=CL)
+                and not ops.native.deterministic() and conv._takes_bn_grad_pre(gz, x)):
+            coef = torch.empty(3 * x.shape[1], dtype=torch.float32, device=x.device)
+            bnops.bn_backward_gpu(gz, None, x, self.saveMean, self.saveStd, self.weight, dg, db, training=True,
+                                  need_dx=False, aff=aff, red=red, coef=coef)
+            dx, dres = gz.detach(), None
+            dx._bn_grad_pre = (x, coef, aff)
+        else:
+            dx, dres = bnops.bn_backward_gpu(gz, z, x, self.saveMean, self.saveStd, self.weight, dg, db,
+                                             training=self.train, need_dres=need_dres or graph_res,
+                                             sync_fn=self.sync_fn if self.train else None, aff=aff, red=red, zm=zm,
+                                             sec=sec)
         if graph_res:
             self._dres = dres
         if not direct and self.affine and not self._frozen:
diff --git a/bigdl_amd/ops/bn.py b/bigdl_amd/ops/bn.py
--- a/bigdl_amd/ops/bn.py
+++ b/bigdl_amd/ops/bn.py
@@ -59,7 +59,7 @@
 
 
 def bn_forward_gpu(x, gamma, beta, rmean, rvar, eps, momentum, training, stats=None, res=None, relu=False,
-                   out=None, sync_fn=None, zm=None):
+                   out=None, sync_fn=None, zm=None, res_aff=None):
     C = x.shape[1]
     P = _P(x)
     C_ = native.get()
@@ -82,7 +82,10 @@
         stats, nslots = scale, 0
     C_.bn_finalize(stats, nslots, gamma, beta, rmean, rvar, smean, sinv, scale, shift, Ptot, C, float(eps),
                    float(momentum), bool(training))
-    C_.bn_apply(x, scale, shift, res, out, P, C, bool(relu), zm)
+    if res_aff is not None:
+        C_.bn_apply(x, scale, shift, res, out, P, C, bool(relu), zm, res_aff[:C], res_aff[C:])
+    else:
+        C_.bn_apply(x, scale, shift, res, out, P, C, bool(relu), zm)
     return out, smean, sinv, aff
 
 
@@ -105,24 +108,29 @@
     return smean, sinv, aff
 
 
-def deferred(x, aff):
+def deferred(x, aff, relu=True):
     y = x.detach()
-    y._bn_pre = aff
+    if relu:
+        y._bn_pre = aff
+    else:
+        y._bn_lin = aff
     return y
 
 
 def materialize(t):
-    aff = getattr(t, "_bn_pre", None)
+    aff, relu = getattr(t, "_bn_pre", None), True
+    if aff is None:
+        aff, relu = getattr(t, "_bn_lin", None), False
     if aff is None:
         return t
     C = t.shape[1]
     y = torch.empty_like(t)
-    native.get().bn_apply(t, aff[:C], aff[C:], None, y, _P(t), C, True)
+    native.get().bn_apply(t, aff[:C], aff[C:], None, y, _P(t), C, relu)
     return y
 
 
 def bn_backward_gpu(dz, z, x, smean, sinv, gamma, dgamma, dbeta, training=True, need_dres=False, need_dx=True,
-                    sync_fn=None, aff=None, red=None, zm=None, sec=None):
+                    sync_fn=None, aff=None, red=None, zm=None, sec=None, coef=None):
     C = x.shape[1]
     P = _P(x)
     C_ = native.get()
@@ -136,10 +144,11 @@
         nslots = stat_slots()
         if sync_fn is not None:
             red, nslots, Ptot = _reduce_slots_for_sync(red, C, P, sync_fn)
-    coef = torch.empty(3 * C, dtype=torch.float32, device=x.device)
+    if coef is None:
+        coef = torch.empty(3 * C, dtype=torch.float32, device=x.device)
     dx = torch.empty_like(x) if need_dx else None
     dres = torch.empty_like(x) if need_dres else None
-    if sec is not None and dres is not None and training:
+    if sec is not None and training:
         x2, mean2, red2 = sec
         C_.bn_bwd_apply(dz, z, x, smean, sinv, gamma, red, nslots, coef, dx, dres, dgamma, dbeta, Ptot, C, aff, zm,
                         x2=x2, mean2=mean2, red2=red2)
diff --git a/bigdl_amd/ops/conv.py b/bigdl_amd/ops/conv.py
--- a/bigdl_amd/ops/conv.py
+++ b/bigdl_amd/ops/conv.py
@@ -374,10 +374,22 @@
     return out
 
 
-def conv2d_pairs_wgrad(dy, xp, R, S2, sh, dwp32, dbias32):
+def _pairs_wgrad_geo(N, Hp, Wq, K, OH, OW, R, S2, sh):
+    return [N, Hp, Wq, 8, OH, OW, R, S2, sh, 1, 0, 0, 1, 1, N * OH * OW, K, R * S2 * 8, K]
+
+
+def pairs_wgrad_takes_bn_pre(xp, K, OH, OW, R, S2, sh, bias):
+    N, Hp, Wq, _ = xp.shape
+    return native.get().conv_wgrad_plan_info(_pairs_wgrad_geo(N, Hp, Wq, K, OH, OW, R, S2, sh), bool(bias))[0] == -1
+
+
+def conv2d_pairs_wgrad(dy, xp, R, S2, sh, dwp32, dbias32, bn_pre=None):
     N, Hp, Wq, _ = xp.shape
     _, K, OH, OW = dy.shape
-    geo = [N, Hp, Wq, 8, OH, OW, R, S2, sh, 1, 0, 0, 1, 1, N * OH * OW, K, R * S2 * 8, K]
+    geo = _pairs_wgrad_geo(N, Hp, Wq, K, OH, OW, R, S2, sh)
+    if bn_pre is not None:
+        native.get().conv_wgrad(dy, xp, dwp32, dbias32, geo, None, bn_pre[0], bn_pre[1], bn_pre[2])
+        return
     native.get().conv_wgrad(dy, xp, dwp32, dbias32, geo)
 
 
diff --git a/csrc/batchnorm.hip b/csrc/batchnorm.hip
--- a/csrc/batchnorm.hip
+++ b/csrc/batchnorm.hip
@@ -152,11 +152,17 @@
   shift[c] = b - mean * g * invstd;
 }
 
-template <int U>
+__device__ __forceinline__ void load8(const float* p, float* v) {
+  const v4f a = *reinterpret_cast<const v4f*>(p), b = *reinterpret_cast<const v4f*>(p + 4);
+  v[0] = a[0]; v[1] = a[1]; v[2] = a[2]; v[3] = a[3]; v[4] = b[0]; v[5] = b[1]; v[6] = b[2]; v[7] = b[3];
+}
+
+template <int U, bool RA>
 __global__ __launch_bounds__(256) void bn_apply_kernel(const bf16_t* __restrict__ x, const float* __restrict__ scale,
                                                        const float* __restrict__ shift, const bf16_t* __restrict__ res,
                                                        bf16_t* __restrict__ y, long P, int C, long rpb, int relu,
-                                                       uint8_t* __restrict__ zm) {
+                                                       uint8_t* __restrict__ zm, const float* __restrict__ res_scale,
+                                                       const float* __restrict__ res_shift) {
   const int G = C >> 3;
   const int gbase = blockIdx.y * 256;
   const int gcount = min(256, G - gbase);
@@ -169,6 +175,11 @@
   const v4f b0 = *reinterpret_cast<const v4f*>(shift + c0), b1 = *reinterpret_cast<const v4f*>(shift + c0 + 4);
   const float sc[8] = {s0[0], s0[1], s0[2], s0[3], s1[0], s1[1], s1[2], s1[3]};
   const float sh[8] = {b0[0], b0[1], b0[2], b0[3], b1[0], b1[1], b1[2], b1[3]};
+  float rsc[8], rsh[8];
+  if (RA) {
+    load8(res_scale + c0, rsc);
+    load8(res_shift + c0, rsh);
+  }
   for (long r0 = rbeg + rsub; r0 < rend; r0 += (long)U * rpi) {
     v4u vx[U], vr[U];
 #pragma unroll
@@ -187,7 +198,11 @@
       for (int e = 0; e < 4; ++e) {
         float l = lo_bf(vx[u][e]) * sc[2 * e] + sh[2 * e];
         float h = hi_bf(vx[u][e]) * sc[2 * e + 1] + sh[2 * e + 1];
-        if (res) { l += lo_bf(vr[u][e]); h += hi_bf(vr[u][e]); }
+        if (RA) {
+          const unsigned q = pack2bf(lo_bf(vr[u][e]) * rsc[2 * e] + rsh[2 * e],
+                                     hi_bf(vr[u][e]) * rsc[2 * e + 1] + rsh[2 * e + 1]);
+          l += lo_bf(q); h += hi_bf(q);
+        } else if (res) { l += lo_bf(vr[u][e]); h += hi_bf(vr[u][e]); }
         if (relu) { l = fmaxf(l, 0.f); h = fmaxf(h, 0.f); }
         o[e] = pack2bf(l, h);
       }
@@ -228,11 +243,6 @@
   float t = 0.f;
   for (int k = 0; k < nslots; ++k) t += in[(size_t)k * 2 * C + c];
   out[c] = t;
-}
-
-__device__ __forceinline__ void load8(const float* p, float* v) {
-  const v4f a = *reinterpret_cast<const v4f*>(p), b = *reinterpret_cast<const v4f*>(p + 4);
-  v[0] = a[0]; v[1] = a[1]; v[2] = a[2]; v[3] = a[3]; v[4] = b[0]; v[5] = b[1]; v[6] = b[2]; v[7] = b[3];
 }
 
 template <int U, bool R2>
@@ -292,13 +302,8 @@
         float d0 = lo_bf(vd[u][e]), d1 = hi_bf(vd[u][e]);
         const float x0 = lo_bf(vx[u][e]), x1 = hi_bf(vx[u][e]);
         if (z || zm) { if (!(lo_bf(vz[u][e]) > 0.f)) d0 = 0.f; if (!(hi_bf(vz[u][e]) > 0.f)) d1 = 0.f; }
-        if (xmask) {
-          if (!(x0 * S[2 * e] + T[2 * e] > 0.f)) d0 = 0.f;
-          if (!(x1 * S[2 * e + 1] + T[2 * e + 1] > 0.f)) d1 = 0.f;
-        }
-        const float r0v = A[2 * e] * d0 + B[2 * e] * x0 + D[2 * e];
-        const float r1v = A[2 * e + 1] * d1 + B[2 * e + 1] * x1 + D[2 * e + 1];
-        o[e] = pack2bf(r0v, r1v);
+        o[e] = bn_bwd_pair(d0, d1, x0, x1, xmask, A[2 * e], A[2 * e + 1], B[2 * e], B[2 * e + 1], D[2 * e],
+                           D[2 * e + 1], S[2 * e], S[2 * e + 1], T[2 * e], T[2 * e + 1]);
         od[e] = pack2bf(d0, d1);
         if (R2 && r < rend) {
           const float q0 = lo_bf(od[e]), q1 = hi_bf(od[e]);
@@ -395,15 +400,22 @@
 }
 
 void bigdl_bn_apply(const uint16_t* x, const float* scale, const float* shift, const uint16_t* res, uint16_t* y,
-                    long P, int C, int relu, hipStream_t st, uint8_t* zm) {
+                    long P, int C, int relu, hipStream_t st, uint8_t* zm, const float* res_scale,
+                    const float* res_shift) {
   long rpb = 0;
   const dim3 grid = stationary_grid(P, C, &rpb);
+#define BN_APPLY(UU)                                                                                                   \
+  if (res && res_scale && res_shift)                                                                                   \
+    bn_apply_kernel<UU, true><<<grid, 256, 0, st>>>(x, scale, shift, res, y, P, C, rpb, relu, zm, res_scale, res_shift); \
+  else                                                                                                                 \
+    bn_apply_kernel<UU, false><<<grid, 256, 0, st>>>(x, scale, shift, res, y, P, C, rpb, relu, zm, nullptr, nullptr)
   switch (bn_unroll()) {
-    case 1: bn_apply_kernel<1><<<grid, 256, 0, st>>>(x, scale, shift, res, y, P, C, rpb, relu, zm); break;
-    case 2: bn_apply_kernel<2><<<grid, 256, 0, st>>>(x, scale, shift, res, y, P, C, rpb, relu, zm); break;
-    case 8: bn_apply_kernel<8><<<grid, 256, 0, st>>>(x, scale, shift, res, y, P, C, rpb, relu, zm); break;
-    default: bn_apply_kernel<4><<<grid, 256, 0, st>>>(x, scale, shift, res, y, P, C, rpb, relu, zm); break;
-  }
+    case 1: BN_APPLY(1); break;
+    case 2: BN_APPLY(2); break;
+    case 8: BN_APPLY(8); break;
+    default: BN_APPLY(4); break;
+  }
+#undef BN_APPLY
   HIP_LAUNCH_CHECK();
 }
 
@@ -421,7 +433,7 @@
   const bf16_t* x2 = reinterpret_cast<const bf16_t*>(x2u);
   bn_bwd_coeff_kernel<<<(C + 7) / 8, 256, 0, st>>>(red, nslots, mean, invstd, gamma, coef, dgamma, dbeta, P, C,
                                                     training);
-  if (dx || dres) {
+  if (dx || dres || red2) {
     long rpb = 0;
     const dim3 grid = stationary_grid(P, C, &rpb);
     if (red2) {
diff --git a/csrc/bindings.cpp b/csrc/bindings.cpp
--- a/csrc/bindings.cpp
+++ b/csrc/bindings.cpp
@@ -191,9 +191,9 @@
 }
 
 void conv_wgrad(const Tensor& dy, const Tensor& src, const Tensor& dw, const OptT& dbias, std::vector<int64_t> geo,
-                const OptT& pre) {
+                const OptT& pre, const OptT& bn_x, const OptT& bn_coef, const OptT& bn_aff) {
   TORCH_CHECK(geo.size() == 18, "conv_wgrad: bad geometry");
-  WgradArgs a;
+  WgradArgs a{};
   a.dy = cbf(dy, "dy"); a.src = cbf(src, "src"); a.dw = mf(dw, "dw"); a.dbias = omf(dbias, "dbias");
   int* f = &a.Nb;
   for (int i = 0; i < 18; ++i) f[i] = (int)geo[i];
@@ -201,6 +201,19 @@
   a.ws = nullptr;
   a.splits = 0;
   a.pre = ocf(pre, "pre");
+  const bool bnpre = bn_x && bn_x->defined();
+  if (bnpre) {
+    TORCH_CHECK(!a.pre && bn_coef && bn_coef->defined() && bn_aff && bn_aff->defined(),
+                "conv_wgrad: bn_x comes with bn_coef and bn_aff and without pre");
+    TORCH_CHECK(bn_x->numel() == dy.numel() && bn_x->strides() == dy.strides() && a.ldy == a.Ncol,
+                "conv_wgrad: bn_x must have dy's shape and layout");
+    TORCH_CHECK(bn_coef->numel() >= 3 * a.Ncol && bn_coef->is_contiguous() && bn_aff->numel() >= 2 * a.Ncol &&
+                    bn_aff->is_contiguous(),
+                "conv_wgrad: bn_coef is [3 Ncol], bn_aff is [2 Ncol]");
+    a.pre_x = cbf(*bn_x, "bn_x");
+    a.pre_coef = cf(*bn_coef, "bn_coef");
+    a.pre_aff = cf(*bn_aff, "bn_aff");
+  }
   Tensor det_ws;
   a.det_ws = nullptr;
   if (bigdl_deterministic() && a.dbias) {
@@ -229,6 +242,7 @@
     a.ws = ws.data_ptr<float>();
   }
   const int rc = bigdl_conv_wgrad(&a, stream());
+  TORCH_CHECK(rc != -7, "conv_wgrad: a BN backward on load needs the pair-view stem kernel");
   TORCH_CHECK(rc == 0, "conv_wgrad: unsupported shape (channels must be a multiple of 8)");
 }
 
@@ -279,10 +293,19 @@
   bigdl_bn_slot_reduce(cf(in, "in"), (int)nslots, (int)C, mf(out, "out"), stream());
 }
 void bn_apply(const Tensor& x, const Tensor& scale, const Tensor& shift, const OptT& res, const Tensor& y, int64_t P,
-              int64_t C, bool relu, const OptT& zm) {
+              int64_t C, bool relu, const OptT& zm, const OptT& res_scale, const OptT& res_shift) {
   TORCH_CHECK(C % 8 == 0 && x.numel() == P * C && y.numel() == P * C, "bn_apply: shape");
+  const bool ra = res_scale && res_scale->defined();
+  TORCH_CHECK(ra == (res_shift && res_shift->defined()), "bn_apply: res_scale and res_shift come together");
+  if (ra) {
+    TORCH_CHECK(res && res->defined() && res->numel() == P * C, "bn_apply: the residual affine needs a residual");
+    TORCH_CHECK(res_scale->numel() >= C && res_shift->numel() >= C && res_scale->is_contiguous() &&
+                    res_shift->is_contiguous(),
+                "bn_apply: res_scale / res_shift are [C]");
+  }
   bigdl_bn_apply(cbf(x, "x"), cf(scale, "scale"), cf(shift, "shift"), ocbf(res, "res"), mbf(y, "y"), P, (int)C,
-                 relu ? 1 : 0, stream(), omzm(zm, P, C, "zm"));
+                 relu ? 1 : 0, stream(), omzm(zm, P, C, "zm"), ocf(res_scale, "res_scale"),
+                 ocf(res_shift, "res_shift"));
 }
 void bn_bwd_reduce(const Tensor& dz, const OptT& z, const Tensor& x, const Tensor& mean, const Tensor& red, int64_t P,
                    int64_t C, const OptT& aff, const OptT& zm) {
@@ -299,8 +322,7 @@
   TORCH_CHECK(coef.numel() >= 3 * C, "bn_bwd_apply: coef size");
   const bool r2 = red2 && red2->defined();
   if (r2) {
-    TORCH_CHECK(dres && dres->defined() && x2 && x2->defined() && mean2 && mean2->defined(),
-                "bn_bwd_apply: red2 needs dres, x2 and mean2");
+    TORCH_CHECK(x2 && x2->defined() && mean2 && mean2->defined(), "bn_bwd_apply: red2 needs x2 and mean2");
     TORCH_CHECK(x2->numel() == x.numel() && x2->strides() == x.strides(), "bn_bwd_apply: x2 must match x's layout");
     TORCH_CHECK(mean2->numel() >= C && red2->numel() >= (int64_t)BIGDL_STAT_SLOTS * 2 * C, "bn_bwd_apply: mean2 / red2 size");
   }
@@ -1597,12 +1619,14 @@
   m.def("conv_addend_stride_applies", &conv_addend_stride_applies, py::arg("geo"), py::arg("taps"), py::arg("sh"),
         py::arg("sw"), py::arg("bn") = 0);
   m.def("conv_wgrad", &conv_wgrad, py::arg("dy"), py::arg("src"), py::arg("dw"), py::arg("dbias"), py::arg("geo"),
-        py::arg("pre") = py::none());
+        py::arg("pre") = py::none(), py::arg("bn_x") = py::none(), py::arg("bn_coef") = py::none(),
+        py::arg("bn_aff") = py::none());
   m.def("transpose_krsc", &transpose_krsc);
   m.def("bn_stats", &bn_stats);
   m.def("bn_finalize", &bn_finalize);
   m.def("bn_apply", &bn_apply, py::arg("x"), py::arg("scale"), py::arg("shift"), py::arg("res"), py::arg("y"),
-        py::arg("P"), py::arg("C"), py::arg("relu"), py::arg("zm") = py::none());
+        py::arg("P"), py::arg("C"), py::arg("relu"), py::arg("zm") = py::none(), py::arg("res_scale") = py::none(),
+        py::arg("res_shift") = py::none());
   m.def("bn_slot_reduce", &bn_slot_reduce);
   m.attr("STAT_SLOTS") = BIGDL_STAT_SLOTS;
   m.def("bn_bwd_reduce", &bn_bwd_reduce, py::arg("dz"), py::arg("z"), py::arg("x"), py::arg("mean"), py::arg("red"),
diff --git a/csrc/common.h b/csrc/common.h
--- a/csrc/common.h
+++ b/csrc/common.h
@@ -63,4 +63,17 @@
   return b;
 }
 
+__device__ __forceinline__ unsigned bn_bwd_pair(float& d0, float& d1, float x0, float x1, bool xmask, float A0,
+                                                float A1, float B0, float B1, float D0, float D1, float S0, float S1,
+                                                float T0, float T1) {
+#pragma clang fp contract(off)
+  if (xmask) {
+    if (!(__builtin_fmaf(S0, x0, T0) > 0.f)) d0 = 0.f;
+    if (!(__builtin_fmaf(S1, x1, T1) > 0.f)) d1 = 0.f;
+  }
+  const float r0v = A0 * d0 + B0 * x0 + D0;
+  const float r1v = A1 * d1 + B1 * x1 + D1;
+  return pack2bf(r0v, r1v);
+}
+
 #define HIP_LAUNCH_CHECK() (void)hipGetLastError()
diff --git a/csrc/conv_igemm.hip b/csrc/conv_igemm.hip
--- a/csrc/conv_igemm.hip
+++ b/csrc/conv_igemm.hip
@@ -2989,7 +2989,7 @@
 static int conv_wgrad_impl(const WgradArgs* a_in, hipStream_t st);
 
 int bigdl_conv_wgrad(const WgradArgs* a_in, hipStream_t st) {
-  if (bigdl_deterministic() && a_in->dbias != nullptr && (a_in->ldy % 8) == 0) {
+  if (bigdl_deterministic() && a_in->dbias != nullptr && (a_in->ldy % 8) == 0 && a_in->pre_x == nullptr) {
     WgradArgs b = *a_in;
     b.dbias = nullptr;
     const int rc = conv_wgrad_impl(&b, st);
@@ -3001,6 +3001,12 @@
 
 static int conv_wgrad_impl(const WgradArgs* a_in, hipStream_t st) {
   WgradArgs a = *a_in;
+  if (a.pre_x) {
+    if (a.pre || a.splits != -1 || a.ws == nullptr || bigdl_stem_wgrad_plan(&a) <= 0) return -7;
+    const int rc = bigdl_stem_wgrad(&a, st);
+    HIP_LAUNCH_CHECK();
+    return rc;
+  }
   if (a.pre) {
     WgradArgs b = a;
     const int hs = bigdl_wgrad_halo_plan(&b);
diff --git a/csrc/kernels.h b/csrc/kernels.h
--- a/csrc/kernels.h
+++ b/csrc/kernels.h
@@ -59,6 +59,9 @@
   int splits;
   float* det_ws;
   const float* pre;
+  const uint16_t* pre_x;
+  const float* pre_coef;
+  const float* pre_aff;
 };
 
 extern "C" {
@@ -107,7 +110,8 @@
                        long P, int C, float eps, float momentum, int training, hipStream_t st);
 void bigdl_bn_slot_reduce(const float* in, int nslots, int C, float* out, hipStream_t st);
 void bigdl_bn_apply(const uint16_t* x, const float* scale, const float* shift, const uint16_t* res,
-                    uint16_t* y, long P, int C, int relu, hipStream_t st, uint8_t* zm = nullptr);
+                    uint16_t* y, long P, int C, int relu, hipStream_t st, uint8_t* zm = nullptr,
+                    const float* res_scale = nullptr, const float* res_shift = nullptr);
 void bigdl_bn_bwd_reduce(const uint16_t* dz, const uint16_t* z, const uint16_t* x, const float* mean,
                          float* red, long P, int C, const float* aff, hipStream_t st, const uint8_t* zm = nullptr);
 void bigdl_bn_bwd_apply(const uint16_t* dz, const uint16_t* z, const uint16_t* x, const float* mean,
diff --git a/csrc/stem_fwd.hip b/csrc/stem_fwd.hip
--- a/csrc/stem_fwd.hip
+++ b/csrc/stem_fwd.hip
@@ -114,16 +114,17 @@
 
 constexpr int SWRB = 2, SWPX = SWRB * SOW, SWXROWS = 2 * SWRB + SR - 2;
 
-template <int WQ>
+template <int WQ, bool PRE = false>
 struct StemW {
   static constexpr int XB = SWXROWS * WQ * 16;
   static constexpr int XI = (XB + 7 * 1024 - 1) / (7 * 1024);
   static constexpr int XR = XI * 7 * 1024;
   static constexpr int DB = SWPX * 128;
   static constexpr int DI = DB / (7 * 1024);
-  static constexpr int LDS1 = XR + DB;
+  static constexpr int LDS1 = XR + (PRE ? 2 : 1) * DB;
   static constexpr int LDS = 2 * LDS1;
   static_assert(DB % (7 * 1024) == 0, "dy tile must split into DMA rounds");
+  static_assert(DB < 65536, "the BN input tile is addressed through a ds offset field");
   static_assert(LDS <= 160 * 1024, "two tile buffers per workgroup");
 };
 
@@ -137,15 +138,16 @@
   return v8s{lo[0], lo[1], lo[2], lo[3], hi[0], hi[1], hi[2], hi[3]};
 }
 
-template <int WQ>
+template <int WQ, bool PRE>
 __global__ __launch_bounds__(448, 1) void stem_wgrad_kernel(WgradArgs a) {
-  using L = StemW<WQ>;
+  using L = StemW<WQ, PRE>;
   __shared__ __attribute__((aligned(1024))) unsigned char lds[L::LDS];
   const int tid = threadIdx.x, lane = tid & 63;
   const int r = __builtin_amdgcn_readfirstlane(tid >> 6);
   const int tiles_img = a.OH / SWRB, ntiles = a.Nb * tiles_img;
   const bf16_t* xs = reinterpret_cast<const bf16_t*>(a.src);
   const bf16_t* dys = reinterpret_cast<const bf16_t*>(a.dy);
+  const bf16_t* pxs = reinterpret_cast<const bf16_t*>(a.pre_x);
   const size_t xend = (size_t)a.Nb * a.Hs * WQ * 8, dend = (size_t)a.M * 64;
   const unsigned lb = (unsigned)(uintptr_t)(LDS_PTR(unsigned char))lds;
   unsigned dsrc[L::DI];
@@ -153,6 +155,26 @@
   for (int d = 0; d < L::DI; ++d) {
     const int Q = (d * 7 + r) * 64 + lane, row = Q >> 3, sl = Q & 7;
     dsrc[d] = (unsigned)((row * 8 + (sl ^ dyswz(row))) * 16);
+  }
+  float cA[2][8], cB[2][8], cD[2][8], cS[2][8], cT[2][8];
+  if constexpr (PRE) {
+#pragma unroll
+    for (int k = 0; k < 2; ++k) {
+      const int row = ((k * 7 + r) << 3) + (lane >> 3), c0 = ((lane & 7) ^ dyswz(row)) * 8;
+#pragma unroll
+      for (int h = 0; h < 2; ++h) {
+        const v4f va = *reinterpret_cast<const v4f*>(a.pre_coef + c0 + 4 * h);
+        const v4f vb = *reinterpret_cast<const v4f*>(a.pre_coef + 64 + c0 + 4 * h);
+        const v4f vd = *reinterpret_cast<const v4f*>(a.pre_coef + 128 + c0 + 4 * h);
+        const v4f vs = *reinterpret_cast<const v4f*>(a.pre_aff + c0 + 4 * h);
+        const v4f vt = *reinterpret_cast<const v4f*>(a.pre_aff + 64 + c0 + 4 * h);
+#pragma unroll
+        for (int e = 0; e < 4; ++e) {
+          cA[k][4 * h + e] = va[e]; cB[k][4 * h + e] = vb[e]; cD[k][4 * h + e] = vd[e];
+          cS[k][4 * h + e] = vs[e]; cT[k][4 * h + e] = vt[e];
+        }
+      }
+    }
   }
   const int g = lane >> 4, q = (lane & 15) >> 2, p = lane & 3;
   v4f acc[4][2], accb[4];
@@ -178,11 +200,44 @@
     for (int d = 0; d < L::DI; ++d)
       __builtin_amdgcn_raw_ptr_buffer_load_lds(rd, (LDS_PTR(void))(B + L::XR + (d * 7 + r) * 1024), 16,
                                                (int)dsrc[d], 0, 0, 0);
+    if constexpr (PRE) {
+      const __amdgpu_buffer_rsrc_t rp = __builtin_amdgcn_make_buffer_rsrc(const_cast<bf16_t*>(pxs + dofs), (short)0,
+                                                                          (int)((dend - dofs) * 2), 0x00020000);
+#pragma unroll
+      for (int d = 0; d < L::DI; ++d)
+        __builtin_amdgcn_raw_ptr_buffer_load_lds(rp, (LDS_PTR(void))(B + L::XR + L::DB + (d * 7 + r) * 1024), 16,
+                                                 (int)dsrc[d], 0, 0, 0);
+    }
   };
   int buf = 0;
   if ((int)blockIdx.x < ntiles) issue(blockIdx.x, 0);
   for (int t = blockIdx.x; t < ntiles; t += gridDim.x, buf ^= 1) {
     asm volatile("s_waitcnt vmcnt(0)" ::: "memory");
+    if constexpr (PRE) {
+      const unsigned db = lb + (unsigned)(buf * L::LDS1 + L::XR) + (unsigned)((r * 64 + lane) * 16);
+      v4u vd[L::DI], vx[L::DI];
+#pragma unroll
+      for (int d = 0; d < L::DI; ++d)
+        asm volatile("ds_read_b128 %0, %2\n\tds_read_b128 %1, %2 offset:%3"
+                     : "=v"(vd[d]), "=v"(vx[d]) : "v"(db + (unsigned)(d * 7 * 1024)), "n"(L::DB) : "memory");
+      asm volatile("s_waitcnt lgkmcnt(0)" ::: "memory");
+#pragma unroll
+      for (int d = 0; d < L::DI; ++d) asm volatile("" : "+v"(vd[d]), "+v"(vx[d]));
+#pragma unroll
+      for (int d = 0; d < L::DI; ++d) {
+        const int k = d & 1;
+        v4u o;
+#pragma unroll
+        for (int e = 0; e < 4; ++e) {
+          float d0 = lo_bf(vd[d][e]), d1 = hi_bf(vd[d][e]);
+          o[e] = bn_bwd_pair(d0, d1, lo_bf(vx[d][e]), hi_bf(vx[d][e]), true, cA[k][2 * e], cA[k][2 * e + 1],
+                             cB[k][2 * e], cB[k][2 * e + 1], cD[k][2 * e], cD[k][2 * e + 1], cS[k][2 * e],
+                             cS[k][2 * e + 1], cT[k][2 * e], cT[k][2 * e + 1]);
+        }
+        asm volatile("ds_write_b128 %0, %1" ::"v"(db + (unsigned)(d * 7 * 1024)), "v"(o) : "memory");
+      }
+      asm volatile("s_waitcnt lgkmcnt(0)" ::: "memory");
+    }
     __syncthreads();
     if (t + (int)gridDim.x < ntiles) issue(t + gridDim.x, buf ^ 1);
     const unsigned bb = lb + (unsigned)(buf * L::LDS1);
@@ -274,7 +329,12 @@
 int bigdl_stem_wgrad(const WgradArgs* a, hipStream_t st) {
   const long tiles = (long)a->Nb * (a->OH / SWRB);
   const int grid = (int)std::min<long>(tiles, stem_wgrad_grid());
-  stem_wgrad_kernel<115><<<dim3(grid), dim3(448), 0, st>>>(*a);
+  if (a->pre_x) {
+    if (!a->pre_coef || !a->pre_aff) return -7;
+    stem_wgrad_kernel<115, true><<<dim3(grid), dim3(448), 0, st>>>(*a);
+  } else {
+    stem_wgrad_kernel<115, false><<<dim3(grid), dim3(448), 0, st>>>(*a);
+  }
   bigdl_split_reduce_f32(a->ws, a->dw, 64 * 224, grid, st);
   if (a->dbias) bigdl_split_reduce_f32(a->ws + (size_t)grid * 64 * 224, a->dbias, 64, grid, st);
   return 0;
```

Measured after the change: 12530 images/sec, median of 6. 1.02x the previous value.
